# simonamtoft/downsampled-diffusion

Hardware: AMD Instinct MI355X
Metric: images/sec (T=1000 sampling), 256x256 dDDPM-x3 (higher is better)
Workload: dtype f32

## Files before the change

downsampled-diffusion_amd/csrc/attention.hip:

```cpp
#include <cstdlib>

#include "conv_common.h"

namespace ddk {

constexpr int DH = 32;

constexpr int PART = DH + DH + DH * DH;

__global__ __launch_bounds__(256) void linattn_context_kernel(const float* __restrict__ qkv, float* __restrict__ ctx,
                                                              float* __restrict__ part, int HW, int heads, int splits, int rows_per_split,
                                                              int kv_only) {
    __shared__ __attribute__((aligned(16))) float stage[4 * 32 * 33];
    float* kexp = stage;
    float* vs = stage + 64 * DH;
    __shared__ float smax[8 * DH];
    const int bh = blockIdx.x / splits, sp = blockIdx.x % splits;
    const int b = bh / heads, h = bh % heads;
    const int HC = heads * DH, RS = (kv_only ? 2 : 3) * HC;
    const float* base = qkv + (long long)b * HW * RS;
    const float* kp = base + (kv_only ? 0 : HC) + h * DH;
    const float* vp = kp + HC;
    const int tid = threadIdx.x;
    const int n_begin = sp * rows_per_split, n_end = min(HW, n_begin + rows_per_split);

    {
        const int d = tid & 31, ng = tid >> 5;
        float m = -INFINITY;
        for (int n = n_begin + ng; n < n_end; n += 8) m = fmaxf(m, kp[(long long)n * RS + d]);
        smax[ng * DH + d] = m;
        __syncthreads();
        if (tid < DH) {
            float mm = smax[tid];
#pragma unroll
            for (int j = 1; j < 8; ++j) mm = fmaxf(mm, smax[j * DH + tid]);
            smax[tid] = mm;
        }
        __syncthreads();
    }

    const int d = tid >> 3, e0 = (tid & 7) * 4;
    typedef float ctx_f32x16 __attribute__((ext_vector_type(16)));
    const int lane = tid & 63, wv = tid >> 6, l31 = lane & 31, kh = lane >> 5;
    ctx_f32x16 macc;
#pragma unroll
    for (int r = 0; r < 16; ++r) macc[r] = 0.f;
    float dsum = 0.f;
    for (int n0 = n_begin; n0 < n_end; n0 += 64) {
#pragma unroll
        for (int j = 0; j < 2; ++j) {
            const int idx4 = tid + j * 256;
            const int row = idx4 >> 3, c = (idx4 & 7) * 4;
            float4 kv = make_float4(0.f, 0.f, 0.f, 0.f), vv = kv;
            if (n0 + row < n_end) {
                kv = *reinterpret_cast<const float4*>(kp + (long long)(n0 + row) * RS + c);
                vv = *reinterpret_cast<const float4*>(vp + (long long)(n0 + row) * RS + c);
                kv.x = __expf(kv.x - smax[c]);
                kv.y = __expf(kv.y - smax[c + 1]);
                kv.z = __expf(kv.z - smax[c + 2]);
                kv.w = __expf(kv.w - smax[c + 3]);
            }
            *reinterpret_cast<float4*>(kexp + row * DH + c) = kv;
            *reinterpret_cast<float4*>(vs + row * DH + c) = vv;
        }
        __syncthreads();
#pragma unroll
        for (int s2 = 0; s2 < 8; ++s2) {
            const int n = wv * 16 + 2 * s2 + kh;
            const float a = kexp[n * DH + l31];
            macc = __builtin_amdgcn_mfma_f32_32x32x2f32(a, vs[n * DH + l31], macc, 0, 0, 0);
            dsum += a;
        }
        __syncthreads();
    }
    float4 acc;
    float den;
    {
        float* pt = stage;
        static_assert(4 * 32 * 33 >= 2 * 64 * DH, "the staging array holds both tiles");
#pragma unroll
        for (int r = 0; r < 16; ++r) pt[(wv * 32 + (r & 3) + 8 * (r >> 2) + 4 * kh) * 33 + l31] = macc[r];
        dsum += __shfl_xor(dsum, 32, 64);
        __shared__ float dpart[4 * DH];
        if (kh == 0) dpart[wv * DH + l31] = dsum;
        __syncthreads();
        acc = make_float4(0.f, 0.f, 0.f, 0.f);
        den = 0.f;
#pragma unroll
        for (int w = 0; w < 4; ++w) {
            const float* q = pt + (w * 32 + d) * 33 + e0;
            acc.x += q[0]; acc.y += q[1]; acc.z += q[2]; acc.w += q[3];
            den += dpart[w * DH + d];
        }
    }
    if (splits == 1) {
        const float inv = 1.0f / den;
        acc.x *= inv; acc.y *= inv; acc.z *= inv; acc.w *= inv;
        *reinterpret_cast<float4*>(ctx + ((long long)bh * DH + d) * DH + e0) = acc;
    } else {
        float* pp = part + ((long long)bh * splits + sp) * PART;
        if (e0 == 0) { pp[d] = smax[d]; pp[DH + d] = den; }
        *reinterpret_cast<float4*>(pp + 2 * DH + d * DH + e0) = acc;
    }
}

__global__ __launch_bounds__(256) void linattn_merge_kernel(const float* __restrict__ part, float* __restrict__ ctx, int splits) {
    const int bh = blockIdx.x, tid = threadIdx.x;
    const int d = tid >> 3, e0 = (tid & 7) * 4;
    const float* pp = part + (long long)bh * splits * PART;
    float M = -INFINITY;
    for (int s = 0; s < splits; ++s) M = fmaxf(M, pp[s * PART + d]);
    float4 acc = make_float4(0.f, 0.f, 0.f, 0.f);
    float den = 0.f;
    for (int s = 0; s < splits; ++s) {
        const float w = expf(pp[s * PART + d] - M);
        const float4 a = *reinterpret_cast<const float4*>(pp + s * PART + 2 * DH + d * DH + e0);
        den += pp[s * PART + DH + d] * w;
        acc.x += a.x * w; acc.y += a.y * w; acc.z += a.z * w; acc.w += a.w * w;
    }
    const float inv = 1.0f / den;
    acc.x *= inv; acc.y *= inv; acc.z *= inv; acc.w *= inv;
    *reinterpret_cast<float4*>(ctx + ((long long)bh * DH + d) * DH + e0) = acc;
}

constexpr int KC_K = 128, KC_BM = 64;
constexpr int KC_W_FLOATS = 128 * KC_K, KC_A_FLOATS = KC_BM * KC_K;
constexpr int KC_LDS_FLOATS = KC_W_FLOATS + 2 * KC_A_FLOATS + 2 * KC_BM + 64 + 64 + 8 * 64 + 8 * DH;

#if !defined(DDK_TUNING) || !defined(DDK_KVCTX_ABL)
#undef DDK_KVCTX_ABL
#define DDK_KVCTX_ABL 0
#endif
struct KvCtxParams {
    const float* x;
    const float* w;
    const float* c1;
    const float* c2;
    float eps;
    float* part;
    int tiles_per_image, tiles_per_split, splits;
};

__global__ __launch_bounds__(512) void attn_kvctx_kernel(const KvCtxParams p) {
    extern __shared__ __attribute__((aligned(16))) float smem[];
    float* Ws = smem;
    float* As = smem + KC_W_FLOATS;
    float* rowstat = As + 2 * KC_A_FLOATS;
    float* Mx = rowstat + 2 * KC_BM;
    float* Sc = Mx + 64;
    float* cmx = Sc + 64;
    float* dpart = cmx + 8 * 64;
    const int tid = threadIdx.x, lane = tid & 63;
    const int wid = __builtin_amdgcn_readfirstlane(tid >> 6);
    const int sp = blockIdx.x, hp = blockIdx.y, b = blockIdx.z;
// ... 366 lines not shown
        *reinterpret_cast<float4*>(vs + row * DH + c) = vv;
        qs[row * (DH + 1) + c] = qv.x; qs[row * (DH + 1) + c + 1] = qv.y; qs[row * (DH + 1) + c + 2] = qv.z; qs[row * (DH + 1) + c + 3] = qv.w;
    }
    __syncthreads();
    if constexpr (ROWS >= 128) linattn_core_mfma<ROWS>(ks, vs, qs, cs, smax, part, ctx, out, b, h, HW, heads);
    else linattn_small_core<ROWS>(ks, vs, qs, cs, smax, ctx, out, b, h, HW, heads);
}

static size_t small_lds_bytes(int rows) {
    return ((size_t)rows * DH * 2 + (size_t)rows * (DH + 1) + DH * (DH + 4) + 16 * DH + (rows >= 128 ? 4 * 32 * 33 : 0)) * 4;
}

typedef float f32x4_att __attribute__((ext_vector_type(4)));
constexpr int QP_PITCH = 100;

__host__ __device__ static inline size_t small_qkv_lds_bytes(int MB, int C) {
    const size_t xs = (size_t)16 * MB * (C + 4), part = (size_t)4 * 16 * MB * QP_PITCH;
    const size_t core = 64 * DH * 2 + 64 * (DH + 1) + DH * (DH + 4) + 8 * DH + 128 + 192;
    return ((xs > part ? xs : part) + core) * 4;
}

template <int MB>
__global__ __launch_bounds__(256) void linattn_small_qkv_kernel(const float* __restrict__ x, const float* __restrict__ wop,
                                                                const float* __restrict__ c1, const float* __restrict__ c2, float ln_eps,
                                                                float* __restrict__ ctx, float* __restrict__ out, int HW, int C, int heads) {
    extern __shared__ __align__(16) float sm[];
    constexpr int ROWS = 16 * MB;
    const int pitch = C + 4, nch = C >> 5;
    const size_t big = (size_t)ROWS * pitch > (size_t)4 * ROWS * QP_PITCH ? (size_t)ROWS * pitch : (size_t)4 * ROWS * QP_PITCH;
    float* xs = sm;
    float* ks = sm + big;
    float* vs = ks + 64 * DH;
    float* qs = vs + 64 * DH;
    float* cs = qs + 64 * (DH + 1);
    float* smax = cs + DH * (DH + 4);
    float* rowstat = smax + 8 * DH;
    float* cfold = rowstat + 128;
    const int b = blockIdx.x / heads, h = blockIdx.x % heads;
    const int tid = threadIdx.x, lane = tid & 63;
    const int wave = __builtin_amdgcn_readfirstlane(tid >> 6);
    const int m = lane & 15, kq = lane >> 4;
    const int HC = heads * DH;

    const float* wl = wop + (size_t)h * nch * 3072 + lane * 4;
    float4 bA[6][2], bB[6][2];
    auto load_b = [&](int chunk, float4 (&bq)[6][2]) {
        chunk = chunk < nch ? chunk : nch - 1;
        const float* wp = wl + (size_t)chunk * 3072;
#pragma unroll
        for (int nb = 0; nb < 6; ++nb) {
            bq[nb][0] = *reinterpret_cast<const float4*>(wp + nb * 512);
            bq[nb][1] = *reinterpret_cast<const float4*>(wp + nb * 512 + 256);
        }
    };
    load_b(wave, bA);
    load_b(wave + 4, bB);
    if (tid < 192) {
        const int n = tid % 96;
        const int col = (n >> 5) * HC + h * DH + (n & 31);
        cfold[tid] = tid < 96 ? c1[col] : c2[col];
    }
    {
        const int q4 = C >> 2;
        for (int i = tid; i < ROWS * q4; i += 256) {
            const int row = i / q4, c = (i - row * q4) << 2;
            const float4 v = row < HW ? *reinterpret_cast<const float4*>(x + ((long long)b * HW + row) * C + c) : make_float4(0.f, 0.f, 0.f, 0.f);
            *reinterpret_cast<float4*>(xs + row * pitch + c) = v;
        }
    }
    __syncthreads();
    {
        constexpr int TPR = 256 / ROWS;
        const int row = tid / TPR, sub = tid % TPR;
        float s1 = 0.f;
        for (int c = sub * 4; c < C; c += TPR * 4) {
            const float4 v = *reinterpret_cast<const float4*>(xs + row * pitch + c);
            s1 += (v.x + v.y) + (v.z + v.w);
        }
#pragma unroll
        for (int o = 1; o < TPR; o <<= 1) s1 += __shfl_xor(s1, o, 64);
        const float inv_c = 1.0f / (float)C;
        const float mean = s1 * inv_c;
        float s2 = 0.f;
        for (int c = sub * 4; c < C; c += TPR * 4) {
            const float4 v = *reinterpret_cast<const float4*>(xs + row * pitch + c);
            const float a0 = v.x - mean, a1 = v.y - mean, a2 = v.z - mean, a3 = v.w - mean;
            s2 += (a0 * a0 + a1 * a1) + (a2 * a2 + a3 * a3);
        }
#pragma unroll
        for (int o = 1; o < TPR; o <<= 1) s2 += __shfl_xor(s2, o, 64);
        if (sub == 0) {
            const float var = s2 * inv_c;
            const float r = 1.0f / (sqrtf(var) + ln_eps);
            rowstat[2 * row] = r;
            rowstat[2 * row + 1] = r * mean;
        }
    }

    f32x4_att acc[MB][6];
#pragma unroll
    for (int i = 0; i < MB; ++i)
#pragma unroll
        for (int nb = 0; nb < 6; ++nb) acc[i][nb] = f32x4_att{0.f, 0.f, 0.f, 0.f};
    auto compute = [&](int chunk, const float4 (&bq)[6][2]) {
        float4 a[MB][2];
#pragma unroll
        for (int i = 0; i < MB; ++i) {
            const float* ap = xs + (i * 16 + m) * pitch + (chunk << 5) + kq * 8;
            a[i][0] = *reinterpret_cast<const float4*>(ap);
            a[i][1] = *reinterpret_cast<const float4*>(ap + 4);
        }
#pragma unroll
        for (int kk = 0; kk < 8; ++kk)
#pragma unroll
            for (int i = 0; i < MB; ++i) {
                const float av = reinterpret_cast<const float*>(&a[i][0])[kk];
#pragma unroll
                for (int nb = 0; nb < 6; ++nb)
                    acc[i][nb] = __builtin_amdgcn_mfma_f32_16x16x4f32(av, reinterpret_cast<const float*>(&bq[nb][0])[kk], acc[i][nb], 0, 0, 0);
            }
    };
    for (int c = wave; c < nch; c += 8) {
        compute(c, bA);
        load_b(c + 8, bA);
        if (c + 4 < nch) compute(c + 4, bB);
        load_b(c + 12, bB);
    }
    __syncthreads();
#pragma unroll
    for (int i = 0; i < MB; ++i)
#pragma unroll
        for (int nb = 0; nb < 6; ++nb)
#pragma unroll
            for (int r = 0; r < 4; ++r) xs[((wave * ROWS) + i * 16 + kq * 4 + r) * QP_PITCH + nb * 16 + m] = acc[i][nb][r];
    __syncthreads();
    for (int e = tid; e < ROWS * 96; e += 256) {
        const int row = e / 96, n = e - row * 96;
        const int sel = n >> 5, d = n & 31;
        float v = sel == 1 ? -INFINITY : 0.f;
        if (row < HW) {
            float s = xs[row * QP_PITCH + n];
#pragma unroll
            for (int w = 1; w < 4; ++w) s += xs[(w * ROWS + row) * QP_PITCH + n];
            v = rowstat[2 * row] * s - rowstat[2 * row + 1] * cfold[n] + cfold[96 + n];
        }
        if (sel == 0) qs[row * (DH + 1) + d] = v;
        else if (sel == 1) ks[row * DH + d] = v;
        else vs[row * DH + d] = v;
    }
    __syncthreads();
    linattn_small_core<ROWS>(ks, vs, qs, cs, smax, ctx, out, b, h, HW, heads);
}

__global__ __launch_bounds__(256) void qkv_operand_pack_kernel(const float* __restrict__ lnw, float* __restrict__ wop, int heads, int cp,
                                                               long long total) {
    const int nch = cp >> 5, HC = heads * DH;
    for (long long idx = blockIdx.x * 256LL + threadIdx.x; idx < total; idx += (long long)gridDim.x * 256) {
        const int j = (int)(idx & 3), lane = (int)((idx >> 2) & 63), half = (int)((idx >> 8) & 1);
        long long r = idx >> 9;
        const int nb = (int)(r % 6); r /= 6;
        const int chunk = (int)(r % nch);
        const int head = (int)(r / nch);
        const int o = (nb >> 1) * HC + head * DH + (nb & 1) * 16 + (lane & 15);
        const int i = chunk * 32 + (lane >> 4) * 8 + half * 4 + j;
        wop[idx] = lnw[(long long)o * cp + i];
    }
}

typedef float f32x16_att __attribute__((ext_vector_type(16)));
__global__ __launch_bounds__(512) void linattn_apply_kernel(const float* __restrict__ qkv, const float* __restrict__ ctx,
                                                            float* __restrict__ out, int HW, int heads, int tiles_per_sample) {
    extern __shared__ __attribute__((aligned(16))) float qs[];
    const int b = blockIdx.x / tiles_per_sample, tile = blockIdx.x % tiles_per_sample;
    const int HC = heads * DH, RS = 3 * HC;
    const int nthreads = 64 * heads;
    const int n0 = tile * 64;
    const int f4_per_row = HC / 4;
    for (int i = threadIdx.x; i < 64 * f4_per_row; i += nthreads) {
        const int row = i / f4_per_row, c4 = i - row * f4_per_row;
        float4 v = make_float4(0.f, 0.f, 0.f, 0.f);
        if (n0 + row < HW) v = *reinterpret_cast<const float4*>(qkv + ((long long)b * HW + n0 + row) * RS + c4 * 4);
        const int hh = (c4 * 4) / DH, d = (c4 * 4) % DH;
        float* dst = qs + (hh * 64 + row) * 33 + d;
        dst[0] = v.x; dst[1] = v.y; dst[2] = v.z; dst[3] = v.w;
    }
    const int h = threadIdx.x >> 6, lane = threadIdx.x & 63;
    const int l31 = lane & 31, fh = lane >> 5;
    const float* cp = ctx + ((long long)b * heads + h) * DH * DH + l31;
    float bf[16];
#pragma unroll
    for (int kk = 0; kk < 16; ++kk) bf[kk] = cp[(2 * kk + fh) * DH];
    __syncthreads();
    const float* qh = qs + h * 64 * 33;
    f32x16_att acc0, acc1;
#pragma unroll
    for (int r = 0; r < 16; ++r) { acc0[r] = 0.f; acc1[r] = 0.f; }
#pragma unroll
    for (int kk = 0; kk < 16; ++kk) {
        const float a0 = qh[l31 * 33 + 2 * kk + fh], a1 = qh[(32 + l31) * 33 + 2 * kk + fh];
        acc0 = __builtin_amdgcn_mfma_f32_32x32x2f32(a0, bf[kk], acc0, 0, 0, 0);
        acc1 = __builtin_amdgcn_mfma_f32_32x32x2f32(a1, bf[kk], acc1, 0, 0, 0);
    }
#pragma unroll
    for (int r = 0; r < 16; ++r) {
        const int px = (r & 3) + 8 * (r >> 2) + 4 * fh;
        if (n0 + px < HW) out[((long long)b * HW + n0 + px) * HC + h * DH + l31] = acc0[r];
        if (n0 + 32 + px < HW) out[((long long)b * HW + n0 + 32 + px) * HC + h * DH + l31] = acc1[r];
    }
}

static void linattn_splits(int B, int HW, int heads, int& splits, int& rows) {
    const int max_s = (int)ceil_div(HW, 64);
#ifdef DDK_TUNING
    const char* cap_env = getenv("DDK_LINATTN_WGS");
    const int cap = cap_env ? atoi(cap_env) : 1024;
#else
    const int cap = 1024;
#endif
    int s = cap / (B * heads);
    if (s < 1) s = 1;
    if (s > max_s) s = max_s;
    rows = (int)(ceil_div(ceil_div(HW, s), 64) * 64);
    splits = (int)ceil_div(HW, rows);
}

size_t linattn_context_workspace_bytes(int B, int HW, int heads) {
    if (B <= 0 || HW <= 0 || heads <= 0) return 0;
    int s, rows;
    linattn_splits(B, HW, heads, s, rows);
    return s > 1 ? (size_t)B * heads * s * PART * sizeof(float) : 0;
}

int linattn_context(const float* qkv, float* ctx, int B, int HW, int heads, void* workspace, size_t workspace_bytes, hipStream_t st,
                    bool kv_only) {
    DDK_REQUIRE(qkv && ctx && B > 0 && HW > 0 && heads > 0, "linattn_context: arguments");
    DDK_REQUIRE(aligned16(qkv) && aligned16(ctx) && aligned16(workspace), "linattn_context: alignment");
    int s, rows;
    linattn_splits(B, HW, heads, s, rows);
    if (s > 1 && (!workspace || workspace_bytes < (size_t)B * heads * s * PART * sizeof(float))) {
        if (workspace) {
            set_error("linattn_context: workspace too small (%zu < %zu)", workspace_bytes, (size_t)B * heads * s * PART * sizeof(float));
            return DDK_ERR_WORKSPACE;
        }
        s = 1;
        rows = HW;
    }
    hipLaunchKernelGGL(linattn_context_kernel, dim3(B * heads * s), dim3(256), 0, st, qkv, ctx, static_cast<float*>(workspace), HW, heads, s, rows,
                       kv_only ? 1 : 0);
    DDK_TRY(check_launch("linattn_context_kernel"));
    if (s > 1) {
        hipLaunchKernelGGL(linattn_merge_kernel, dim3(B * heads), dim3(256), 0, st, static_cast<const float*>(workspace), ctx, s);
        DDK_TRY(check_launch("linattn_merge_kernel"));
    }
    return DDK_OK;
}

int linattn_fused_small(const float* qkv, float* ctx, float* out, int B, int HW, int heads, hipStream_t st) {
    DDK_REQUIRE(qkv && ctx && out && B > 0 && HW > 0 && HW <= 256 && heads > 0, "linattn_fused_small: arguments (HW <= 256)");
    DDK_REQUIRE(aligned16(qkv) && aligned16(ctx) && aligned16(out), "linattn_fused_small: alignment");
    DDK_TRY(ensure_device_init());
    if (HW <= 64)
        hipLaunchKernelGGL(linattn_small_kernel<64>, dim3(B * heads), dim3(256), small_lds_bytes(64), st, qkv, ctx, out, HW, heads);
    else
        hipLaunchKernelGGL(linattn_small_kernel<256>, dim3(B * heads), dim3(256), small_lds_bytes(256), st, qkv, ctx, out, HW, heads);
    return check_launch("linattn_small_kernel");
}

bool linattn_small_qkv_ok(int HW, int C) { return HW > 0 && HW <= 64 && C % 32 == 0 && C >= 32 && small_qkv_lds_bytes(HW <= 16 ? 1 : 4, C) <= 160 * 1024; }

constexpr int FOLD_C = 128;
constexpr int FOLD_LDS_FLOATS = FOLD_C * FOLD_C + 32 * (FOLD_C + 1) + 2 * FOLD_C;
typedef float f32x16_att __attribute__((ext_vector_type(16)));
__global__ __launch_bounds__(256) void attn_fold_kernel(const float* __restrict__ ctx, const float* __restrict__ wqg,
                                                        const float* __restrict__ c1q, const float* __restrict__ c2q,
                                                        const float* __restrict__ wout, const float* __restrict__ bout,
                                                        float* __restrict__ A, float* __restrict__ a1, float* __restrict__ a2) {
    extern __shared__ __align__(16) float sm[];
    float* T = sm;
    float* Wq = T + FOLD_C * FOLD_C;
    float* t1 = Wq + 32 * (FOLD_C + 1);
    float* t2 = t1 + FOLD_C;
    const int b = blockIdx.x, nq = blockIdx.y, tid = threadIdx.x, lane = tid & 63;
    const int wave = __builtin_amdgcn_readfirstlane(tid >> 6);
    const int l31 = lane & 31, kh = lane >> 5;
    {
        const float* cp = ctx + ((long long)b * 4 + wave) * DH * DH;
        const float* wp = wqg + (long long)wave * DH * FOLD_C;
        f32x16_att acc[4];
#pragma unroll
        for (int j = 0; j < 4; ++j)
#pragma unroll
            for (int r = 0; r < 16; ++r) acc[j][r] = 0.f;
        float av[DH / 2], bv[DH / 2][4];
#pragma unroll
        for (int s2 = 0; s2 < DH / 2; ++s2) {
            const int d = 2 * s2 + kh;
            av[s2] = cp[d * DH + l31];
#pragma unroll
            for (int j = 0; j < 4; ++j) bv[s2][j] = wp[d * FOLD_C + j * 32 + l31];
        }
        __builtin_amdgcn_sched_barrier(0);
#pragma unroll
        for (int s2 = 0; s2 < DH / 2; ++s2)
#pragma unroll
            for (int j = 0; j < 4; ++j) acc[j] = __builtin_amdgcn_mfma_f32_32x32x2f32(av[s2], bv[s2][j], acc[j], 0, 0, 0);
#pragma unroll
        for (int j = 0; j < 4; ++j)
#pragma unroll
            for (int r = 0; r < 16; ++r) T[(wave * DH + (r & 3) + 8 * (r >> 2) + 4 * kh) * FOLD_C + j * 32 + l31] = acc[j][r];
    }
    for (int i = tid; i < 32 * FOLD_C; i += 256) Wq[(i >> 7) * (FOLD_C + 1) + (i & 127)] = wout[(long long)nq * 32 * FOLD_C + i];
    if (tid < FOLD_C) {
        const int h = tid >> 5, e = tid & 31;
        const float* ch = ctx + ((long long)b * 4 + h) * DH * DH;
        float u1 = 0.f, u2 = 0.f;
#pragma unroll
        for (int d = 0; d < DH; ++d) {
            const float cv = ch[d * DH + e];
            u1 += cv * c1q[h * DH + d];
            u2 += cv * c2q[h * DH + d];
        }
        t1[tid] = u1;
        t2[tid] = u2;
    }
    __syncthreads();
    {
        f32x16_att acc;
#pragma unroll
        for (int r = 0; r < 16; ++r) acc[r] = 0.f;
#pragma unroll 8
        for (int s2 = 0; s2 < FOLD_C / 2; ++s2) {
            const int he = 2 * s2 + kh;
            acc = __builtin_amdgcn_mfma_f32_32x32x2f32(Wq[l31 * (FOLD_C + 1) + he], T[he * FOLD_C + wave * 32 + l31], acc, 0, 0, 0);
        }
        float* Ab = A + ((long long)b * FOLD_C + nq * 32) * FOLD_C + wave * 32 + l31;
#pragma unroll
        for (int r = 0; r < 16; ++r) Ab[((r & 3) + 8 * (r >> 2) + 4 * kh) * FOLD_C] = acc[r];
        if (tid < 32) {
            float u1 = 0.f, u2 = 0.f;
#pragma unroll 16
            for (int he = 0; he < FOLD_C; ++he) {
                u1 += Wq[tid * (FOLD_C + 1) + he] * t1[he];
                u2 += Wq[tid * (FOLD_C + 1) + he] * t2[he];
            }
            const int n = nq * 32 + tid;
            a1[(long long)b * FOLD_C + n] = u1;
            a2[(long long)b * FOLD_C + n] = u2 + (bout ? bout[n] : 0.f);
        }
    }
}

int linattn_small_qkv_init_device() {
    DDK_HIP(hipFuncSetAttribute(reinterpret_cast<const void*>(attn_kvctx_kernel), hipFuncAttributeMaxDynamicSharedMemorySize,
                                (int)(KC_LDS_FLOATS * sizeof(float))));
    DDK_HIP(hipFuncSetAttribute(reinterpret_cast<const void*>(attn_fold_kernel), hipFuncAttributeMaxDynamicSharedMemorySize,
                                (int)(FOLD_LDS_FLOATS * sizeof(float))));
    DDK_HIP(hipFuncSetAttribute(reinterpret_cast<const void*>(linattn_small_kernel<256>), hipFuncAttributeMaxDynamicSharedMemorySize, 160 * 1024));
    DDK_HIP(hipFuncSetAttribute(reinterpret_cast<const void*>(linattn_small_qkv_kernel<1>), hipFuncAttributeMaxDynamicSharedMemorySize, 160 * 1024));
    DDK_HIP(hipFuncSetAttribute(reinterpret_cast<const void*>(linattn_small_qkv_kernel<4>), hipFuncAttributeMaxDynamicSharedMemorySize, 160 * 1024));
    return DDK_OK;
}

int qkv_operand_pack(const float* lnw, float* wop, int heads, int cp, hipStream_t st) {
    DDK_REQUIRE(lnw && wop && heads > 0 && cp > 0 && cp % 32 == 0, "qkv_operand_pack: arguments");
    const long long total = (long long)3 * heads * DH * cp;
    const long long blocks = ceil_div(total, 256);
    hipLaunchKernelGGL(qkv_operand_pack_kernel, dim3((unsigned)(blocks < 2048 ? blocks : 2048)), dim3(256), 0, st, lnw, wop, heads, cp, total);
    return check_launch("qkv_operand_pack_kernel");
}

int linattn_small_qkv(const float* x, const float* wop, const float* c1, const float* c2, float ln_eps, float* ctx, float* out, int B, int HW,
                      int C, int heads, hipStream_t st) {
    DDK_REQUIRE(x && wop && c1 && c2 && ctx && out && B > 0 && heads > 0, "linattn_small_qkv: arguments");
    DDK_REQUIRE(linattn_small_qkv_ok(HW, C), "linattn_small_qkv: needs H*W <= 64 and C % 32 == 0 (LDS budget)");
    DDK_REQUIRE(aligned16(x) && aligned16(wop) && aligned16(ctx) && aligned16(out), "linattn_small_qkv: alignment");
    DDK_TRY(ensure_device_init());
    if (HW <= 16)
        hipLaunchKernelGGL(linattn_small_qkv_kernel<1>, dim3(B * heads), dim3(256), small_qkv_lds_bytes(1, C), st, x, wop, c1, c2, ln_eps, ctx, out,
                           HW, C, heads);
    else
        hipLaunchKernelGGL(linattn_small_qkv_kernel<4>, dim3(B * heads), dim3(256), small_qkv_lds_bytes(4, C), st, x, wop, c1, c2, ln_eps, ctx, out,
                           HW, C, heads);
    return check_launch("linattn_small_qkv_kernel");
}

bool attn_kvctx_ok(int B, int HW, int C, int heads) { return B > 0 && C == KC_K && heads == 4 && HW >= 4 * KC_BM && HW % KC_BM == 0; }
int attn_kvctx_splits(int B, int HW) {
    const int tiles = HW / KC_BM;
    int s = 1;
    while (s * 2 <= tiles && tiles % (s * 2) == 0 && (long long)B * 2 * (s * 2) <= 256) s *= 2;
    return s;
}
size_t attn_kvctx_workspace_bytes(int B, int HW) { return (size_t)B * 4 * attn_kvctx_splits(B, HW) * PART * sizeof(float); }

int attn_kvctx(const float* x, const float* w_kv, const float* c1, const float* c2, float ln_eps, float* ctx, int B, int HW, void* workspace,
               size_t workspace_bytes, hipStream_t st) {
    DDK_REQUIRE(x && w_kv && c1 && c2 && ctx && workspace, "attn_kvctx: null pointer");
    DDK_REQUIRE(attn_kvctx_ok(B, HW, KC_K, 4), "attn_kvctx: needs 128 channels, 4 heads, H*W a multiple of 64 and >= 256");
    DDK_REQUIRE(aligned16(x) && aligned16(w_kv) && aligned16(c1) && aligned16(c2) && aligned16(ctx) && aligned16(workspace), "attn_kvctx: alignment");
    DDK_REQUIRE((long long)B * HW * KC_K * 4 < (1LL << 32) && B <= 65535, "attn_kvctx: input of 4 GiB or more, or more than 65535 images");
    const int s = attn_kvctx_splits(B, HW);
    if (workspace_bytes < attn_kvctx_workspace_bytes(B, HW)) {
        set_error("attn_kvctx: workspace too small (%zu < %zu)", workspace_bytes, attn_kvctx_workspace_bytes(B, HW));
        return DDK_ERR_WORKSPACE;
    }
    DDK_TRY(ensure_device_init());
    KvCtxParams p{x, w_kv, c1, c2, ln_eps, static_cast<float*>(workspace), HW / KC_BM, HW / KC_BM / s, s};
    hipLaunchKernelGGL(attn_kvctx_kernel, dim3((unsigned)s, 2, (unsigned)B), dim3(512), KC_LDS_FLOATS * sizeof(float), st, p);
    DDK_TRY(check_launch("attn_kvctx_kernel"));
    hipLaunchKernelGGL(linattn_merge_kernel, dim3(B * 4), dim3(256), 0, st, static_cast<const float*>(workspace), ctx, s);
    return check_launch("linattn_merge_kernel");
}

bool attn_fold_ok(int C, int heads) { return C == FOLD_C && heads * DH == FOLD_C; }
size_t attn_fold_out_floats(int B) { return (size_t)B * (FOLD_C * FOLD_C + 2 * FOLD_C); }

int attn_fold(const float* ctx, const float* wqg, const float* c1q, const float* c2q, const float* wout, const float* bout, float* A,
              float* a1, float* a2, int B, int C, int heads, hipStream_t st) {
    DDK_REQUIRE(ctx && wqg && c1q && c2q && wout && A && a1 && a2 && B > 0, "attn_fold: arguments");
    DDK_REQUIRE(attn_fold_ok(C, heads), "attn_fold: C == 128 and heads * 32 == 128 only");
    DDK_REQUIRE(aligned16(ctx) && aligned16(wout) && aligned16(A), "attn_fold: alignment");
    DDK_TRY(ensure_device_init());
    hipLaunchKernelGGL(attn_fold_kernel, dim3(B, 4), dim3(256), FOLD_LDS_FLOATS * sizeof(float), st, ctx, wqg, c1q, c2q, wout, bout, A, a1, a2);
    return check_launch("attn_fold_kernel");
}

int linattn_apply(const float* qkv, const float* ctx, float* out, int B, int HW, int heads, hipStream_t st) {
    DDK_REQUIRE(qkv && ctx && out && B > 0 && HW > 0, "linattn_apply: arguments");
    DDK_REQUIRE(heads >= 1 && heads <= 8, "linattn_apply: heads must be in 1..8");
    DDK_REQUIRE(aligned16(qkv) && aligned16(ctx) && aligned16(out), "linattn_apply: alignment");
    const int tiles = (int)ceil_div(HW, 64);
    const size_t lds = (size_t)heads * 64 * 33 * sizeof(float);
    hipLaunchKernelGGL(linattn_apply_kernel, dim3(B * tiles), dim3(64 * heads), lds, st, qkv, ctx, out, HW, heads, tiles);
    return check_launch("linattn_apply_kernel");
}

}

extern "C" {
size_t ddk_linattn_context_workspace_bytes(int B, int HW, int heads) { return ddk::linattn_context_workspace_bytes(B, HW, heads); }
int ddk_linattn_context(const float* qkv, float* ctx, int B, int HW, int heads, void* workspace, size_t workspace_bytes, ddk_stream_t s) {
    return ddk::linattn_context(qkv, ctx, B, HW, heads, workspace, workspace_bytes, ddk::as_stream(s), false);
}
int ddk_linattn_context_kv(const float* kv, float* ctx, int B, int HW, int heads, void* workspace, size_t workspace_bytes, ddk_stream_t s) {
    return ddk::linattn_context(kv, ctx, B, HW, heads, workspace, workspace_bytes, ddk::as_stream(s), true);
}
size_t ddk_attention_kv_context_workspace_bytes(int B, int HW) { return ddk::attn_kvctx_workspace_bytes(B, HW); }
int ddk_attention_kv_context_ok(int B, int HW, int C, int heads) { return ddk::attn_kvctx_ok(B, HW, C, heads) ? 1 : 0; }
int ddk_attention_kv_context(const float* x, const float* w_kv, const float* c1, const float* c2, float ln_eps, float* ctx, int B, int HW,
                             void* workspace, size_t workspace_bytes, ddk_stream_t s) {
    return ddk::attn_kvctx(x, w_kv, c1, c2, ln_eps, ctx, B, HW, workspace, workspace_bytes, ddk::as_stream(s));
}
int ddk_attention_fold(const float* ctx, const float* wqg, const float* c1q, const float* c2q, const float* wout, const float* bout, float* A,
                       float* a1, float* a2, int B, int C, int heads, ddk_stream_t s) {
    return ddk::attn_fold(ctx, wqg, c1q, c2q, wout, bout, A, a1, a2, B, C, heads, ddk::as_stream(s));
}
int ddk_linattn_fused_small(const float* qkv, float* ctx, float* out, int B, int HW, int heads, ddk_stream_t s) {
    return ddk::linattn_fused_small(qkv, ctx, out, B, HW, heads, ddk::as_stream(s));
}
int ddk_pack_qkv_operand(const float* folded_w, float* dst, int heads, int c_pad, ddk_stream_t s) {
    return ddk::qkv_operand_pack(folded_w, dst, heads, c_pad, ddk::as_stream(s));
}
int ddk_linattn_small_from_x(const float* x, const float* w_operand, const float* c1, const float* c2, float ln_eps, float* ctx, float* out,
                             int B, int HW, int C, int heads, ddk_stream_t s) {
    return ddk::linattn_small_qkv(x, w_operand, c1, c2, ln_eps, ctx, out, B, HW, C, heads, ddk::as_stream(s));
}
int ddk_linattn_apply(const float* qkv, const float* ctx, float* out, int B, int HW, int heads, ddk_stream_t s) {
    return ddk::linattn_apply(qkv, ctx, out, B, HW, heads, ddk::as_stream(s));
}
}
```

downsampled-diffusion_amd/csrc/ddk_internal.h:

```cpp
#pragma once
#include <hip/hip_runtime.h>

#include <cstdarg>
#include <cstddef>
#include <cstdint>
#include <cstdio>

#include "ddk.h"

#ifdef DDK_HOST_SANITIZE
#include "host_sanitize.h"
#endif

namespace ddk {

void set_error(const char* fmt, ...);

inline int fail_arg(const char* what) {
    set_error("bad argument: %s", what);
    return DDK_ERR_ARG;
}

inline int check_launch(const char* what) {
    hipError_t e = hipGetLastError();
    if (e != hipSuccess) {
        set_error("%s: %s", what, hipGetErrorString(e));
        return DDK_ERR_HIP;
    }
    return DDK_OK;
}

#define DDK_REQUIRE(cond, msg)              \
    do {                                    \
        if (!(cond)) return ddk::fail_arg(msg); \
    } while (0)

#define DDK_HIP(call)                                                    \
    do {                                                                 \
        hipError_t e_ = (call);                                          \
        if (e_ != hipSuccess) {                                          \
            ddk::set_error("%s: %s", #call, hipGetErrorString(e_));      \
            return DDK_ERR_HIP;                                          \
        }                                                                \
    } while (0)

#define DDK_TRY(expr)              \
    do {                           \
        int rc_ = (expr);          \
        if (rc_ != DDK_OK) return rc_; \
    } while (0)

inline bool aligned16(const void* p) { return (reinterpret_cast<uintptr_t>(p) & 15u) == 0; }
inline hipStream_t as_stream(ddk_stream_t s) { return reinterpret_cast<hipStream_t>(s); }
inline long long ceil_div(long long a, long long b) { return (a + b - 1) / b; }

__device__ __forceinline__ float mish_f(float x) {
    if (x > 20.0f) return x;
    const float e = __expf(x);
    const float n = e * (e + 2.0f);
    return x * (n * __frcp_rn(n + 2.0f));
}

__device__ __forceinline__ float mish_grad_f(float u) {
    if (u > 20.0f) return 1.0f;
    const float e = __expf(u);
    const float n = e * (e + 2.0f);
    const float r = __frcp_rn(n + 2.0f);
    return n * r + u * (4.0f * e * (e + 1.0f)) * (r * r);
}

__device__ __forceinline__ int div_upr(int u, int upr) {
    return (upr & (upr - 1)) == 0 ? u >> (31 - __builtin_clz(upr)) : u / upr;
}
__device__ __forceinline__ long long div_upr(long long u, int upr) {
    return (upr & (upr - 1)) == 0 ? u >> (31 - __builtin_clz(upr)) : u / upr;
}

__device__ __forceinline__ float wave_sum(float v) {
#pragma unroll
    for (int o = 32; o > 0; o >>= 1) v += __shfl_xor(v, o, 64);
    return v;
}

__device__ __forceinline__ float wave_max(float v) {
#pragma unroll
    for (int o = 32; o > 0; o >>= 1) v = fmaxf(v, __shfl_xor(v, o, 64));
    return v;
}

__device__ __forceinline__ float block_sum(float v, float* red) {
    v = wave_sum(v);
    const int lane = threadIdx.x & 63, wid = threadIdx.x >> 6, nw = blockDim.x >> 6;
    __syncthreads();
    if (lane == 0) red[wid] = v;
    __syncthreads();
    float t = (lane < nw) ? red[lane] : 0.0f;
    t = wave_sum(t);
    return t;
}

__device__ __forceinline__ float block_max(float v, float* red) {
    v = wave_max(v);
    const int lane = threadIdx.x & 63, wid = threadIdx.x >> 6, nw = blockDim.x >> 6;
    __syncthreads();
    if (lane == 0) red[wid] = v;
    __syncthreads();
    float t = (lane < nw) ? red[lane] : -INFINITY;
    t = wave_max(t);
    return t;
}

int ensure_device_init();
int conv_init_device();
int wgrad_init_device();

size_t conv_workspace_bytes(int kind, int B, int H, int W, int cin, int N);
struct ConvLnFold {
    const float* c1;
    const float* c2;
    float eps;
};
struct WinoGnFuse {
    const float* gamma;
    const float* beta;
    const float* temb;
    const long long* temb_rows;
    int temb_stride;
    float eps;
    int groups;
    float* records;
    unsigned* counters;
    unsigned* fail;
    unsigned* pairs = nullptr;
    const float* res_x = nullptr;
    const float* res_w = nullptr;
    const float* res_b = nullptr;
    int res_cin = 0, res_ld = 0;
};
bool conv_ln_fold_ok(int B, int H, int W, int cin, int N);
int conv_forward(const ddk_conv_args& a, hipStream_t st, const ConvLnFold* ln = nullptr, const WinoGnFuse* fuse = nullptr);
int conv_splits(int kind, int B, int H, int W, int cin, int N);
bool conv_wino_ok(int kind, int H, int W, int cin, int N);
int conv_wino_splits(int B, int H, int W, int cin, int N);
int conv_wino_forward(const ddk_conv_args& a, int splits, hipStream_t st, const WinoGnFuse* fuse = nullptr);
int conv_wino_cluster_np(int B, int H, int W, int cin, int N, int groups);
int conv_wino_cluster_split_np(int B, int H, int W, int cin, int N, int groups, int* splits_out);
size_t conv_wino_cluster_pair_words(int B, int H, int W, int N);
bool conv_wino_variant_new(int B, int H, int W, int N);
bool conv_wino_cluster_device_ok();
size_t conv_wino_cluster_ws_floats(int B, int H, int W, int N);
unsigned conv_wino_cluster_timeouts();
unsigned conv_first_cluster_timeouts();
unsigned level_chain_cluster_timeouts();
constexpr size_t CL_PAIR_WORDS = 128 * 16;
inline size_t cl_fail_offset(int B) { return (size_t)B * 8 * 16; }
inline size_t cl_front_floats(int B) { return cl_fail_offset(B) + 16; }
inline size_t cl_chain_offset(int B) { return cl_front_floats(B); }
inline size_t cl_pair_offset(int B) { return cl_chain_offset(B) + (size_t)B * 64; }
inline size_t cl_counter_floats(int B) { return cl_pair_offset(B) + CL_PAIR_WORDS; }
struct ClWords { unsigned* counters; unsigned* fail; };
inline ClWords cl_words(float* cl, int B) { return {reinterpret_cast<unsigned*>(cl), reinterpret_cast<unsigned*>(cl + cl_fail_offset(B))}; }
int cluster_fail_check(unsigned* word, hipStream_t st, const char* who, const char* tail);
bool convT_wino_ok(int H, int W, int cin, int N);
int convT_wino_splits(int B, int H, int W, int cin, int N);
int convT_wino_forward(const ddk_conv_args& a, int splits, hipStream_t st);
int conv_wino_init_device();
int conv_wino_stats_parts(int B, int H, int W, int cin, int N, int groups);
bool conv_first_ok(int cin, int N, int H, int W, int groups);
int conv_first(const float* x, const float* wp, const float* bias, float* out, float* gn_partials, int B, int H, int W, int cin, int N,
               int groups, int64_t* counter, int64_t* t_cur, hipStream_t st);
int conv_first_init_device();
bool conv_first_gn_ok(int cin, int N, int H, int W, int groups);
size_t conv_first_gn_ws_floats(int B, int H, int W);
int conv_first_gn(const float* x, const float* wp, const float* bias, const float* gamma, const float* beta, const float* temb,
                  int temb_stride, const long long* temb_rows, float eps, float* out, int B, int H, int W, int cin, int N, int groups,
                  float* records, unsigned* counters, unsigned* fail, int64_t* counter, int64_t* t_cur, hipStream_t st);
bool conv1x1_sm_ok(long long M, int c0, int c1, int N);
int conv1x1_sm(const float* src0, int c0, const float* src1, int c1, const float* w, const float* bias, const float* resid, float* out,
               long long M, int N, const ConvLnFold* ln, hipStream_t st);
int conv1x1_sm_init_device();
bool conv1x1_stream_ok(long long M, int cin, int N);
int conv1x1_stream(const float* x, int cin, const float* w, const float* bias, const float* dmish_src, const float* resid, float* out,
                   float* mish_out, long long M, int N, int pre_mish, int post_mish, hipStream_t st);
bool conv1x1_ws_ok(long long M, int K, int N);
int conv1x1_ws(const float* x, const float* w, const float* bias, const float* resid, float* out, long long M, int N, const ConvLnFold* ln,
               hipStream_t st, int images = 0);
int conv1x1_ws_init_device();
struct AddendSlabs {
    int n = 1;
    long long stride = 0;
    const float* bias = nullptr;
};
bool conv_gn_local_ok(int H, int W, int cin, int c0, int N, int groups);
int conv_gn_local(const float* src0, int c0, const float* src1, int c1, const float* w, const float* bias, const float* gamma,
                  const float* beta, const float* temb, int temb_stride, const long long* temb_rows, const float* addend, float* out,
                  int B, int H, int W, int N, int groups, float eps, hipStream_t st, const AddendSlabs& as = AddendSlabs(),
                  const AddendSlabs& src_slabs = AddendSlabs());
int conv_gn_local_init_device();
bool conv_gn_wlocal_ok(int H, int W, int cin, int c0, int N, int groups);
int conv_gn_wlocal(const float* src0, int c0, const float* src1, int c1, const float* w, const float* bias, const float* gamma,
                   const float* beta, const float* temb, int temb_stride, const long long* temb_rows, const float* addend, float* out,
                   int B, int H, int W, int N, int groups, float eps, hipStream_t st, const AddendSlabs& as = AddendSlabs(),
                   const AddendSlabs& src_slabs = AddendSlabs());
double conv_flops(int kind, int B, int H, int W, int cin, int N);
size_t groupnorm_workspace_bytes(int B, int HW, int C, int groups);
int gn_train_nsplit(int HW, int cpg);
int gn_stats_partials(const float* x, float* part, int B, int HW, int C, int groups, int ns, hipStream_t st);
int groupnorm_mish(const float* x, const float* gamma, const float* beta, const float* temb, int temb_stride,
                   const float* addend, float* out, int B, int HW, int C, int groups, float eps, void* ws, size_t ws_bytes,
                   hipStream_t st, const long long* temb_rows = nullptr);
int groupnorm_mish_ex(const float* x, int nslab, long long slab_stride, const float* cbias, const float* gamma,
                      const float* beta, const float* temb, int temb_stride, const float* addend, float* out, int B, int HW, int C,
                      int groups, float eps, void* ws, size_t ws_bytes, hipStream_t st, const long long* temb_rows = nullptr);
int groupnorm_mish_parts(const float* x, const float* part, int np, const float* gamma, const float* beta, const float* temb,
                         int temb_stride, const float* addend, float* out, int B, int HW, int C, int groups, float eps, hipStream_t st,
                         const long long* temb_rows = nullptr, const float* rc_x = nullptr, const float* rc_w = nullptr,
                         const float* rc_b = nullptr, int rc_cin = 0, int rc_ld = 0);
int chan_layernorm(const float* x, const float* g, const float* b, float* out, long long M, int C, float eps, hipStream_t st);
int groupnorm_mish_generic(const float* x, const float* gamma, const float* beta, const float* temb, int temb_stride, const float* addend,
                           float* out, int B, int HW, int CP, int C, int groups, float eps, hipStream_t st, const long long* temb_rows = nullptr);
int chan_layernorm_generic(const float* x, const float* g, const float* b, float* out, long long M, int CP, int C, float eps, hipStream_t st);
int unary(int op, const float* x, float* out, long long n, hipStream_t st);
int add(const float* a, const float* b, float* out, long long n, hipStream_t st);
int avgpool2(const float* x, float* out, int B, int H, int W, int C, hipStream_t st);
int upsample_nearest2(const float* x, float* out, int B, int H, int W, int C, hipStream_t st);
size_t linattn_context_workspace_bytes(int B, int HW, int heads);
int linattn_context(const float* qkv, float* ctx, int B, int HW, int heads, void* workspace, size_t workspace_bytes, hipStream_t st,
                    bool kv_only = false);
bool attn_fold_ok(int C, int heads);
bool attn_kvctx_ok(int B, int HW, int C, int heads);
size_t attn_kvctx_workspace_bytes(int B, int HW);
int attn_kvctx(const float* x, const float* w_kv, const float* c1, const float* c2, float ln_eps, float* ctx, int B, int HW, void* workspace,
               size_t workspace_bytes, hipStream_t st);
size_t attn_fold_out_floats(int B);
int attn_fold(const float* ctx, const float* wqg, const float* c1q, const float* c2q, const float* wout, const float* bout, float* A,
              float* a1, float* a2, int B, int C, int heads, hipStream_t st);
int linattn_apply(const float* qkv, const float* ctx, float* out, int B, int HW, int heads, hipStream_t st);
int linattn_fused_small(const float* qkv, float* ctx, float* out, int B, int HW, int heads, hipStream_t st);
bool linattn_small_qkv_ok(int HW, int C);
int linattn_small_qkv_init_device();
int qkv_operand_pack(const float* lnw, float* wop, int heads, int cp, hipStream_t st);
int linattn_small_qkv(const float* x, const float* wop, const float* c1, const float* c2, float ln_eps, float* ctx, float* out, int B, int HW,
                      int C, int heads, hipStream_t st);
int time_mlp(const int64_t* t, const float* freqs, const float* w1t, const float* b1, const float* w2t, const float* b2,
             float* act, float* raw, int B, int dim, hipStream_t st);
int time_proj(const float* act, const float* wt, const float* bias, float* out, int B, int dim, int n_out, hipStream_t st);
int conv1x1_small_n(const float* x, const float* w, const float* bias, float* out, long long M, int C, int n_out, hipStream_t st);
struct InpaintOps {
    const float* known;
    const float* mask;
    const float *ka, *kb;
    const float *ja, *jb;
};
struct NoisyTables {
    const float *lam, *sgm;
};
constexpr uint32_t INPAINT_Z2_BIT = 0x40000000u;
constexpr uint32_t INPAINT_Z3_BIT = 0x20000000u;
struct RestoreOps {
    const float* y;
    int n;
    int H, W;
    int gray;
    const float* mask;
};
static_assert(sizeof(RestoreOps) == 32 && offsetof(RestoreOps, mask) == 24, "RestoreOps: gray fills the padding, nothing moves");
constexpr int GRAY_MEAN = 1;
constexpr int GRAY_LUMA = 2;
struct VlbStep {
    const float* x;
    float* xt;
    const float* noise;
    long long noise_step_stride;
    int t_first;
    const float *c_recip, *c_recipm1, *c1, *c2, *logvar;
    float* partials;
    int nslot;
};
constexpr uint32_t VLB_STREAM_BIT = 0x80000000u;

enum class StepKind {
    Eps,
    Ancestral,
    Multistep,
    Inpaint,
    Restore,
    RestoreMasked,
    Vlb,
    RestoreMultistep,
    RestoreNoisy,
    RestoreGray
};
struct StepRule {
    StepKind kind;
    float* eps_out;
    float* x;
    const float* noise;
    long long noise_step_stride;
    int t_first;
    const float *c_recip, *c_recipm1, *c1, *c2, *sigma;
    float* x0_hist;
    const float* c3;
    union {
        InpaintOps inp;
        NoisyTables nsy;
    };
    const VlbStep* vlb;
    RestoreOps rst;
};
inline StepRule vlb_rule(const VlbStep& v) {
    StepRule r{};
    r.kind = StepKind::Vlb;
    r.x = const_cast<float*>(v.x); r.noise = v.noise; r.noise_step_stride = v.noise_step_stride; r.t_first = v.t_first;
    r.c_recip = v.c_recip; r.c_recipm1 = v.c_recipm1; r.c1 = v.c1; r.c2 = v.c2;
    r.vlb = &v;
    return r;
}
struct ChainHooks {
    const int64_t* chain_state;
    int64_t* dec_counter;
    uint64_t seed;
    uint32_t stream_id;
};
int p_update(const StepRule& r, const float* eps_hat, const int64_t* t, int B, long long per, const ChainHooks& h, hipStream_t st,
             const char* who = "p_update");
int randn(float* out, long long n, uint64_t seed, uint32_t step, uint32_t stream_id, hipStream_t st);
int vlb_sweep_slots_unfused(int B, long long per);
int vlb_step_input(const VlbStep& v, const float* sqrt_acp, const float* sqrt_1m_acp, const int64_t* chain_state, int B, long long per,
                   hipStream_t st);
int vlb_sweep_finalize(const float* partials, int nslot, float* vlb_t, float* l_simple_t, int T, int B, long long per, hipStream_t st);
struct TailIn {
    const float* raw;
    const float* part;
    int np;
    const float *gamma, *beta;
    float eps;
    const float* w;
    const float* bias;
    int n_out, B, HW, C, groups;
};
bool final_tail_ok(int HW, int C, int groups, int n_out, int np, StepKind kind, int restore_w = 0, int restore_n = 0);
int final_tail(const TailIn& in, const StepRule& r, const int64_t* t, const ChainHooks& h, hipStream_t st);

}
```

downsampled-diffusion_amd/csrc/unet_plan.hip:

```cpp
#include <algorithm>
#include <mutex>
#include <string>
#include <vector>

#include "ddk_internal.h"
#include "level_chain.h"

namespace ddk {

constexpr int HEADS = 4;
constexpr int HIDDEN = HEADS * 32;
constexpr int GROUPS = 8;
constexpr float GN_EPS = 1e-5f, LN_EPS = 1e-5f;

static inline int pad32(int c) { return (c + 31) / 32 * 32; }

enum PackKind { PK_COPY = 0, PK_CONV = 1, PK_CONVT = 2, PK_LINEAR_T = 3, PK_WINO = 4, PK_LOCAL = 5, PK_WLOCAL = 6, PK_FIRST = 7, PK_CONVT_WINO = 8,
                PK_ROWS = 9 , PK_LOCAL1 = 10 ,
                PK_CONVT_LOCAL = 11  };

struct Slot {
    std::string name;
    long long numel;
    int kind;
    size_t off;
    int O, I, KH, KW, i_pad, ld, col0;
    int split = 0, split_pad = 0;
    int attn = -1;
};

struct ConvW {
    size_t w = 0, b = 0;
    bool has_bias = false;
    int cin = 0, cin_pad = 0, cout = 0;
    size_t wu = 0;
    bool has_wu = false;
    size_t wl = 0;
    bool has_wl = false;
    size_t wwl = 0;
    bool has_wwl = false;
    size_t wf = 0;
    bool has_wf = false;
    size_t wl1 = 0;
    bool has_wl1 = false;
    size_t wtl = 0;
    bool has_wtl = false;
};
struct NormW { size_t g = 0, b = 0; int c_real = 0; };
struct ResW {
    int ci = 0, ci_pad = 0, co = 0, temb_off = 0, ci_real = 0, co_real = 0;
    ConvW c1, c2, res;
    NormW n1, n2;
    bool has_res = false;
};
struct AttnW {
    int c = 0, c_real = 0;
    NormW ln;
    ConvW qkv, out;
    size_t qkv_lnw = 0, ln_c1 = 0, ln_c2 = 0;
    size_t qkv_op = 0;
};

}

using namespace ddk;

struct ChainKey {
    StepKind kind;
    const void* bufs[14];
    const void* ws;
    const void* noise;
    int B, H, W, t_start, device;
    unsigned long long pack_epoch;
    int restore_n = 0;
    bool restore_mask = false;
    int restore_gray = 0;
    bool operator==(const ChainKey& o) const {
        for (int i = 0; i < 14; ++i)
            if (bufs[i] != o.bufs[i]) return false;
        return kind == o.kind && ws == o.ws && noise == o.noise && B == o.B && H == o.H && W == o.W && t_start == o.t_start &&
               device == o.device && pack_epoch == o.pack_epoch && restore_n == o.restore_n && restore_mask == o.restore_mask && restore_gray == o.restore_gray;
    }
};
struct SamplerGraph {
    ChainKey key;
    hipGraph_t graph = nullptr;
    hipGraphExec_t exec = nullptr;
    hipGraph_t graph_multi = nullptr;
    hipGraphExec_t exec_multi = nullptr;
    hipEvent_t done = nullptr;
    unsigned long long last_use = 0;
};
constexpr int SAMPLER_MULTI = 16;

struct ddk_unet {
    std::mutex mu;
    std::vector<SamplerGraph> graphs;
    unsigned long long use_clock = 0;
    unsigned long long pack_epoch = 0;
    struct {
        const void* ws = nullptr;
        int t_start = -1, B = 0, H = 0, W = 0;
        unsigned long long pack_epoch = 0;
        std::vector<int64_t> map;
    } table;
    ddk_unet_config cfg;
    int cluster_gn = 1;
    int cluster_limit = 1 << 30;
    int cluster_np_max = 8;
    bool cluster_split = true;
    bool attn_kvctx = true;
    bool fold_down_reduce = false;
    bool restore_fused = true;
    bool first_gn = true;
    int level_chain = 9;
    int level_chain_max_batch = 32;
    int attn_fold_min_hw = 256;
    bool attn_fold = true;
    bool generic = false;
    std::vector<int> dimp;
    std::vector<Slot> slots;
    size_t packed_floats = 0;
    int L = 0;
    std::vector<int> dims;
    int time_dim = 0, temb_total = 0;
    size_t freqs = 0, w1t = 0, b1 = 0, w2t = 0, b2 = 0, temb_wt = 0, temb_bias = 0;
    std::vector<ResW> down_res, up_res;
    std::vector<AttnW> down_attn, up_attn;
    std::vector<ConvW> down_conv, up_conv;
    ResW mid1, mid2;
    AttnW mid_attn;
    ConvW final_conv;
    NormW final_norm;
    size_t final_w = 0, final_b = 0;

    size_t alloc(size_t n) {
        const size_t o = packed_floats;
        packed_floats += (n + 3) / 4 * 4;
        return o;
    }
    size_t add_copy(const std::string& name, long long n) {
        const size_t o = alloc((size_t)n);
        slots.push_back(Slot{name, n, PK_COPY, o, 0, 0, 0, 0, 0, 0, 0});
        return o;
    }
    void add_copy_at(const std::string& name, long long n, size_t off) {
        slots.push_back(Slot{name, n, PK_COPY, off, 0, 0, 0, 0, 0, 0, 0});
    }
    ConvW add_conv(const std::string& prefix, int cout, int cin, int k, bool bias, bool gn_follows = false, int split = 0, bool local = false) {
        ConvW c;
        c.cin = cin; c.cin_pad = split > 0 ? pad32(split) + pad32(cin - split) : pad32(cin); c.cout = cout;
        const int cout_rows = pad32(cout);
        c.w = alloc((size_t)cout_rows * k * k * c.cin_pad);
        Slot sl{prefix + "weight", (long long)cout * cin * k * k, PK_CONV, c.w, cout, cin, k, k, c.cin_pad, 0, 0};
        if (split > 0 && c.cin_pad != cin) { sl.split = split; sl.split_pad = pad32(split); }
        slots.push_back(sl);
        c.has_bias = bias;
        if (bias) {
            c.b = alloc((size_t)cout_rows);
            slots.push_back(Slot{prefix + "bias", cout, PK_COPY, c.b, 0, 0, 0, 0, 0, 0, 0});
        }
        if (generic) return c;
        if (k == 1 && bias && cout % 32 == 0 && c.cin_pad == cin && cin % 32 == 0) {
            c.wl1 = alloc((size_t)cout * c.cin_pad);
            c.has_wl1 = true;
            slots.push_back(Slot{prefix + "weight", (long long)cout * cin, PK_LOCAL1, c.wl1, cout, cin, 1, 1, c.cin_pad, 0, 0});
        }
        if (k == 3 && cout % 64 == 0) {
            c.wu = alloc((size_t)16 * cout * c.cin_pad);
            c.has_wu = true;
            slots.push_back(Slot{prefix + "weight", (long long)cout * cin * k * k, PK_WINO, c.wu, cout, cin, k, k, c.cin_pad, 0, 0});
        }
        if (k == 3 && (gn_follows || local) && cout % 32 == 0) {
            c.wl = alloc((size_t)9 * cout * c.cin_pad);
            c.has_wl = true;
            slots.push_back(Slot{prefix + "weight", (long long)cout * cin * k * k, PK_LOCAL, c.wl, cout, cin, k, k, c.cin_pad, 0, 0});
            if (gn_follows && (c.cin_pad <= 320 || c.cin_pad == 512)) {
                c.wwl = alloc((size_t)16 * cout * c.cin_pad);
                c.has_wwl = true;
                slots.push_back(Slot{prefix + "weight", (long long)cout * cin * k * k, PK_WLOCAL, c.wwl, cout, cin, k, k, c.cin_pad, 0, 0});
            }
        }
        return c;
    }
    ConvW add_convT(const std::string& prefix, int ch, bool local = false) {
        ConvW c;
        c.cin = ch; c.cin_pad = pad32(ch); c.cout = ch;
        c.w = alloc((size_t)16 * pad32(ch) * pad32(ch));
        slots.push_back(Slot{prefix + "weight", (long long)16 * ch * ch, PK_CONVT, c.w, ch, ch, 4, 4, pad32(ch), 0, 0});
        c.has_bias = true;
        c.b = alloc((size_t)pad32(ch));
        slots.push_back(Slot{prefix + "bias", ch, PK_COPY, c.b, 0, 0, 0, 0, 0, 0, 0});
        if (local && ch % 32 == 0 && !generic) {
            c.wtl = alloc((size_t)16 * ch * ch);
            c.has_wtl = true;
            slots.push_back(Slot{prefix + "weight", (long long)16 * ch * ch, PK_CONVT_LOCAL, c.wtl, ch, ch, 4, 4, ch, 0, 0});
        }
        if (ch % 128 == 0) {
            c.wu = alloc((size_t)36 * ch * ch);
            c.has_wu = true;
            slots.push_back(Slot{prefix + "weight", (long long)16 * ch * ch, PK_CONVT_WINO, c.wu, ch, ch, 4, 4, ch, 0, 0});
        }
        return c;
    }
    NormW add_norm(const std::string& wname, const std::string& bname, int c) {
        NormW n;
        n.c_real = c;
        n.g = alloc((size_t)pad32(c));
        slots.push_back(Slot{wname, c, PK_COPY, n.g, 0, 0, 0, 0, 0, 0, 0});
        n.b = alloc((size_t)pad32(c));
        slots.push_back(Slot{bname, c, PK_COPY, n.b, 0, 0, 0, 0, 0, 0, 0});
        return n;
    }
    ResW add_res(const std::string& p, int ci, int co, int& temb_cursor, int split = 0) {
        ResW r;
        r.ci_real = ci; r.co_real = co;
        r.ci = ci; r.ci_pad = split > 0 ? pad32(split) + pad32(ci - split) : pad32(ci); r.co = pad32(co);
        if (!generic) r.co = co;
        r.temb_off = temb_cursor;
        temb_cursor += co;
        slots.push_back(Slot{p + "mlp.1.weight", (long long)co * time_dim, PK_LINEAR_T, temb_wt, co, time_dim, 0, 0, 0, temb_total, r.temb_off});
        add_copy_at(p + "mlp.1.bias", co, temb_bias + r.temb_off);
        r.c1 = add_conv(p + "block1.block.0.", co, ci, 3, true, true, split);
        r.n1 = add_norm(p + "block1.block.1.weight", p + "block1.block.1.bias", co);
        r.c2 = add_conv(p + "block2.block.0.", co, co, 3, true, true);
        r.n2 = add_norm(p + "block2.block.1.weight", p + "block2.block.1.bias", co);
        r.has_res = ci != co;
        if (r.has_res) r.res = add_conv(p + "res_conv.", co, ci, 1, true, false, split);
        return r;
    }
    int n_attn = 0;
    std::vector<AttnW> attn_all;
    AttnW add_attn(const std::string& p, int c) {
        AttnW a;
        a.c = generic ? pad32(c) : c;
        a.c_real = c;
        const size_t s0 = slots.size();
        a.qkv = add_conv(p + "fn.fn.to_qkv.", 3 * HIDDEN, c, 1, false);
        const size_t s1 = slots.size();
        a.out = add_conv(p + "fn.fn.to_out.", c, HIDDEN, 1, true);
        const size_t s2 = slots.size();
        a.ln = add_norm(p + "fn.norm.g", p + "fn.norm.b", c);
        for (size_t i = s0; i < s1; ++i) slots[i].attn = n_attn;
        for (size_t i = s2; i < slots.size(); ++i) slots[i].attn = n_attn;
        a.qkv_lnw = alloc((size_t)3 * HIDDEN * pad32(c));
        a.ln_c1 = alloc((size_t)3 * HIDDEN);
        a.ln_c2 = alloc((size_t)3 * HIDDEN);
        a.qkv_op = alloc((size_t)3 * HIDDEN * pad32(c));
        attn_all.push_back(a);
        ++n_attn;
        return a;
    }
};

static int total_temb(const ddk_unet& u) {
    int tot = 0;
    for (int l = 0; l < u.L; ++l) tot += 2 * u.dims[l + 1];
    tot += 2 * u.dims[u.L];
    for (int i = 0; i < u.L - 1; ++i) tot += 2 * u.dims[u.L - 1 - i];
    return tot;
}

extern "C" ddk_unet* ddk_unet_create(const ddk_unet_config* cfg) {
    if (!cfg || cfg->n_levels < 1 || cfg->n_levels > 8 || cfg->in_ch < 1 || cfg->chan < 8 || cfg->chan % 8 ||
        cfg->chan > 512) {
        set_error("unet_create: need 1 <= n_levels <= 8, in_ch >= 1, unet_chan a multiple of 8 in [8, 512]");
        return nullptr;
    }
    for (int i = 0; i < cfg->n_levels; ++i)
        if (cfg->mults[i] < 1) { set_error("unet_create: unet_dims entries must be >= 1"); return nullptr; }
    if (cfg->mults[0] != 1) {
        set_error("unet_create: unet_dims[0] must be 1 (the reference's final Block(dim, dim) meets dim * unet_dims[0] channels "
                  "otherwise and raises, unet.py:69-72)");
        return nullptr;
    }
    {
        int ndev = 0;
        if (hipGetDeviceCount(&ndev) == hipSuccess && ndev > 0 && ensure_device_init() != DDK_OK) return nullptr;
        (void)hipGetLastError();
    }
    ddk_unet* u = new ddk_unet();
    u->cfg = *cfg;
    u->L = cfg->n_levels;
    u->generic = cfg->chan % 32 != 0;
    for (int i = 0; i < cfg->n_levels; ++i)
        if (cfg->chan * cfg->mults[i] > 512) { set_error("unet_create: level widths above 512 channels are not supported"); delete u; return nullptr; }
    u->dims.push_back(cfg->in_ch);
    for (int i = 0; i < u->L; ++i) u->dims.push_back(cfg->chan * cfg->mults[i]);
    for (int d : u->dims) u->dimp.push_back(u->generic ? pad32(d) : d);
    u->time_dim = cfg->chan;
    u->temb_total = total_temb(*u);
    const int td = u->time_dim;

    u->freqs = u->add_copy("@sinusoidal_freqs", td / 2);
    u->w1t = u->alloc((size_t)td * 4 * td);
    u->slots.push_back(Slot{"time_mlp.1.weight", (long long)4 * td * td, PK_LINEAR_T, u->w1t, 4 * td, td, 0, 0, 0, 4 * td, 0});
    u->b1 = u->add_copy("time_mlp.1.bias", 4 * td);
    u->w2t = u->alloc((size_t)4 * td * td);
    u->slots.push_back(Slot{"time_mlp.3.weight", (long long)4 * td * td, PK_LINEAR_T, u->w2t, td, 4 * td, 0, 0, 0, td, 0});
    u->b2 = u->add_copy("time_mlp.3.bias", td);
    u->temb_wt = u->alloc((size_t)td * u->temb_total);
    u->temb_bias = u->alloc((size_t)u->temb_total);

    int cur = 0;
    for (int l = 0; l < u->L; ++l) {
        const std::string p = "downs." + std::to_string(l) + ".";
        const int ci = u->dims[l], co = u->dims[l + 1];
        u->down_res.push_back(u->add_res(p + "0.", ci, co, cur));
        if (l == 0 && ci <= 8 && co <= 256 && !u->generic) {
            ConvW& c1 = u->down_res[0].c1;
            const int K2 = (9 * ci + 1) / 2;
            c1.wf = u->alloc((size_t)(co / 32) * K2 * 64);
            c1.has_wf = true;
            u->slots.push_back(Slot{p + "0.block1.block.0.weight", (long long)co * ci * 9, PK_FIRST, c1.wf, co, ci, 3, 3, 0, 0, 0});
        }
        u->down_res.push_back(u->add_res(p + "1.", co, co, cur));
        u->down_attn.push_back(u->add_attn(p + "2.", co));
        if (l < u->L - 1) u->down_conv.push_back(u->add_conv(p + "3.conv.", co, co, 3, true, false, 0, l == u->L - 2));
    }
    const int mid = u->dims[u->L];
    u->mid1 = u->add_res("mid_block1.", mid, mid, cur);
    u->mid_attn = u->add_attn("mid_attn.", mid);
    u->mid2 = u->add_res("mid_block2.", mid, mid, cur);
    for (int i = 0; i < u->L - 1; ++i) {
        const std::string p = "ups." + std::to_string(i) + ".";
        const int din = u->dims[u->L - 1 - i], dout = u->dims[u->L - i];
        u->up_res.push_back(u->add_res(p + "0.", 2 * dout, din, cur, dout));
        u->up_res.push_back(u->add_res(p + "1.", din, din, cur));
        u->up_attn.push_back(u->add_attn(p + "2.", din));
        u->up_conv.push_back(u->add_convT(p + "3.conv.", din, i == 0));
    }
    u->final_conv = u->add_conv("final_conv.0.block.0.", cfg->chan, cfg->chan, 3, true, true);
    u->final_norm = u->add_norm("final_conv.0.block.1.weight", "final_conv.0.block.1.bias", cfg->chan);
    if (u->generic) {
        u->final_w = u->alloc((size_t)cfg->in_ch * pad32(cfg->chan));
        u->slots.push_back(Slot{"final_conv.1.weight", (long long)cfg->in_ch * cfg->chan, PK_ROWS, u->final_w, cfg->in_ch, cfg->chan, 0, 0, 0,
                                pad32(cfg->chan), 0});
    } else {
        u->final_w = u->add_copy("final_conv.1.weight", (long long)cfg->in_ch * cfg->chan);
    }
    u->final_b = u->add_copy("final_conv.1.bias", cfg->in_ch);
    if (cur != u->temb_total) {
        set_error("unet_create: internal temb accounting mismatch");
        delete u;
        return nullptr;
    }
    return u;
}

static void drop_graphs(ddk_unet* u) {
    for (SamplerGraph& g : u->graphs) {
        if (g.exec) (void)hipGraphExecDestroy(g.exec);
        if (g.graph) (void)hipGraphDestroy(g.graph);
        if (g.exec_multi) (void)hipGraphExecDestroy(g.exec_multi);
        if (g.graph_multi) (void)hipGraphDestroy(g.graph_multi);
        if (g.done) (void)hipEventDestroy(g.done);
    }
    u->graphs.clear();
    u->table.ws = nullptr;
}

extern "C" void ddk_unet_destroy(ddk_unet* u) {
    if (!u) return;
    if (!u->graphs.empty()) (void)hipDeviceSynchronize();
    drop_graphs(u);
    delete u;
}

extern "C" int ddk_sampler_invalidate(ddk_unet* u) {
    DDK_REQUIRE(u, "sampler_invalidate: null plan");
    std::lock_guard<std::mutex> lock(u->mu);
    if (!u->graphs.empty()) DDK_HIP(hipDeviceSynchronize());
    drop_graphs(u);
    return DDK_OK;
}
static void destroy_entry(SamplerGraph& g) {
    if (g.done) { (void)hipEventSynchronize(g.done); (void)hipEventDestroy(g.done); }
    if (g.exec) (void)hipGraphExecDestroy(g.exec);
    if (g.graph) (void)hipGraphDestroy(g.graph);
    if (g.exec_multi) (void)hipGraphExecDestroy(g.exec_multi);
    if (g.graph_multi) (void)hipGraphDestroy(g.graph_multi);
}

extern "C" int ddk_sampler_release_workspace(ddk_unet* u, const void* workspace) {
    DDK_REQUIRE(u && workspace, "sampler_release_workspace: arguments");
    std::lock_guard<std::mutex> lock(u->mu);
    for (size_t i = 0; i < u->graphs.size();) {
        if (u->graphs[i].key.ws == workspace) {
            destroy_entry(u->graphs[i]);
            u->graphs.erase(u->graphs.begin() + (long)i);
        } else {
            ++i;
        }
    }
    if (u->table.ws == workspace) u->table.ws = nullptr;
    return DDK_OK;
}

extern "C" int ddk_unet_set_option(ddk_unet* u, int option, int value) {
    DDK_REQUIRE(u, "unet_set_option: null plan");
    static const struct {
        int option;
        bool drops_graphs;
        void (*set)(ddk_unet&, int);
    } options[] = {
        {DDK_OPT_CLUSTER_GROUPNORM, true, [](ddk_unet& p, int v) { p.cluster_gn = v < 0 ? 0 : v > 2 ? 2 : v; }},
        {DDK_OPT_ATTENTION_FOLD, true, [](ddk_unet& p, int v) { p.attn_fold = v != 0; }},
        {DDK_OPT_ATTENTION_KV_CONTEXT, true, [](ddk_unet& p, int v) { p.attn_kvctx = v != 0; }},
        {DDK_OPT_FIRST_GROUPNORM, true, [](ddk_unet& p, int v) { p.first_gn = v != 0; }},
        {DDK_OPT_RESTORE_FUSED_TAIL, true, [](ddk_unet& p, int v) { p.restore_fused = v != 0; }},
        {DDK_OPT_LEVEL_CHAIN, true, [](ddk_unet& p, int v) {
             p.level_chain = v == 1 ? 9 : v == 2 ? 1 : v == 3 ? 15 : v == 4 ? 6 : v == 8 ? 2 : v == 16 ? 4 : v != 0 ? 9 : 0;
         }},
        {DDK_OPT_FOLD_DOWNSAMPLE_REDUCE, true, [](ddk_unet& p, int v) { p.fold_down_reduce = v != 0; }},
        {10, true, [](ddk_unet& p, int v) { p.level_chain_max_batch = v; }},
        {9, true, [](ddk_unet& p, int v) { p.attn_fold_min_hw = v; }},
        {2, false, [](ddk_unet& p, int v) { p.cluster_limit = v; }},
        {4, true, [](ddk_unet& p, int v) { p.cluster_np_max = v; }},
        {11, true, [](ddk_unet& p, int v) { p.cluster_split = v != 0; }},
    };
    for (const auto& o : options) {
        if (o.option != option) continue;
        std::lock_guard<std::mutex> lock(u->mu);
        if (o.drops_graphs) {
            if (!u->graphs.empty()) DDK_HIP(hipDeviceSynchronize());
            drop_graphs(u);
        }
        o.set(*u, value);
        return DDK_OK;
    }
    return fail_arg("unet_set_option: unknown option");
}
extern "C" unsigned ddk_debug_cluster_timeouts(void) {
    unsigned sum = 0;
    for (unsigned v : {ddk::conv_wino_cluster_timeouts(), ddk::conv_first_cluster_timeouts(), ddk::level_chain_cluster_timeouts()}) {
        if (v == ~0u) return ~0u;
        sum += v;
    }
    return sum;
}
extern "C" int ddk_unet_num_slots(const ddk_unet* u) { return u ? (int)u->slots.size() : 0; }
extern "C" const char* ddk_unet_slot_name(const ddk_unet* u, int slot) {
    return (u && slot >= 0 && slot < (int)u->slots.size()) ? u->slots[slot].name.c_str() : nullptr;
}
extern "C" long long ddk_unet_slot_numel(const ddk_unet* u, int slot) {
    return (u && slot >= 0 && slot < (int)u->slots.size()) ? u->slots[slot].numel : -1;
}
extern "C" size_t ddk_unet_packed_bytes(const ddk_unet* u) { return u ? u->packed_floats * sizeof(float) : 0; }

__global__ __launch_bounds__(64) void ln_fold_kernel(const float* __restrict__ w, const float* __restrict__ g, const float* __restrict__ b,
                                                     float* __restrict__ wg, float* __restrict__ c1, float* __restrict__ c2, int C, int cp) {
    const int n = blockIdx.x;
    float s1 = 0.f, s2 = 0.f;
    for (int c = threadIdx.x; c < cp; c += 64) {
        const float wv = w[(long long)n * cp + c];
        const float gv = c < C ? g[c] : 0.f, bv = c < C ? b[c] : 0.f;
        wg[(long long)n * cp + c] = wv * gv;
        s1 += wv * gv;
        s2 += wv * bv;
    }
    s1 = wave_sum(s1);
    s2 = wave_sum(s2);
    if (threadIdx.x == 0) { c1[n] = s1; c2[n] = s2; }
}

static int fold_attn(const AttnW& a, float* P, hipStream_t st) {
    hipLaunchKernelGGL(ln_fold_kernel, dim3(3 * HIDDEN), dim3(64), 0, st, P + a.qkv.w, P + a.ln.g, P + a.ln.b, P + a.qkv_lnw, P + a.ln_c1,
                       P + a.ln_c2, a.c, pad32(a.c));
    DDK_TRY(check_launch("ln_fold_kernel"));
    return qkv_operand_pack(P + a.qkv_lnw, P + a.qkv_op, HEADS, pad32(a.c), st);
}

static void weights_changed(const ddk_unet* u) {
    ddk_unet* m = const_cast<ddk_unet*>(u);
    std::lock_guard<std::mutex> lock(m->mu);
    ++m->pack_epoch;
}

extern "C" int ddk_unet_finalize_pack(const ddk_unet* u, void* packed, ddk_stream_t s) {
    DDK_REQUIRE(u && packed, "unet_finalize_pack: arguments");
    weights_changed(u);
    for (const AttnW& a : u->attn_all) DDK_TRY(fold_attn(a, static_cast<float*>(packed), as_stream(s)));
    return DDK_OK;
}

extern "C" int ddk_unet_pack_slot(const ddk_unet* u, int slot, const float* canonical, void* packed, ddk_stream_t s) {
    DDK_REQUIRE(u && canonical && packed && slot >= 0 && slot < (int)u->slots.size(), "unet_pack_slot: arguments");
    const Slot& sl = u->slots[slot];
    float* dst = static_cast<float*>(packed) + sl.off;
    weights_changed(u);
    int rc;
    switch (sl.kind) {
        case PK_COPY:
            DDK_HIP(hipMemcpyAsync(dst, canonical, (size_t)sl.numel * sizeof(float), hipMemcpyDeviceToDevice, as_stream(s)));
            rc = DDK_OK;
            break;
        case PK_CONV:
            rc = sl.split > 0 ? ddk_pack_conv_weight_split(canonical, dst, sl.O, sl.I, sl.KH, sl.KW, sl.i_pad, sl.split, sl.split_pad, s)
                              : ddk_pack_conv_weight(canonical, dst, sl.O, sl.I, sl.KH, sl.KW, sl.i_pad, s);
            break;
        case PK_CONVT: rc = sl.i_pad == sl.I ? ddk_pack_convT_weight(canonical, dst, sl.I, sl.O, s)
                                             : ddk_pack_convT_weight_padded(canonical, dst, sl.I, sl.O, sl.i_pad, s); break;
        case PK_ROWS:
            DDK_HIP(hipMemcpy2DAsync(dst, (size_t)sl.ld * sizeof(float), canonical, (size_t)sl.I * sizeof(float), (size_t)sl.I * sizeof(float),
                                     (size_t)sl.O, hipMemcpyDeviceToDevice, as_stream(s)));
            rc = DDK_OK;
            break;
        case PK_LINEAR_T: rc = ddk_pack_linear_T(canonical, dst, sl.O, sl.I, sl.ld, sl.col0, s); break;
        case PK_WINO: rc = ddk_pack_conv_weight_wino(canonical, dst, sl.O, sl.I, sl.i_pad, s); break;
        case PK_LOCAL: rc = ddk_pack_conv_weight_local(canonical, dst, sl.O, sl.I, sl.i_pad, s); break;
        case PK_LOCAL1: rc = ddk_pack_conv1x1_weight_local(canonical, dst, sl.O, sl.I, sl.i_pad, s); break;
        case PK_CONVT_LOCAL: rc = ddk_pack_convT_weight_local(canonical, dst, sl.I, sl.O, s); break;
        case PK_WLOCAL: rc = ddk_pack_conv_weight_wino_local(canonical, dst, sl.O, sl.I, sl.i_pad, s); break;
        case PK_FIRST: rc = ddk_pack_conv_weight_first(canonical, dst, sl.O, sl.I, s); break;
        case PK_CONVT_WINO: rc = ddk_pack_convT_weight_wino(canonical, dst, sl.I, sl.O, sl.i_pad, s); break;
        default: return fail_arg("unet_pack_slot: slot kind");
    }
    DDK_TRY(rc);
    if (sl.attn >= 0) DDK_TRY(fold_attn(u->attn_all[sl.attn], static_cast<float*>(packed), as_stream(s)));
    return DDK_OK;
}

namespace ddk {

struct Layout {
    size_t act = 0;
    size_t qkv = 0, o = 0, ctx = 0, splitk = 0, gn_ws = 0, cl = 0, chain = 0;
    std::vector<size_t> skip;
    size_t xpad = 0, temb = 0, tact = 0;
    size_t off_A = 0, off_B = 0, off_C = 0, off_raw = 0, off_a1 = 0, off_res = 0, off_xn = 0, off_qkv = 0, off_o = 0, off_ctx = 0,
           off_splitk = 0, off_gn = 0, off_xpad = 0, off_temb = 0, off_tact = 0, off_cl = 0, off_chain = 0;
    std::vector<size_t> off_skip;
    size_t total = 0;
};

static size_t al4(size_t n) { return (n + 3) / 4 * 4; }

static void upd(size_t& m, size_t v) { if (v > m) m = v; }

static bool convT_wino_use(int B, int H, int W, int cin, int N) {
    return convT_wino_ok(H, W, cin, N) && convT_wino_splits(B, H, W, cin, N) <= 2;
}
static bool use_wino(const ConvW& cw, int H, int W, int cin, int N) {
    return cw.has_wu && conv_wino_ok(DDK_CONV3X3_S1, H, W, cin, N);
}
static size_t conv3_ws_floats(const ConvW& cw, int B, int H, int W, int cin, int N) {
    if (!use_wino(cw, H, W, cin, N)) return conv_workspace_bytes(DDK_CONV3X3_S1, B, H, W, cin, N) / 4;
    const int s = conv_wino_splits(B, H, W, cin, N);
    return s > 1 ? (size_t)s * B * H * W * N : 0;
}

constexpr int CHAIN_BUFS = 18;
constexpr int CHAIN8_BUFS = 5;

static void res_sizes(const ResW& r, int B, int H, int W, Layout& ly) {
    const size_t M = (size_t)B * H * W;
    upd(ly.act, M * r.co);
    upd(ly.splitk, conv3_ws_floats(r.c1, B, H, W, r.ci_pad, r.co));
    upd(ly.splitk, conv3_ws_floats(r.c2, B, H, W, r.co, r.co));
    if (r.has_res) upd(ly.splitk, conv_workspace_bytes(DDK_CONV1X1, B, H, W, r.ci_pad, r.co) / 4);
    upd(ly.gn_ws, groupnorm_workspace_bytes(B, H * W, r.co, GROUPS) / 4);
    upd(ly.gn_ws, (size_t)2 * GROUPS * (M / 128 + 1));
    upd(ly.cl, cl_counter_floats(B) + conv_wino_cluster_ws_floats(B, H, W, r.co));
    if (H * W % 128 == 0 && H * W / 128 <= 8) upd(ly.cl, cl_counter_floats(B) + conv_first_gn_ws_floats(B, H, W));
}

static void attn_sizes(const AttnW& a, int B, int H, int W, Layout& ly) {
    const size_t M = (size_t)B * H * W;
    upd(ly.act, M * a.c);
    upd(ly.qkv, M * 3 * HIDDEN);
    upd(ly.o, M * HIDDEN);
    upd(ly.ctx, (size_t)B * HEADS * 32 * 32);
    upd(ly.splitk, linattn_context_workspace_bytes(B, H * W, HEADS) / 4);
    if (attn_kvctx_ok(B, H * W, a.c, HEADS)) upd(ly.splitk, attn_kvctx_workspace_bytes(B, H * W) / 4);
    upd(ly.splitk, conv_workspace_bytes(DDK_CONV1X1, B, H, W, a.c, 3 * HIDDEN) / 4);
    upd(ly.splitk, conv_workspace_bytes(DDK_CONV1X1, B, H, W, HIDDEN, a.c) / 4);
}

static bool chain_plain(const ResW& r, bool wino) {
    return r.ci == 256 && r.co == 256 && !r.has_res && r.c1.has_bias && r.c2.has_bias && (wino ? r.c1.has_wwl && r.c2.has_wwl : r.c1.has_wl && r.c2.has_wl);
}
static bool chain_att(const AttnW& a) { return a.c == 256 && a.out.has_wl1 && a.out.has_bias; }
static bool chain_cat(const ResW& r, bool wino) {
    return r.ci == 512 && r.ci_pad == 512 && r.co == 256 && r.has_res && r.res.has_wl1 && r.res.has_bias && r.c1.cin_pad == 512 && r.c1.has_bias &&
           r.c2.has_bias && (wino ? r.c1.has_wwl && r.c2.has_wwl : r.c1.has_wl && r.c2.has_wl);
}
static bool level_chain_shape_ok(const ddk_unet& u, int H0, int W0) {
    if (u.generic || u.L < 2) return false;
    const int sh = u.L - 1;
    if ((H0 >> sh) != 4 || (W0 >> sh) != 4 || (H0 & ((1 << sh) - 1)) || (W0 & ((1 << sh) - 1))) return false;
    if (u.dimp[u.L] != 256 || u.dimp[u.L - 1] != 256 || GROUPS != 8) return false;
    return chain_plain(u.down_res[2 * sh], false) && chain_plain(u.down_res[2 * sh + 1], false) && chain_plain(u.mid1, false) &&
           chain_plain(u.mid2, false) && chain_plain(u.up_res[1], false) && chain_att(u.down_attn[sh]) && chain_att(u.mid_attn) &&
           chain_att(u.up_attn[0]) && chain_cat(u.up_res[0], false);
}
static bool level8_chain_shape_ok(const ddk_unet& u, int H0, int W0) {
    if (u.generic || u.L < 3) return false;
    const int sh = u.L - 2;
    if ((H0 >> sh) != 8 || (W0 >> sh) != 8 || (H0 & ((1 << sh) - 1)) || (W0 & ((1 << sh) - 1))) return false;
    if (u.dimp[sh + 1] != 256 || u.dimp[sh] != 256 || u.dimp[sh + 2] != 256 || GROUPS != 8) return false;
    return chain_plain(u.down_res[2 * sh], true) && chain_plain(u.down_res[2 * sh + 1], true) && chain_att(u.down_attn[sh]) &&
           chain_cat(u.up_res[2], true) && chain_plain(u.up_res[3], true) && chain_att(u.up_attn[1]);
}

static Layout make_layout(const ddk_unet& u, int B, int H0, int W0) {
    Layout ly;
    int H = H0, W = W0;
    ly.skip.resize(u.L);
    for (int l = 0; l < u.L; ++l) {
        res_sizes(u.down_res[2 * l], B, H, W, ly);
        res_sizes(u.down_res[2 * l + 1], B, H, W, ly);
        attn_sizes(u.down_attn[l], B, H, W, ly);
        ly.skip[l] = al4((size_t)B * H * W * u.dimp[l + 1]);
        if (l < u.L - 1) {
            upd(ly.splitk, conv_workspace_bytes(DDK_CONV3X3_S2, B, H, W, u.dimp[l + 1], u.dimp[l + 1]) / 4);
            H /= 2; W /= 2;
            upd(ly.act, (size_t)B * H * W * u.dimp[l + 1]);
        }
    }
    res_sizes(u.mid1, B, H, W, ly);
    attn_sizes(u.mid_attn, B, H, W, ly);
    res_sizes(u.mid2, B, H, W, ly);
    for (int i = 0; i < u.L - 1; ++i) {
        res_sizes(u.up_res[2 * i], B, H, W, ly);
        res_sizes(u.up_res[2 * i + 1], B, H, W, ly);
        attn_sizes(u.up_attn[i], B, H, W, ly);
        const int c = pad32(u.up_conv[i].cout);
        upd(ly.splitk, conv_workspace_bytes(DDK_CONVT4X4_S2, B, H, W, c, c) / 4);
        H *= 2; W *= 2;
        upd(ly.act, (size_t)B * H * W * c);
    }
    upd(ly.act, (size_t)B * H * W * pad32(u.cfg.chan));
    upd(ly.splitk, conv3_ws_floats(u.final_conv, B, H, W, pad32(u.cfg.chan), pad32(u.cfg.chan)));
    upd(ly.gn_ws, groupnorm_workspace_bytes(B, H * W, pad32(u.cfg.chan), GROUPS) / 4);
    upd(ly.gn_ws, (size_t)2 * GROUPS * ((size_t)B * H * W / 128 + 1));
    ly.xpad = al4((size_t)B * H0 * W0 * pad32(u.cfg.in_ch));
    ly.temb = al4((size_t)B * u.temb_total);
    ly.tact = al4((size_t)B * u.time_dim);
    ly.act = al4(ly.act); ly.qkv = al4(ly.qkv); ly.o = al4(ly.o); ly.ctx = al4(ly.ctx);
    ly.splitk = al4(ly.splitk); ly.gn_ws = al4(ly.gn_ws); ly.cl = al4(ly.cl);
    if (level_chain_shape_ok(u, H0, W0)) ly.chain = (size_t)CHAIN_BUFS * B * 16 * 256;
    if (level8_chain_shape_ok(u, H0, W0)) upd(ly.chain, (size_t)CHAIN8_BUFS * B * 64 * 256);

    size_t off = 0;
    auto take = [&](size_t n) { const size_t o = off; off += n; return o; };
    ly.off_A = take(ly.act); ly.off_B = take(ly.act); ly.off_C = take(ly.act);
    ly.off_raw = take(ly.act); ly.off_a1 = take(ly.act); ly.off_res = take(ly.act); ly.off_xn = take(ly.act);
    ly.off_qkv = take(ly.qkv); ly.off_o = take(ly.o); ly.off_ctx = take(ly.ctx);
    ly.off_splitk = take(ly.splitk); ly.off_gn = take(ly.gn_ws); ly.off_cl = take(ly.cl); ly.off_chain = take(ly.chain);
    ly.off_xpad = take(ly.xpad); ly.off_temb = take(ly.temb); ly.off_tact = take(ly.tact);
    ly.off_skip.resize(u.L);
    for (int l = 0; l < u.L; ++l) ly.off_skip[l] = take(ly.skip[l]);
    ly.total = off;
    return ly;
}

struct Ctx {
    const ddk_unet& u;
    const float* P;
    float* W;
    const Layout& ly;
    int B;
    hipStream_t st;
    const float* temb;
    const long long* temb_rows;
    bool allow_cluster = false;
    int n_cluster = 0;
    const float* x_first = nullptr;
    const float* x_padded = nullptr;

    ddk_conv_args conv_args(int kind, const ConvW& cw, const float* src0, int c0, const float* src1, int c1, float* out, int H, int Wd, int N,
                            const float* weight_override = nullptr) const {
        ddk_conv_args a{};
        a.kind = kind;
        a.src0 = src0; a.src1 = src1; a.c0 = c0; a.c1 = c1;
        a.weight = weight_override ? weight_override : P + cw.w;
        a.bias = cw.has_bias ? P + cw.b : nullptr;
        a.out = out;
        a.B = B; a.H = H; a.W = Wd; a.N = N;
        a.workspace = W + ly.off_splitk;
        a.workspace_bytes = ly.splitk * sizeof(float);
        if (kind == DDK_CONV3X3_S1 && !weight_override && use_wino(cw, H, Wd, c0 + c1, N)) a.weight_wino = P + cw.wu;
        if (kind == DDK_CONVT4X4_S2 && !weight_override && cw.has_wu && !src1 && convT_wino_use(B, H, Wd, c0, N)) a.weight_wino = P + cw.wu;
        return a;
    }
    WinoGnFuse gn_fuse(const NormW& n, const float* temb_shift, const long long* rows) const {
        float* cl = W + ly.off_cl;
        const ClWords w = cl_words(cl, B);
        return WinoGnFuse{P + n.g, P + n.b, temb_shift, rows, u.temb_total, GN_EPS, GROUPS, cl + cl_counter_floats(B), w.counters, w.fail};
    }
};

static int run_conv(Ctx& c, int kind, const ConvW& cw, const float* src0, int c0, const float* src1, int c1, const float* resid,
                    float* out, int H, int W, int N, const float* weight_override = nullptr, const ConvLnFold* ln = nullptr) {
    ddk_conv_args a = c.conv_args(kind, cw, src0, c0, src1, c1, out, H, W, N, weight_override);
    a.resid = resid;
    return conv_forward(a, c.st, ln);
}
static int run_conv_slabs(Ctx& c, int kind, const ConvW& cw, const float* src0, int c0, const float* src1, int c1, float* out, int H, int W, int N,
                          int splits, AddendSlabs& left) {
    ddk_conv_args a = c.conv_args(kind, cw, src0, c0, src1, c1, out, H, W, N);
    a.bias = nullptr;
    a.defer_reduce = 1;
    const int s = kind == DDK_CONV3X3_S2 ? 2 : 1;
    left = AddendSlabs{splits, (long long)c.B * (H / s) * (W / s) * N, cw.has_bias ? c.P + cw.b : nullptr};
    return conv_forward(a, c.st);
}
static int run_conv_parts(Ctx& c, const ConvW& cw, const float* src0, int c0, const float* src1, int c1, float* raw, int H, int W, int N) {
    ddk_conv_args a = c.conv_args(DDK_CONV3X3_S1, cw, src0, c0, src1, c1, raw, H, W, N);
    a.gn_partials = c.W + c.ly.off_gn;
    a.gn_groups = GROUPS;
    return conv_forward(a, c.st);
}

enum ConvGnPath {
    CG_GENERIC,
    CG_LOCAL,
    CG_WLOCAL,
    CG_FIRST,
    CG_CLUSTER,
    CG_CLUSTER_SPLIT,
    CG_PARTS,
    CG_SLABS,
    CG_PLAIN
};
struct ConvGnChoice {
    ConvGnPath path = CG_PLAIN;
    int np = 0;
    int cl_splits = 1;
    int splits = 1;
    bool wino = false;
    bool local() const { return path == CG_LOCAL || path == CG_WLOCAL; }
};
static ConvGnChoice classify_conv_gn(const ddk_unet& u, const ConvW& cw, int B, int H, int W, int c0, int c1, int N, bool first_input,
                                     bool cluster, size_t splitk_floats) {
    ConvGnChoice k;
    const int cin = c0 + c1;
    auto is = [&](ConvGnPath p) { k.path = p; return k; };
    if (u.generic) return is(CG_GENERIC);
    if (cw.has_wl && (H * W == 16 || (H * W == 4 && B % 4 == 0)) && conv_gn_local_ok(H, W, cin, c0, N, GROUPS)) return is(CG_LOCAL);
    if (cw.has_wwl && H * W == 64 && conv_gn_wlocal_ok(H, W, cin, c0, N, GROUPS)) return is(CG_WLOCAL);
    k.wino = use_wino(cw, H, W, cin, N);
    if (cw.has_wf && first_input && conv_first_ok(u.cfg.in_ch, N, H, W, GROUPS)) return is(CG_FIRST);
    cluster = cluster && cw.has_wu && conv_wino_cluster_device_ok();
    k.np = cluster ? conv_wino_cluster_np(B, H, W, cin, N, GROUPS) : 0;
    if (k.np > 0 && k.np <= u.cluster_np_max) return is(CG_CLUSTER);
    k.np = cluster && u.cluster_split ? conv_wino_cluster_split_np(B, H, W, cin, N, GROUPS, &k.cl_splits) : 0;
    if (k.np > 0 && k.np <= u.cluster_np_max && (size_t)k.cl_splits * B * H * W * N <= splitk_floats &&
        conv_wino_cluster_pair_words(B, H, W, N) <= CL_PAIR_WORDS)
        return is(CG_CLUSTER_SPLIT);
    k.np = cw.has_wu ? conv_wino_stats_parts(B, H, W, cin, N, GROUPS) : 0;
    if (k.np > 0) return is(CG_PARTS);
    k.splits = k.wino ? conv_wino_splits(B, H, W, cin, N) : conv_splits(DDK_CONV3X3_S1, B, H, W, cin, N);
    return is(k.splits > 1 && groupnorm_workspace_bytes(B, H * W, N, GROUPS) == 0 ? CG_SLABS : CG_PLAIN);
}
static bool conv_gn_is_local(const ddk_unet& u, const ConvW& cw, int B, int H, int W, int c0, int c1, int N) {
    return classify_conv_gn(u, cw, B, H, W, c0, c1, N, false, false, 0).local();
}

static int run_conv_gn(Ctx& c, const ConvW& cw, const float* src0, int c0, const float* src1, int c1, float* raw, const NormW& n,
                       const float* temb, const float* addend, float* out, int H, int W, int N, const AddendSlabs& as = AddendSlabs(),
                       const AddendSlabs& ss = AddendSlabs()) {
    const ConvGnChoice k = classify_conv_gn(c.u, cw, c.B, H, W, c0, c1, N, c.x_first && src0 == c.x_padded && !src1,
                                            c.allow_cluster && c.n_cluster < c.u.cluster_limit, c.ly.splitk);
    if (ss.n > 1 && !k.local()) return fail_arg("run_conv_gn: slab source on a path that cannot sum it");
    if (as.n > 1 && !k.local())
        return fail_arg(k.path == CG_GENERIC ? "run_conv_gn: slab addend / source on the generic path"
                                             : "run_conv_gn: slab addend on a path that cannot sum it");
    const float* bias = cw.has_bias ? c.P + cw.b : nullptr;
    const float *g = c.P + n.g, *b = c.P + n.b;
    float* gnp = c.W + c.ly.off_gn;
    switch (k.path) {
        case CG_GENERIC:
            DDK_TRY(run_conv(c, DDK_CONV3X3_S1, cw, src0, c0, src1, c1, nullptr, raw, H, W, N));
            return groupnorm_mish_generic(raw, g, b, temb, c.u.temb_total, addend, out, c.B, H * W, N, n.c_real, GROUPS, GN_EPS, c.st, c.temb_rows);
        case CG_LOCAL:
        case CG_WLOCAL:
            return (k.path == CG_LOCAL ? conv_gn_local : conv_gn_wlocal)(src0, c0, src1, c1, c.P + (k.path == CG_LOCAL ? cw.wl : cw.wwl), bias, g, b,
                       temb, c.u.temb_total, c.temb_rows, addend, out, c.B, H, W, N, GROUPS, GN_EPS, c.st, as, ss);
        case CG_FIRST:
            DDK_TRY(conv_first(c.x_first, c.P + cw.wf, bias, raw, nullptr, c.B, H, W, c.u.cfg.in_ch, N, GROUPS, nullptr, nullptr, c.st));
            break;
        case CG_CLUSTER:
        case CG_CLUSTER_SPLIT: {
            ++c.n_cluster;
            ddk_conv_args a = c.conv_args(DDK_CONV3X3_S1, cw, src0, c0, src1, c1, out, H, W, N);
            a.resid = addend;
            WinoGnFuse f = c.gn_fuse(n, temb, c.temb_rows);
            if (k.path == CG_CLUSTER_SPLIT) f.pairs = reinterpret_cast<unsigned*>(c.W + c.ly.off_cl + cl_pair_offset(c.B));
            return conv_forward(a, c.st, nullptr, &f);
        }
        case CG_PARTS:
            DDK_TRY(run_conv_parts(c, cw, src0, c0, src1, c1, raw, H, W, N));
            return groupnorm_mish_parts(raw, gnp, k.np, g, b, temb, c.u.temb_total, addend, out, c.B, H * W, N, GROUPS, GN_EPS, c.st, c.temb_rows);
        case CG_SLABS: {
            AddendSlabs sl;
            DDK_TRY(run_conv_slabs(c, DDK_CONV3X3_S1, cw, src0, c0, src1, c1, raw, H, W, N, k.splits, sl));
            return groupnorm_mish_ex(c.W + c.ly.off_splitk, sl.n, sl.stride, sl.bias, g, b, temb, c.u.temb_total, addend, out, c.B, H * W, N,
                                     GROUPS, GN_EPS, nullptr, 0, c.st, c.temb_rows);
        }
        case CG_PLAIN:
            DDK_TRY(run_conv(c, DDK_CONV3X3_S1, cw, src0, c0, src1, c1, nullptr, raw, H, W, N));
            break;
    }
    return groupnorm_mish(raw, g, b, temb, c.u.temb_total, addend, out, c.B, H * W, N, GROUPS, GN_EPS, gnp, c.ly.gn_ws * sizeof(float), c.st,
                          c.temb_rows);
}

static bool res_takes_slab_source(const ddk_unet& u, const ResW& r, int B, int H, int W, int c0) {
    return !u.generic && !r.has_res && conv_gn_is_local(u, r.c1, B, H, W, c0, 0, r.co) && conv_gn_is_local(u, r.c2, B, H, W, r.co, 0, r.co);
}

static int run_res(Ctx& c, const ResW& r, const float* src0, int c0, const float* src1, int c1, float* out, int H, int W,
                   const AddendSlabs& ss = AddendSlabs()) {
    float* raw = c.W + c.ly.off_raw;
    float* a1 = c.W + c.ly.off_a1;
    float* res = c.W + c.ly.off_res;
    const float* addend = src0;
    AddendSlabs as;
    if (ss.n > 1) {
        if (r.has_res || src1) return fail_arg("run_res: slab source with a skip conv or a second source");
        as = ss;
    }
    if (r.has_res) {
        const int rs = conv_splits(DDK_CONV1X1, c.B, H, W, c0 + c1, r.co);
        if (rs > 1 && !conv1x1_sm_ok((long long)c.B * H * W, c0, c1, r.co) && conv_gn_is_local(c.u, r.c1, c.B, H, W, c0, c1, r.co) &&
            conv_gn_is_local(c.u, r.c2, c.B, H, W, r.co, 0, r.co)) {
            DDK_TRY(run_conv_slabs(c, DDK_CONV1X1, r.res, src0, c0, src1, c1, res, H, W, r.co, rs, as));
            addend = c.W + c.ly.off_splitk;
        } else {
            DDK_TRY(run_conv(c, DDK_CONV1X1, r.res, src0, c0, src1, c1, nullptr, res, H, W, r.co));
            addend = res;
        }
    }
    DDK_TRY(run_conv_gn(c, r.c1, src0, c0, src1, c1, raw, r.n1, c.temb + r.temb_off, nullptr, a1, H, W, r.co, AddendSlabs(), ss));
    return run_conv_gn(c, r.c2, a1, r.co, nullptr, 0, raw, r.n2, nullptr, addend, out, H, W, r.co, as);
}

static bool attn_fold_eligible(const ddk_unet& u, const AttnW& a, int B, int H, int W) {
    const long long M = (long long)B * H * W;
    return u.attn_fold && H * W > u.attn_fold_min_hw && (H * W) % 64 == 0 && attn_fold_ok(a.c, HEADS) && conv1x1_ws_ok(M, a.c, a.c) &&
           conv_ln_fold_ok(B, H, W, a.c, 2 * HIDDEN) && B <= 256;
}

static int run_attn(Ctx& c, const AttnW& a, const float* x, float* out, int H, int W) {
    float* xn = c.W + c.ly.off_xn;
    float* qkv = c.W + c.ly.off_qkv;
    float* ctx = c.W + c.ly.off_ctx;
    float* o = c.W + c.ly.off_o;
    const long long M = (long long)c.B * H * W;
    if (!c.u.generic && H * W <= 16 && a.c % 32 == 0 && linattn_small_qkv_ok(H * W, a.c)) {
        DDK_TRY(linattn_small_qkv(x, c.P + a.qkv_op, c.P + a.ln_c1, c.P + a.ln_c2, LN_EPS, ctx, o, c.B, H * W, a.c, HEADS, c.st));
        return run_conv(c, DDK_CONV1X1, a.out, o, HIDDEN, nullptr, 0, x, out, H, W, a.c);
    }
    if (!c.u.generic && attn_fold_eligible(c.u, a, c.B, H, W)) {
        if (c.u.attn_kvctx && attn_kvctx_ok(c.B, H * W, a.c, HEADS) && c.ly.splitk * sizeof(float) >= attn_kvctx_workspace_bytes(c.B, H * W)) {
            DDK_TRY(attn_kvctx(x, c.P + a.qkv_lnw + (size_t)HIDDEN * a.c, c.P + a.ln_c1 + HIDDEN, c.P + a.ln_c2 + HIDDEN, LN_EPS, ctx, c.B, H * W,
                               c.W + c.ly.off_splitk, c.ly.splitk * sizeof(float), c.st));
        } else {
            const ConvLnFold lnkv{c.P + a.ln_c1 + HIDDEN, c.P + a.ln_c2 + HIDDEN, LN_EPS};
            DDK_TRY(run_conv(c, DDK_CONV1X1, a.qkv, x, a.c, nullptr, 0, nullptr, qkv, H, W, 2 * HIDDEN, c.P + a.qkv_lnw + (size_t)HIDDEN * a.c,
                             &lnkv));
            DDK_TRY(linattn_context(qkv, ctx, c.B, H * W, HEADS, c.W + c.ly.off_splitk, c.ly.splitk * sizeof(float), c.st, true));
        }
        float* A = o;
        float* a1 = A + (size_t)c.B * a.c * a.c;
        float* a2 = a1 + (size_t)c.B * a.c;
        DDK_TRY(attn_fold(ctx, c.P + a.qkv_lnw, c.P + a.ln_c1, c.P + a.ln_c2, c.P + a.out.w, a.out.has_bias ? c.P + a.out.b : nullptr, A, a1,
                          a2, c.B, a.c, HEADS, c.st));
        const ConvLnFold lnA{a1, a2, LN_EPS};
        return conv1x1_ws(x, A, nullptr, x, out, M, a.c, &lnA, c.st, c.B);
    }
    if (!c.u.generic && conv_ln_fold_ok(c.B, H, W, a.c, 3 * HIDDEN)) {
        const ConvLnFold ln{c.P + a.ln_c1, c.P + a.ln_c2, LN_EPS};
        DDK_TRY(run_conv(c, DDK_CONV1X1, a.qkv, x, a.c, nullptr, 0, nullptr, qkv, H, W, 3 * HIDDEN, c.P + a.qkv_lnw, &ln));
    } else {
        DDK_TRY(c.u.generic ? chan_layernorm_generic(x, c.P + a.ln.g, c.P + a.ln.b, xn, M, a.c, a.c_real, LN_EPS, c.st)
                            : chan_layernorm(x, c.P + a.ln.g, c.P + a.ln.b, xn, M, a.c, LN_EPS, c.st));
        DDK_TRY(run_conv(c, DDK_CONV1X1, a.qkv, xn, a.c, nullptr, 0, nullptr, qkv, H, W, 3 * HIDDEN));
    }
    if (H * W <= 256) {
        DDK_TRY(linattn_fused_small(qkv, ctx, o, c.B, H * W, HEADS, c.st));
    } else {
        DDK_TRY(linattn_context(qkv, ctx, c.B, H * W, HEADS, c.W + c.ly.off_splitk, c.ly.splitk * sizeof(float), c.st));
        DDK_TRY(linattn_apply(qkv, ctx, o, c.B, H * W, HEADS, c.st));
    }
    return run_conv(c, DDK_CONV1X1, a.out, o, HIDDEN, nullptr, 0, x, out, H, W, a.c);
}

static bool level_chain_use(const Ctx& c, int H0, int W0, int bit) {
    return c.allow_cluster && (c.u.level_chain & bit) && c.B <= c.u.level_chain_max_batch && c.ly.chain > 0 &&
           (bit == 1 ? level_chain_shape_ok(c.u, H0, W0) : level8_chain_shape_ok(c.u, H0, W0)) && level_chain_device_ok();
}

static int run_level_chain(Ctx& c, int part, const float* in, float* skip, float* out, const float* down_src = nullptr, float* up_out = nullptr) {
    const ddk_unet& u = c.u;
    const int hw = part == 0 ? 16 : 64;
    const bool wino = hw == 64;
    ChainParams p{};
    int n = 0, e = 0;
    const size_t per = (size_t)c.B * hw * 256;
    auto buf = [&](int i) { return c.W + c.ly.off_chain + (size_t)i * per; };
    auto conv3 = [&](const ConvW& cw, const NormW& nw, const float* s0, int c0, const float* s1, int c1, int temb_off, int flags, float* o) {
        ChainOp& op = p.op[n++];
        op = ChainOp{s0, s1, c.P + (wino ? cw.wwl : cw.wl), c.P + cw.b, c.P + nw.g, c.P + nw.b, o, c0, c1, CH_CONV3, flags, temb_off, 256};
    };
    auto conv1 = [&](const ConvW& cw, const float* s0, int c0, const float* s1, int c1, int flags, float* o) {
        ChainOp& op = p.op[n++];
        op = ChainOp{s0, s1, c.P + cw.wl1, c.P + cw.b, nullptr, nullptr, o, c0, c1, CH_CONV1, flags, -1, 256};
    };
    auto attn = [&](const AttnW& a, const float* s0, float* o) {
        ChainOp& op = p.op[n++];
        op = ChainOp{s0, nullptr, c.P + a.qkv_op, nullptr, c.P + a.ln_c1, c.P + a.ln_c2, o, a.c, 0, CH_ATTN, CHF_WAIT | CHF_SIGNAL, -1, HIDDEN};
    };
    const int WS = CHF_WAIT | CHF_SIGNAL, RES = CHF_ADD_KEEP | CHF_SAVE_KEEP;
    auto res_plain = [&](const ResW& r, const float* x, bool external, float* o) {
        float* h = buf(e++);
        conv3(r.c1, r.n1, x, 256, nullptr, 0, r.temb_off, external ? (CHF_SIGNAL | CHF_KEEP_FROM_SRC) : WS, h);
        conv3(r.c2, r.n2, h, 256, nullptr, 0, -1, WS | RES, o);
    };
    auto attn_block = [&](const AttnW& a, const float* x, float* o, bool signals) {
        float* heads = buf(e++);
        attn(a, x, heads);
        conv1(a.out, heads, HIDDEN, nullptr, 0, (signals ? WS : CHF_WAIT) | RES, o);
    };
    auto res_cat = [&](const ResW& r, const float* x, bool x_external, const float* sk, float* o) {
        conv1(r.res, x, 256, sk, 256, (x_external ? 0 : CHF_WAIT) | CHF_SAVE_KEEP2 | CHF_NO_OUT, nullptr);
        float* h = buf(e++);
        conv3(r.c1, r.n1, x, 256, sk, 256, r.temb_off, CHF_SIGNAL, h);
        conv3(r.c2, r.n2, h, 256, nullptr, 0, -1, WS | CHF_ADD_KEEP2 | CHF_SAVE_KEEP, o);
    };
    if (part == 0) {
        const int sh = u.L - 1;
        if (down_src) {
            const ConvW& dc = u.down_conv[sh - 1];
            float* dn = buf(e++);
            ChainOp& op = p.op[n++];
            op = ChainOp{down_src, nullptr, c.P + dc.wl, c.P + dc.b, nullptr, nullptr, dn, 256, 0, CH_CONV3,
                         CHF_DOWN | CHF_NO_GN | CHF_SIGNAL | CHF_SAVE_KEEP, -1, 256};
            in = dn;
        }
        float* d0 = buf(e++);
        res_plain(u.down_res[2 * sh], in, down_src == nullptr, d0);
        float* d1 = buf(e++);
        res_plain(u.down_res[2 * sh + 1], d0, false, d1);
        attn_block(u.down_attn[sh], d1, skip, true);
        float* m1 = buf(e++);
        res_plain(u.mid1, skip, false, m1);
        float* ma = buf(e++);
        attn_block(u.mid_attn, m1, ma, true);
        float* m2 = buf(e++);
        res_plain(u.mid2, ma, false, m2);
        float* u0 = buf(e++);
        res_cat(u.up_res[0], m2, false, skip, u0);
        float* u1 = buf(e++);
        res_plain(u.up_res[1], u0, false, u1);
        if (up_out) {
            float* ua = buf(e++);
            attn_block(u.up_attn[0], u1, ua, true);
            const ConvW& uc = u.up_conv[0];
            ChainOp& op = p.op[n++];
            op = ChainOp{ua, nullptr, c.P + uc.wtl, c.P + uc.b, nullptr, nullptr, up_out, 256, 0, CH_UPT, CHF_WAIT, -1, 256};
        } else {
            attn_block(u.up_attn[0], u1, out, false);
        }
    } else if (part == 1) {
        const int sh = u.L - 2;
        float* d0 = buf(e++);
        res_plain(u.down_res[2 * sh], in, true, d0);
        float* d1 = buf(e++);
        res_plain(u.down_res[2 * sh + 1], d0, false, d1);
        attn_block(u.down_attn[sh], d1, skip, false);
    } else {
        float* u0 = buf(e++);
        res_cat(u.up_res[2], in, true, skip, u0);
        float* u1 = buf(e++);
        res_plain(u.up_res[3], u0, false, u1);
        attn_block(u.up_attn[1], u1, out, false);
    }
    if (n > CH_MAX_OPS || e > (part == 0 ? CHAIN_BUFS : CHAIN8_BUFS)) return fail_arg("level_chain: internal op / buffer count");
    p.n_ops = n;
    p.B = c.B;
    p.hw = hw;
    p.temb = c.temb;
    p.temb_rows = c.temb_rows;
    p.temb_stride = u.temb_total;
    float* cl = c.W + c.ly.off_cl;
    p.cnt = reinterpret_cast<unsigned*>(cl + cl_chain_offset(c.B));
    p.done = p.cnt + (size_t)c.B * 32;
    p.fail = cl_words(cl, c.B).fail;
    p.gn_eps = GN_EPS;
    p.ln_eps = LN_EPS;
    return level_chain_launch(p, c.st);
}

struct StepArgs {
    int64_t* state;
    float* eps_hat;
    long long per;
    StepRule rule;
};

static bool restore_kind(StepKind k) {
    return k == StepKind::Restore || k == StepKind::RestoreMasked || k == StepKind::RestoreMultistep || k == StepKind::RestoreNoisy ||
           k == StepKind::RestoreGray;
}
static int fused_tail_parts(const ddk_unet& u, int B, int H, int W, int cin, StepKind kind, int restore_n = 0) {
    const int chan = u.generic ? pad32(u.cfg.chan) : u.cfg.chan, n_out = u.cfg.in_ch;
    const int npf = u.final_conv.has_wu ? conv_wino_stats_parts(B, H, W, cin, chan, GROUPS) : 0;
    if (npf <= 0 || (restore_kind(kind) && !u.restore_fused)) return 0;
    return final_tail_ok(H * W, chan, GROUPS, n_out, npf, kind, W, restore_n) ? npf : 0;
}

__global__ __launch_bounds__(256) void step_prepare_kernel(const float* __restrict__ x, float* __restrict__ xpad, long long total,
                                                           int C, int c_pad, int64_t* __restrict__ counter,
                                                           int64_t* __restrict__ t_cur, int B) {
    if (blockIdx.x == 0) {
        const int64_t v = *counter;
        for (int b = threadIdx.x; b < B; b += blockDim.x) t_cur[b] = v;
        __syncthreads();
        if (threadIdx.x == 0) *counter = v - 1;
    }
    for (long long i = blockIdx.x * 256LL + threadIdx.x; i < total; i += (long long)gridDim.x * 256) {
        const int ch = (int)(i % c_pad);
// ... 857 lines not shown
```

downsampled-diffusion_amd/ddk/lib.py:

```python
import ctypes as C
import os

import torch

_HERE = os.path.dirname(os.path.abspath(__file__))
LIB_PATH = os.environ.get("DDK_LIB", os.path.join(os.path.dirname(_HERE), "csrc", "libddk.so"))


class DDKError(RuntimeError):
    pass


ABI_VERSION = 400
ERR_CLUSTER = -4


class ConvArgs(C.Structure):
    _fields_ = [
        ("kind", C.c_int), ("src0", C.c_void_p), ("src1", C.c_void_p), ("c0", C.c_int), ("c1", C.c_int),
        ("weight", C.c_void_p), ("bias", C.c_void_p), ("resid", C.c_void_p), ("out", C.c_void_p),
        ("B", C.c_int), ("H", C.c_int), ("W", C.c_int), ("N", C.c_int), ("pre_mish", C.c_int), ("post_mish", C.c_int), ("defer_reduce", C.c_int),
        ("workspace", C.c_void_p), ("workspace_bytes", C.c_size_t), ("weight_wino", C.c_void_p),
        ("gn_partials", C.c_void_p), ("gn_groups", C.c_int), ("mish_out", C.c_void_p), ("dmish_src", C.c_void_p),
    ]


class UnetConfig(C.Structure):
    _fields_ = [("in_ch", C.c_int), ("chan", C.c_int), ("n_levels", C.c_int), ("mults", C.c_int * 8)]


class SamplerArgs(C.Structure):
    _fields_ = [
        ("unet", C.c_void_p), ("packed", C.c_void_p), ("x", C.c_void_p), ("noise", C.c_void_p),
        ("c_recip", C.c_void_p), ("c_recipm1", C.c_void_p), ("c1", C.c_void_p), ("c2", C.c_void_p),
        ("sigma", C.c_void_p), ("B", C.c_int), ("H", C.c_int), ("W", C.c_int), ("t_start", C.c_int),
        ("t_end", C.c_int), ("seed", C.c_uint64), ("stream_id", C.c_uint32), ("use_graph", C.c_int),
        ("workspace", C.c_void_p), ("workspace_bytes", C.c_size_t),
    ]


class InpaintArgs(C.Structure):
    _fields_ = [
        ("timestep_map", C.POINTER(C.c_int64)), ("known", C.c_void_p), ("mask", C.c_void_p), ("ka", C.c_void_p), ("kb", C.c_void_p),
        ("ja", C.c_void_p), ("jb", C.c_void_p),
    ]


class VlbSweepArgs(C.Structure):
    _fields_ = [
        ("unet", C.c_void_p), ("packed", C.c_void_p), ("x", C.c_void_p), ("noise", C.c_void_p),
        ("sqrt_acp", C.c_void_p), ("sqrt_1m_acp", C.c_void_p), ("c_recip", C.c_void_p), ("c_recipm1", C.c_void_p),
        ("c1", C.c_void_p), ("c2", C.c_void_p), ("post_logvar", C.c_void_p), ("B", C.c_int), ("H", C.c_int), ("W", C.c_int),
        ("T", C.c_int), ("seed", C.c_uint64), ("stream_id", C.c_uint32), ("use_graph", C.c_int),
        ("workspace", C.c_void_p), ("workspace_bytes", C.c_size_t), ("vlb_t", C.c_void_p), ("l_simple_t", C.c_void_p),
    ]


class WgradReduceJob(C.Structure):
    _fields_ = [("slab", C.c_void_p), ("grad", C.c_void_p), ("bias_slab", C.c_void_p), ("grad_b", C.c_void_p), ("slab_stride", C.c_longlong),
                ("block0", C.c_longlong), ("splits", C.c_int), ("N", C.c_int), ("ntaps", C.c_int), ("cx", C.c_int), ("c_real", C.c_int),
                ("cw", C.c_int), ("c_off", C.c_int), ("reserved", C.c_int)]


class RowsSumJob(C.Structure):
    _fields_ = [("rows", C.c_void_p), ("out", C.c_void_p * 4), ("batch_stride", C.c_longlong), ("row_stride", C.c_longlong),
                ("block0", C.c_longlong), ("nbatch", C.c_int), ("nrows", C.c_int), ("n", C.c_int), ("reserved", C.c_int)]


class PackJob(C.Structure):
    _fields_ = [("src", C.c_void_p), ("dst", C.c_void_p), ("total", C.c_longlong), ("block0", C.c_longlong), ("kind", C.c_int),
                ("p", C.c_int * 7)]


_P, _I, _LL, _F, _SZ = C.c_void_p, C.c_int, C.c_longlong, C.c_float, C.c_size_t

GRAY_WEIGHTS = {"mean": 1, "luma": 2}

SIGNATURES = {
    "ddk_version": (_I, []),
    "ddk_last_error": (C.c_char_p, []),
    "ddk_device_ok": (_I, []),
    "ddk_nchw_to_nhwc": (_I, [_P, _P, _I, _I, _I, _I, _I, _P]),
    "ddk_nhwc_to_nchw": (_I, [_P, _P, _I, _I, _I, _I, _I, _P]),
    "ddk_pad_channels": (_I, [_P, _P, _LL, _I, _I, _P]),
    "ddk_pack_conv_weight": (_I, [_P, _P, _I, _I, _I, _I, _I, _P]),
    "ddk_pack_convT_weight": (_I, [_P, _P, _I, _I, _P]),
    "ddk_pack_conv_weight_split": (_I, [_P, _P, _I, _I, _I, _I, _I, _I, _I, _P]),
    "ddk_pack_convT_weight_padded": (_I, [_P, _P, _I, _I, _I, _P]),
    "ddk_pack_linear_T": (_I, [_P, _P, _I, _I, _I, _I, _P]),
    "ddk_pack_conv_weight_wino": (_I, [_P, _P, _I, _I, _I, _P]),
    "ddk_pack_conv_weight_wino_dgrad": (_I, [_P, _P, _I, _I, _I, _I, _I, _P]),
    "ddk_conv_wino_splits": (_I, [_I, _I, _I, _I, _I]),
    "ddk_pack_convT_weight_wino": (_I, [_P, _P, _I, _I, _I, _P]),
    "ddk_convT_wino_splits": (_I, [_I, _I, _I, _I, _I]),
    "ddk_conv_gn_partials": (_I, [_I, _I, _I, _I, _I, _I]),
    "ddk_groupnorm_mish_partials": (_I, [_P, _P, _I, _P, _P, _P, _I, _P, _P, _I, _I, _I, _I, _F, _P]),
    "ddk_pack_conv_weight_first": (_I, [_P, _P, _I, _I, _P]),
    "ddk_conv_first_ok": (_I, [_I, _I, _I, _I, _I]),
    "ddk_conv_first": (_I, [_P, _P, _P, _P, _P, _I, _I, _I, _I, _I, _I, _P]),
    "ddk_conv1x1_ws_ok": (_I, [C.c_longlong, _I, _I]),
    "ddk_conv1x1_ws": (_I, [_P, _P, _P, _P, _P, C.c_longlong, _I, _P, _P, _F, _P]),
    "ddk_conv1x1_ws_images": (_I, [_P, _P, _P, _P, _P, C.c_longlong, _I, _P, _P, _F, _I, _P]),
    "ddk_linattn_context_kv": (_I, [_P, _P, _I, _I, _I, _P, _SZ, _P]),
    "ddk_attention_fold": (_I, [_P, _P, _P, _P, _P, _P, _P, _P, _P, _I, _I, _I, _P]),
    "ddk_groupnorm_mish_partials_res1x1": (_I, [_P, _P, _I, _P, _P, _P, _I, _P, _P, _P, _I, _P, _I, _I, _I, _I, _F, _P]),
    "ddk_final_tail": (_I, [_P, _P, _I, _P, _P, _F, _P, _P, _I, _P, _P, _P, _P, _P, _P, _P, _P, _P, C.c_uint64, C.c_uint32, _I, _I, _I, _I, _P]),
    "ddk_pack_conv_weight_local": (_I, [_P, _P, _I, _I, _I, _P]),
    "ddk_pack_conv1x1_weight_local": (_I, [_P, _P, _I, _I, _I, _P]),
    "ddk_pack_convT_weight_local": (_I, [_P, _P, _I, _I, _P]),
    "ddk_pack_conv_weight_wino_local": (_I, [_P, _P, _I, _I, _I, _P]),
    "ddk_conv3x3_gn_mish_wino_ok": (_I, [_I, _I, _I, _I, _I, _I]),
    "ddk_conv3x3_gn_mish_wino": (_I, [_P, _I, _P, _I, _P, _P, _P, _P, _P, _I, _P, _P, _I, _I, _I, _I, _I, _F, _P]),
    "ddk_conv3x3_gn_mish_slabs": (_I, [_P, _I, _LL, _P, _I, _P, _P, _P, _P, _P, _I, _P, _I, _LL, _P, _P, _I, _I, _I, _I, _I, _F, _P]),
    "ddk_attention_kv_context_workspace_bytes": (_SZ, [_I, _I]),
    "ddk_attention_kv_context_ok": (_I, [_I, _I, _I, _I]),
    "ddk_attention_kv_context": (_I, [_P, _P, _P, _P, _F, _P, _I, _I, _P, _SZ, _P]),
    "ddk_pack_qkv_operand": (_I, [_P, _P, _I, _I, _P]),
    "ddk_linattn_small_from_x": (_I, [_P, _P, _P, _P, _F, _P, _P, _I, _I, _I, _I, _P]),
    "ddk_conv3x3_gn_mish_ok": (_I, [_I, _I, _I, _I, _I, _I]),
    "ddk_conv3x3_gn_mish": (_I, [_P, _I, _P, _I, _P, _P, _P, _P, _P, _I, _P, _P, _I, _I, _I, _I, _I, _F, _P]),
    "ddk_conv_workspace_bytes": (_SZ, [_I, _I, _I, _I, _I, _I]),
    "ddk_conv_splits": (_I, [_I, _I, _I, _I, _I, _I]),
    "ddk_conv_forward": (_I, [C.POINTER(ConvArgs), _P]),
    "ddk_debug_read_stamps": (_I, [_P]),
    "ddk_groupnorm_mish": (_I, [_P, _P, _P, _P, _I, _P, _P, _I, _I, _I, _I, _F, _P, _SZ, _P]),
    "ddk_groupnorm_workspace_bytes": (_SZ, [_I, _I, _I, _I]),
    "ddk_groupnorm_mish_slabs": (_I, [_P, _I, _LL, _P, _P, _P, _P, _I, _P, _P, _I, _I, _I, _I, _F, _P]),
    "ddk_chan_layernorm": (_I, [_P, _P, _P, _P, _LL, _I, _F, _P]),
    "ddk_mish": (_I, [_P, _P, _LL, _P]),
    "ddk_tanh": (_I, [_P, _P, _LL, _P]),
    "ddk_avgpool2": (_I, [_P, _P, _I, _I, _I, _I, _P]),
    "ddk_upsample_nearest2": (_I, [_P, _P, _I, _I, _I, _I, _P]),
    "ddk_add": (_I, [_P, _P, _P, _LL, _P]),
    "ddk_linattn_context_workspace_bytes": (_SZ, [_I, _I, _I]),
    "ddk_linattn_context": (_I, [_P, _P, _I, _I, _I, _P, _SZ, _P]),
    "ddk_linattn_apply": (_I, [_P, _P, _P, _I, _I, _I, _P]),
    "ddk_linattn_fused_small": (_I, [_P, _P, _P, _I, _I, _I, _P]),
    "ddk_time_mlp": (_I, [_P, _P, _P, _P, _P, _P, _P, _P, _I, _I, _P]),
    "ddk_time_proj": (_I, [_P, _P, _P, _P, _I, _I, _I, _P]),
    "ddk_conv1x1_small_n": (_I, [_P, _P, _P, _P, _LL, _I, _I, _P]),
    "ddk_q_sample": (_I, [_P, _P, _P, _P, _P, _P, _I, _LL, _P]),
    "ddk_p_sample_update": (_I, [_P, _P, _P, _P, _P, _P, _P, _P, _P, _I, _LL, C.c_uint64, C.c_uint32, _P]),
    "ddk_p_sample_update_multistep": (_I, [_P, _P, _P, _P, _P, _P, _P, _P, _P, _I, _LL, _P]),
    "ddk_p_sample_update_inpaint": (_I, [_P] * 14 + [_I, _LL, C.c_uint64, C.c_uint32, _P]),
    "ddk_p_sample_update_restore": (_I, [_P, _P, _P, _I] + [_P] * 6 + [_I, _I, _I, _I, C.c_uint64, C.c_uint32, _P]),
    "ddk_p_sample_update_restore_masked": (_I, [_P, _P, _P, _P, _I] + [_P] * 6 + [_I, _I, _I, _I, C.c_uint64, C.c_uint32, _P]),
    "ddk_p_sample_update_restore_multistep": (_I, [_P, _P, _P, _P, _P, _I] + [_P] * 6 + [_I, _I, _I, _I, _P]),
    "ddk_p_sample_update_restore_noisy": (_I, [_P, _P, _P, _P, _I] + [_P] * 8 + [_I, _I, _I, _I, C.c_uint64, C.c_uint32, _P]),
    "ddk_p_sample_update_restore_gray": (_I, [_P, _P, _P, _P, _I, _I] + [_P] * 8 + [_I, _I, _I, _I, C.c_uint64, C.c_uint32, _P]),
    "ddk_randn": (_I, [_P, _LL, C.c_uint64, C.c_uint32, C.c_uint32, _P]),
    "ddk_fix_samples": (_I, [_P, _P, _I, _I, _I, _I, _P]),
    "ddk_sq_err_sum": (_I, [_P, _P, _P, _I, _LL, _P]),
    "ddk_vlb_terms_workspace_bytes": (_SZ, [_I, _LL]),
    "ddk_vlb_terms": (_I, [_P, _P, _P, _P, _P, _P, _P, _P, _P, _P, _P, _P, _I, _LL, _P, _SZ, _P]),
    "ddk_image_metrics_workspace_bytes": (_SZ, [_I, _I, _I, _I]),
    "ddk_image_metrics": (_I, [_P, _P, _P, _I, _I, _I, _I, _P, _P, _P, _SZ, _P]),
    "ddk_unet_create": (_P, [C.POINTER(UnetConfig)]),
    "ddk_unet_destroy": (None, [_P]),
    "ddk_unet_num_slots": (_I, [_P]),
    "ddk_unet_slot_name": (C.c_char_p, [_P, _I]),
    "ddk_unet_slot_numel": (_LL, [_P, _I]),
    "ddk_unet_packed_bytes": (_SZ, [_P]),
    "ddk_unet_pack_slot": (_I, [_P, _I, _P, _P, _P]),
    "ddk_unet_finalize_pack": (_I, [_P, _P, _P]),
    "ddk_unet_workspace_bytes": (_SZ, [_P, _I, _I, _I]),
    "ddk_unet_forward": (_I, [_P, _P, _P, _P, _P, _I, _I, _I, _P, _SZ, _P]),
    "ddk_conv3x3_gn_mish_cluster_ok": (_I, [_I, _I, _I, _I, _I, _I]),
    "ddk_conv3x3_gn_mish_cluster_workspace_bytes": (_SZ, [_I, _I, _I, _I]),
    "ddk_conv3x3_gn_mish_cluster_split_workspace_bytes": (_SZ, [_I, _I, _I, _I, _I, _I]),
    "ddk_conv3x3_gn_mish_cluster": (_I, [_P, _I, _P, _I, _P, _P, _P, _P, _P, _I, _P, _P, _I, _I, _I, _I, _I, _F, _P, _SZ, _P]),
    "ddk_unet_set_option": (_I, [_P, _I, _I]),
    "ddk_debug_cluster_timeouts": (C.c_uint, []),
    "ddk_conv3x3_gn_mish_cluster_check": (_I, [_P, _I, _P]),
    "ddk_unet_cluster_check": (_I, [_P, _P, _I, _I, _I, _P]),
    "ddk_debug_occupy": (_I, [_I, _I, _I, _P]),
    "ddk_debug_clock_probe": (_I, [_P, _I, _P]),
    "ddk_unet_flops": (C.c_double, [_P, _I, _I, _I]),
    "ddk_unet_flops_executed": (C.c_double, [_P, _I, _I, _I]),
    "ddk_sampler_workspace_bytes": (_SZ, [_P, _I, _I, _I, _I]),
    "ddk_sampler_run": (_I, [C.POINTER(SamplerArgs), _P]),
    "ddk_sampler_run_spaced": (_I, [C.POINTER(SamplerArgs), C.POINTER(C.c_int64), _P]),
    "ddk_sampler_multistep_workspace_bytes": (_SZ, [_P, _I, _I, _I, _I]),
    "ddk_sampler_run_multistep": (_I, [C.POINTER(SamplerArgs), C.POINTER(C.c_int64), _P, _P]),
    "ddk_sampler_inpaint_workspace_bytes": (_SZ, [_P, _I, _I, _I, _I]),
    "ddk_sampler_run_inpaint": (_I, [C.POINTER(SamplerArgs), C.POINTER(InpaintArgs), _P]),
    "ddk_sampler_restore_workspace_bytes": (_SZ, [_P, _I, _I, _I, _I]),
    "ddk_sampler_restore_tail_parts": (_I, [_P, _I, _I, _I, _I]),
    "ddk_sampler_run_restore": (_I, [C.POINTER(SamplerArgs), C.POINTER(C.c_int64), _P, _I, _P]),
    "ddk_sampler_restore_masked_workspace_bytes": (_SZ, [_P, _I, _I, _I, _I, _I]),
    "ddk_sampler_restore_masked_tail_parts": (_I, [_P, _I, _I, _I, _I]),
    "ddk_sampler_run_restore_masked": (_I, [C.POINTER(SamplerArgs), C.POINTER(C.c_int64), _P, _P, _I, _P]),
    "ddk_sampler_restore_multistep_workspace_bytes": (_SZ, [_P, _I, _I, _I, _I, _I]),
    "ddk_sampler_restore_multistep_tail_parts": (_I, [_P, _I, _I, _I, _I]),
    "ddk_sampler_run_restore_multistep": (_I, [C.POINTER(SamplerArgs), C.POINTER(C.c_int64), _P, _P, _P, _I, _P]),
    "ddk_sampler_restore_noisy_workspace_bytes": (_SZ, [_P, _I, _I, _I, _I, _I]),
    "ddk_sampler_restore_noisy_tail_parts": (_I, [_P, _I, _I, _I, _I]),
    "ddk_sampler_run_restore_noisy": (_I, [C.POINTER(SamplerArgs), C.POINTER(C.c_int64), _P, _P, _P, _P, _I, _P]),
    "ddk_sampler_restore_gray_workspace_bytes": (_SZ, [_P, _I, _I, _I, _I, _I]),
    "ddk_sampler_restore_gray_tail_parts": (_I, [_P, _I, _I, _I, _I]),
    "ddk_sampler_run_restore_gray": (_I, [C.POINTER(SamplerArgs), C.POINTER(C.c_int64), _P, _P, _P, _P, _I, _I, _P]),
    "ddk_sampler_invalidate": (_I, [_P]),
    "ddk_sampler_release_workspace": (_I, [_P, _P]),
    "ddk_vlb_sweep_workspace_bytes": (_SZ, [_P, _I, _I, _I, _I]),
    "ddk_vlb_sweep_run": (_I, [C.POINTER(VlbSweepArgs), _P]),
    "ddk_pack_conv_weight_dgrad": (_I, [_P, _P, _I, _I, _I, _I, _I, _I, _P]),
    "ddk_zero_stuff2": (_I, [_P, _P, _I, _I, _I, _I, _I, _I, _P]),
    "ddk_conv_wgrad_workspace_bytes": (_SZ, [_I, _I, _I, _I, _I, _I]),
    "ddk_conv_wgrad": (_I, [_I, _P, _P, _P, _I, _I, _I, _I, _I, _I, _I, _I, _P, _SZ, _P]),
    "ddk_conv_wgrad_bias": (_I, [_I, _P, _P, _P, _P, _I, _I, _I, _I, _I, _I, _I, _I, _P, _SZ, _P]),
    "ddk_bias_grad": (_I, [_P, _P, _LL, _I, _I, _P, _SZ, _P]),
    "ddk_groupnorm_train_workspace_bytes": (_SZ, [_I, _I, _I, _I]),
    "ddk_dropout_epoch": (_I, [C.c_uint64, _I, _P]),
    "ddk_groupnorm_mish_train_fwd": (_I, [_P, _P, _P, _P, _I, _P, _F, C.c_uint64, C.c_uint32, _P, _I, _I, _I, _I, _F, _P, _SZ, _P]),
    "ddk_groupnorm_mish_bwd": (_I, [_P, _P, _P, _F, C.c_uint64, C.c_uint32, _P, _P, _P, _I, _I, _I, _I, _F, _P, _SZ, _P]),
    "ddk_groupnorm_mish_train_fwd_slabs": (_I, [_P, _I, _LL, _P, _P, _P, _P, _P, _I, _P, _F, C.c_uint64, C.c_uint32, _P, _I, _I, _I, _I,
                                                _F, _P]),
    "ddk_groupnorm_mish_bwd_slabs": (_I, [_P, _P, _P, _F, C.c_uint64, C.c_uint32, _P, _I, _LL, _P, _P, _I, _I, _I, _I, _F, _P]),
    "ddk_rows_sum": (_I, [_P, _I, _LL, _P, _I, _I, _P]),
    "ddk_rows_sum_batched": (_I, [_P, _I, _LL, _I, _LL, _P, _I, _I, _P]),
    "ddk_rows_sum_targets": (_I, [_P, _I, _LL, _I, _LL, _P, _P, _P, _P, _I, _I, _P]),
    "ddk_multi_add": (_I, [_P, _P, _I, _LL, _P]),
    "ddk_conv_wgrad_defer": (_I, [_I, _P, _P, _P, _P, _I, _I, _I, _I, _I, _I, _I, _I, _P, _SZ, _P, _P]),
    "ddk_wgrad_reduce_jobs": (_I, [_P, _I, _P]),
    "ddk_rows_sum_jobs": (_I, [_P, _I, _P]),
    "ddk_pack_jobs_layout": (_LL, [_P, _I]),
    "ddk_pack_jobs": (_I, [_P, _I, _LL, _P]),
    "ddk_chan_layernorm_bwd": (_I, [_P, _P, _P, _P, _P, _I, C.POINTER(C.c_int), _LL, _I, _F, _P]),
    "ddk_chan_layernorm_bwd_add": (_I, [_P, _P, _P, _P, _P, _P, _I, C.POINTER(C.c_int), _LL, _I, _F, _P]),
    "ddk_groupnorm_mish_generic_train_fwd": (_I, [_P, _P, _P, _P, _I, _P, _F, C.c_uint64, C.c_uint32, _P, _I, _I, _I, _I, _I, _F, _P]),
    "ddk_groupnorm_mish_generic_bwd": (_I, [_P, _P, _P, _F, C.c_uint64, C.c_uint32, _P, _P, _P, _I, _I, _I, _I, _I, _F, _P]),
    "ddk_chan_layernorm_generic": (_I, [_P, _P, _P, _P, _LL, _I, _I, _F, _P]),
    "ddk_chan_layernorm_generic_bwd": (_I, [_P, _P, _P, _P, _P, _P, _I, C.POINTER(C.c_int), _LL, _I, _I, _F, _P]),
    "ddk_linattn_train_workspace_bytes": (_SZ, [_I, _I, _I]),
    "ddk_linattn_stats": (_I, [_P, _P, _I, _I, _I, _P, _SZ, _P]),
    "ddk_linattn_bwd": (_I, [_P, _P, _P, _P, _P, _P, _I, _I, _I, _P, _SZ, _P]),
    "ddk_linattn_bwd_recompute": (_I, [_P, _P, _P, _P, _P, _P, _I, _I, _I, _P, _SZ, _P]),
    "ddk_mish_bwd": (_I, [_P, _P, _P, _LL, _P]),
    "ddk_tanh_bwd": (_I, [_P, _P, _P, _LL, _P]),
    "ddk_avgpool2_bwd": (_I, [_P, _P, _I, _I, _I, _I, _P]),
    "ddk_upsample_nearest2_bwd": (_I, [_P, _P, _I, _I, _I, _I, _P]),
    "ddk_sq_err_grad": (_I, [_P, _P, _P, _P, _I, _LL, _P]),
    "ddk_ae_objective": (_I, [_P, _P, _P, _I, _I, _P, _P]),
    "ddk_ae_objective_bwd": (_I, [_P, _P, _I, _I, _P, _P, _P]),
    "ddk_scale_per_sample": (_I, [_P, _P, _P, _I, _LL, _P]),
    "ddk_conv1x1_small_n_bwd": (_I, [_P, _P, _P, _P, _P, _I, C.POINTER(C.c_int), _LL, _I, _I, _P]),
    "ddk_small_gemm_workspace_bytes": (_SZ, [_I, _I, _I, _I]),
    "ddk_small_gemm": (_I, [_I, _P, _P, _P, _I, _I, _I, _I, _I, _I, _I, _P, _SZ, _P]),
    "ddk_sincos_embed": (_I, [_P, _P, _P, _I, _I, _P]),
    "ddk_bias_act": (_I, [_P, _P, _P, _LL, _I, _P]),
    "ddk_grad_norm_clip": (_I, [_P, _LL, _F, _P, _P, _SZ, _P]),
    "ddk_adam_step": (_I, [_P, _P, _P, _P, _LL, C.c_double, C.c_double, C.c_double, C.c_double, _I, _P, _P]),
    "ddk_ema_update": (_I, [_P, _P, _LL, _F, _P]),
}

_lib = None


def load():
    global _lib
    if _lib is not None:
        return _lib
    if not os.path.exists(LIB_PATH):
        raise DDKError(
            f"HIP kernel library not found at {LIB_PATH}. Build it with `make -C {os.path.dirname(LIB_PATH)}` "
            "(or `python -c 'import __graft_entry__ as g; g.build()'`). There is no CPU fallback.")
    lib = C.CDLL(LIB_PATH)
    for name, (res, args) in SIGNATURES.items():
        fn = getattr(lib, name)
        fn.restype = res
# ... 30 lines not shown
```

downsampled-diffusion_amd/ddk/ops.py:

```python
import ctypes as C

import torch

from . import lib as L

CONV3X3_S1, CONV3X3_S2, CONV1X1, CONVT4X4_S2 = 0, 1, 2, 3
GN_GROUPS, GN_EPS, LN_EPS = 8, 1e-5, 1e-5


def pad32(c):
    return (c + 31) // 32 * 32


class _PackEntry:
    __slots__ = ("wref", "out", "job", "fresh", "pooled")


_pack_cache = {}
_weights_epoch = [0]
_pack_table = {}
pack_stats = {"single": 0, "batched_launches": 0, "batched_jobs": 0}
_graph_tables = []
_graph_keep = [_graph_tables]

# ... 997 lines not shown
    stride = temb.stride(0) if temb is not None else 0
    lib = L.load()
    if slabs is not None:
        L.check(lib.ddk_groupnorm_mish_train_fwd_slabs(L.ptr(slabs), slabs.shape[0], slabs.stride(0), L.ptr(conv_bias), L.ptr(x), L.ptr(gamma),
                                                       L.ptr(beta), temb.data_ptr() if temb is not None else None, stride, L.ptr(addend),
                                                       float(drop_p), seed, layer, L.ptr(out), b, h * w, c, groups, eps, L.stream()),
                "groupnorm_mish_train_fwd_slabs")
        return out
    nbytes = lib.ddk_groupnorm_train_workspace_bytes(b, h * w, c, groups)
    ws = _ws(x.device, nbytes, "gn_train") if nbytes else None
    L.check(lib.ddk_groupnorm_mish_train_fwd(L.ptr(_f32(x)), L.ptr(gamma), L.ptr(beta),
                                             temb.data_ptr() if temb is not None else None, stride, L.ptr(addend),
                                             float(drop_p), seed, layer, L.ptr(out), b, h * w, c, groups, eps, L.ptr(ws), nbytes,
                                             L.stream()),
            "groupnorm_mish_train_fwd")
    return out


def groupnorm_mish_bwd(x, gamma, beta, dy, drop_p=0.0, seed=0, layer=0, groups=GN_GROUPS, eps=GN_EPS, acc=None, dy_slabs=None):
    b, h, w, c = x.shape
    dx = torch.empty_like(x)
    part = torch.empty((4, b, c), device=x.device, dtype=torch.float32)
    lib = L.load()
    if dy_slabs is not None:
        L.check(lib.ddk_groupnorm_mish_bwd_slabs(L.ptr(_f32(x)), L.ptr(gamma), L.ptr(beta), float(drop_p), seed, layer, L.ptr(dy_slabs),
                                                 dy_slabs.shape[0], dy_slabs.stride(0), L.ptr(dx), L.ptr(part), b, h * w, c, groups, eps,
                                                 L.stream()), "groupnorm_mish_bwd_slabs")
    else:
        nbytes = lib.ddk_groupnorm_train_workspace_bytes(b, h * w, c, groups)
        ws = _ws(x.device, nbytes, "gn_train") if nbytes else None
        L.check(lib.ddk_groupnorm_mish_bwd(L.ptr(_f32(x)), L.ptr(gamma), L.ptr(beta), float(drop_p), seed, layer, L.ptr(_f32(dy)),
                                           L.ptr(dx), L.ptr(part), b, h * w, c, groups, eps, L.ptr(ws), nbytes, L.stream()),
                "groupnorm_mish_bwd")
    sums = [None, None, None]
    missing = [k for k in range(3) if acc is None or acc[k] is None]
    if acc is not None and any(t is not None for t in acc):
        _rows_sum_targets(part[1], 3, b * c, b, c, [acc[0], acc[1], acc[2]], c)
    if missing:
        out = torch.empty((3, c), device=x.device, dtype=torch.float32)
        L.check(lib.ddk_rows_sum_batched(L.ptr(part[1]), 3, b * c, b, c, L.ptr(out), c, 0, L.stream()), "rows_sum_batched")
        for k in missing:
            sums[k] = out[k]
    return dx, part[0], sums


def groupnorm_mish_generic_train(x, gamma, beta, temb=None, addend=None, drop_p=0.0, seed=0, layer=0, groups=GN_GROUPS, eps=GN_EPS):
    b, h, w, cp = x.shape
    c = gamma.numel()
    out = torch.empty_like(x)
    stride = temb.stride(0) if temb is not None else 0
    L.check(L.load().ddk_groupnorm_mish_generic_train_fwd(L.ptr(_f32(x)), L.ptr(gamma), L.ptr(beta), temb.data_ptr() if temb is not None else None,
                                                          stride, L.ptr(addend), float(drop_p), seed, layer, L.ptr(out), b, h * w, cp, c, groups,
                                                          eps, L.stream()), "groupnorm_mish_generic_train_fwd")
    return out


def groupnorm_mish_generic_bwd(x, gamma, beta, dy, drop_p=0.0, seed=0, layer=0, groups=GN_GROUPS, eps=GN_EPS):
    b, h, w, cp = x.shape
    c = gamma.numel()
    dx = torch.empty_like(x)
    part = torch.empty((4, b, c), device=x.device, dtype=torch.float32)
    lib = L.load()
    L.check(lib.ddk_groupnorm_mish_generic_bwd(L.ptr(_f32(x)), L.ptr(gamma), L.ptr(beta), float(drop_p), seed, layer, L.ptr(_f32(dy)), L.ptr(dx),
                                               L.ptr(part), b, h * w, cp, c, groups, eps, L.stream()), "groupnorm_mish_generic_bwd")
    sums = torch.empty((3, c), device=x.device, dtype=torch.float32)
    L.check(lib.ddk_rows_sum_batched(L.ptr(part[1]), 3, b * c, b, c, L.ptr(sums), c, 0, L.stream()), "rows_sum_batched")
    return dx, part[0], sums


def chan_layernorm_generic(x, g, b, eps=LN_EPS):
    cp, c = x.shape[-1], g.numel()
    out = torch.empty_like(x)
    L.check(L.load().ddk_chan_layernorm_generic(L.ptr(_f32(x)), L.ptr(g.reshape(-1)), L.ptr(b.reshape(-1)), L.ptr(out), x.numel() // cp, cp, c,
                                                eps, L.stream()), "chan_layernorm_generic")
    return out


def chan_layernorm_generic_bwd(x, g, dy, eps=LN_EPS, addend=None):
    cp, c = x.shape[-1], g.numel()
    m = x.numel() // cp
    dx = torch.empty_like(x)
    max_parts = 512
    part = torch.empty((2, max_parts, c), device=x.device, dtype=torch.float32)
    n = C.c_int(0)
    lib = L.load()
    L.check(lib.ddk_chan_layernorm_generic_bwd(L.ptr(_f32(x)), L.ptr(g.reshape(-1)), L.ptr(_f32(dy)), L.ptr(addend), L.ptr(dx), L.ptr(part),
                                               max_parts, C.byref(n), m, cp, c, eps, L.stream()), "chan_layernorm_generic_bwd")
    flat = part.view(-1)
    dg = rows_sum(flat[:n.value * c], n.value, c, c)
    db = rows_sum(flat[n.value * c:2 * n.value * c], n.value, c, c)
    return dx, dg, db


def rows_sum(rows, nrows, row_stride, n, out=None):
    if out is None:
        out = torch.empty(n, device=rows.device, dtype=torch.float32)
    L.check(L.load().ddk_rows_sum(rows.data_ptr(), nrows, row_stride, out.data_ptr(), n, 0, L.stream()), "rows_sum")
    return out


_multi_add_tables = {}


def multi_add_(src, segments):
    key = (str(src.device),) + tuple((int(o), d.data_ptr(), d.numel()) for o, d in segments)
    tab = _multi_add_tables.get(key)
    if tab is None:
        if len(_multi_add_tables) > 64:
            _multi_add_tables.clear()
        host = torch.tensor([[int(o), d.data_ptr(), d.numel()] for o, d in segments], dtype=torch.int64)
        tab = _multi_add_tables[key] = host.to(src.device)
    if torch.cuda.is_current_stream_capturing():
        _graph_keep[-1].append((tab, [d for _, d in segments]))
    L.check(L.load().ddk_multi_add(L.ptr(src), tab.data_ptr(), len(segments), max(d.numel() for _, d in segments), L.stream()), "multi_add")


def chan_layernorm_bwd(x, g, dy, eps=LN_EPS, acc=None, addend=None):
    c = x.shape[-1]
    m = x.numel() // c
    dx = torch.empty_like(x)
    max_parts = 512
    part = torch.empty((2, max_parts, c), device=x.device, dtype=torch.float32)
    n = C.c_int(0)
    lib = L.load()
    L.check(lib.ddk_chan_layernorm_bwd_add(L.ptr(_f32(x)), L.ptr(g.reshape(-1)), L.ptr(_f32(dy)), L.ptr(addend), L.ptr(dx), L.ptr(part),
                                           max_parts, C.byref(n), m, c, eps, L.stream()), "chan_layernorm_bwd")
    if acc is not None and acc[0] is not None and acc[1] is not None:
        _rows_sum_targets(part, 2, n.value * c, n.value, c, [acc[0], acc[1]], c)
        return dx, None, None
    out = torch.empty((2, c), device=x.device, dtype=torch.float32)
    L.check(lib.ddk_rows_sum_batched(L.ptr(part), 2, n.value * c, n.value, c, L.ptr(out), c, 0, L.stream()), "rows_sum_batched")
    return dx, out[0], out[1]


def linattn_small_from_x(x, w_qkv, ln_g, ln_b, heads=4, eps=LN_EPS):
    b, h, w, c = x.shape
    wq = w_qkv.reshape(w_qkv.shape[0], -1).to(torch.float32)
    g, bb = ln_g.reshape(-1).to(torch.float32), ln_b.reshape(-1).to(torch.float32)
    cp = pad32(c)
    lnw = torch.zeros((wq.shape[0], cp), device=x.device, dtype=torch.float32)
    lnw[:, :c] = wq * g[None, :]
    c1 = (wq * g[None, :]).sum(dim=1).contiguous()
    c2 = (wq * bb[None, :]).sum(dim=1).contiguous()
    wop = torch.empty_like(lnw)
    lib = L.load()
    L.check(lib.ddk_pack_qkv_operand(L.ptr(lnw), L.ptr(wop), heads, cp, L.stream()), "pack_qkv_operand")
    ctx = torch.empty((b, heads, 32, 32), device=x.device, dtype=torch.float32)
    out = torch.empty((b, h, w, heads * 32), device=x.device, dtype=torch.float32)
    L.check(lib.ddk_linattn_small_from_x(L.ptr(_f32(x)), L.ptr(wop), L.ptr(c1), L.ptr(c2), eps, L.ptr(ctx), L.ptr(out), b, h * w, c, heads,
                                         L.stream()), "linattn_small_from_x")
    return out, ctx


def linattn_train(qkv, heads=4):
    out, ctx = linattn(qkv, heads)
    b, h, w, _ = qkv.shape
    stats = torch.empty((b, heads, 2, 32), device=qkv.device, dtype=torch.float32)
    lib = L.load()
    nbytes = lib.ddk_linattn_train_workspace_bytes(b, h * w, heads)
    ws = _ws(qkv.device, nbytes, "linattn_train") if nbytes else None
    L.check(lib.ddk_linattn_stats(L.ptr(qkv), L.ptr(stats), b, h * w, heads, L.ptr(ws), nbytes, L.stream()), "linattn_stats")
    return out, ctx, stats


def linattn_bwd(qkv, dout, ctx, stats, heads=4):
    b, h, w, _ = qkv.shape
    dctx = torch.empty_like(ctx)
    dqkv = torch.empty_like(qkv)
    lib = L.load()
    nbytes = lib.ddk_linattn_train_workspace_bytes(b, h * w, heads)
    ws = _ws(qkv.device, nbytes, "linattn_train") if nbytes else None
    if stats is None:
        scratch = torch.empty((b, heads, 2, 32), device=qkv.device, dtype=torch.float32)
        L.check(lib.ddk_linattn_bwd_recompute(L.ptr(qkv), L.ptr(_f32(dout)), L.ptr(ctx), L.ptr(scratch), L.ptr(dctx), L.ptr(dqkv), b, h * w,
                                              heads, L.ptr(ws), nbytes, L.stream()), "linattn_bwd_recompute")
        return dqkv
    L.check(lib.ddk_linattn_bwd(L.ptr(qkv), L.ptr(_f32(dout)), L.ptr(ctx), L.ptr(stats), L.ptr(dctx), L.ptr(dqkv), b, h * w,
                                heads, L.ptr(ws), nbytes, L.stream()), "linattn_bwd")
    return dqkv


def ae_objective(l_ddpm, l_rec, t, t_rec_max):
    out = torch.empty(3, device=l_ddpm.device, dtype=torch.float32)
    L.check(L.load().ddk_ae_objective(L.ptr(_f32(l_ddpm)), L.ptr(_f32(l_rec)), t.data_ptr(), int(t_rec_max), l_ddpm.numel(), L.ptr(out),
                                      L.stream()), "ae_objective")
    return out


def ae_objective_bwd(g, t, t_rec_max):
    d1 = torch.empty(t.numel(), device=g.device, dtype=torch.float32)
    d2 = torch.empty_like(d1)
    L.check(L.load().ddk_ae_objective_bwd(L.ptr(_f32(g)), t.data_ptr(), int(t_rec_max), t.numel(), L.ptr(d1), L.ptr(d2), L.stream()),
            "ae_objective_bwd")
    return d1, d2


def mish_bwd(x, dy):
    dx = torch.empty_like(x)
    L.check(L.load().ddk_mish_bwd(L.ptr(_f32(x)), L.ptr(_f32(dy)), L.ptr(dx), x.numel(), L.stream()), "mish_bwd")
    return dx


def tanh_bwd(y, dy):
    dx = torch.empty_like(y)
    L.check(L.load().ddk_tanh_bwd(L.ptr(_f32(y)), L.ptr(_f32(dy)), L.ptr(dx), y.numel(), L.stream()), "tanh_bwd")
    return dx


def avgpool2_bwd(dy):
    b, h2, w2, c = dy.shape
    dx = torch.empty((b, 2 * h2, 2 * w2, c), device=dy.device, dtype=torch.float32)
    L.check(L.load().ddk_avgpool2_bwd(L.ptr(_f32(dy)), L.ptr(dx), b, 2 * h2, 2 * w2, c, L.stream()), "avgpool2_bwd")
    return dx


def upsample_nearest2_bwd(dy):
    b, h2, w2, c = dy.shape
    dx = torch.empty((b, h2 // 2, w2 // 2, c), device=dy.device, dtype=torch.float32)
    L.check(L.load().ddk_upsample_nearest2_bwd(L.ptr(_f32(dy)), L.ptr(dx), b, h2 // 2, w2 // 2, c, L.stream()), "upsample_nearest2_bwd")
    return dx


def sq_err_grad(a, b, scale):
    out = torch.empty_like(b)
    bsz = a.shape[0]
    L.check(L.load().ddk_sq_err_grad(L.ptr(_f32(a)), L.ptr(_f32(b)), L.ptr(_f32(scale)), L.ptr(out), bsz, a.numel() // bsz, L.stream()),
            "sq_err_grad")
    return out


def scale_per_sample(x, scale):
    out = torch.empty_like(x)
    bsz = x.shape[0]
    L.check(L.load().ddk_scale_per_sample(L.ptr(_f32(x)), L.ptr(_f32(scale)), L.ptr(out), bsz, x.numel() // bsz, L.stream()),
            "scale_per_sample")
    return out


def conv1x1_small_n_bwd(a, w, dy, acc=None):
    c = a.shape[-1]
    n_out = w.shape[0]
    m = a.numel() // c
    da = torch.empty_like(a)
    max_rows = 1024
    rowlen = n_out * c + n_out
    part = torch.empty((max_rows, rowlen), device=a.device, dtype=torch.float32)
    n = C.c_int(0)
    L.check(L.load().ddk_conv1x1_small_n_bwd(L.ptr(_f32(a)), L.ptr(w.reshape(n_out, c).contiguous()), L.ptr(_f32(dy)), L.ptr(da),
                                             L.ptr(part), max_rows, C.byref(n), m, c, n_out, L.stream()), "conv1x1_small_n_bwd")
    if acc is not None and acc[0] is not None and acc[1] is not None:
        flat = part.view(-1)
        _rows_sum_targets(flat, 1, 0, n.value, rowlen, [acc[0]], n_out * c)
        _rows_sum_targets(flat[n_out * c:], 1, 0, n.value, rowlen, [acc[1]], n_out)
        return da, None, None
    tot = rows_sum(part, n.value, rowlen, rowlen)
    return da, tot[:n_out * c].reshape(n_out, c), tot[n_out * c:]


def small_gemm(mode, a, b, out, m, n, k, lda, ldb, ldc, accumulate=False):
    lib = L.load()
    nbytes = lib.ddk_small_gemm_workspace_bytes(m, n, k, ldc)
    ws = _ws(out.device, nbytes, "small_gemm") if nbytes else None
    L.check(lib.ddk_small_gemm(mode, a.data_ptr(), b.data_ptr(), out.data_ptr(), m, n, k, lda, ldb, ldc, int(accumulate), L.ptr(ws), nbytes,
                               L.stream()), "small_gemm")
    return out


def sincos_embed(t, freqs):
    bsz, dim = t.shape[0], freqs.numel() * 2
    e = torch.empty((bsz, dim), device=t.device, dtype=torch.float32)
    L.check(L.load().ddk_sincos_embed(L.ptr(t), L.ptr(freqs), L.ptr(e), bsz, dim, L.stream()), "sincos_embed")
    return e


def bias_act_(y, bias, want_act):
    act = torch.empty_like(y) if want_act else None
    L.check(L.load().ddk_bias_act(L.ptr(y), L.ptr(bias), L.ptr(act), y.shape[0], y.shape[1], L.stream()), "bias_act")
    return act


def grad_norm_clip(flat_grad, max_norm):
    out = torch.empty(2, device=flat_grad.device, dtype=torch.float32)
    ws = _ws(flat_grad.device, 4096, "norm")
    L.check(L.load().ddk_grad_norm_clip(L.ptr(flat_grad), flat_grad.numel(), float(max_norm), L.ptr(out), L.ptr(ws), 4096, L.stream()),
            "grad_norm_clip")
    return out


def adam_step_(p, g, m, v, lr, step, clip=None, betas=(0.9, 0.999), eps=1e-8):
    L.check(L.load().ddk_adam_step(L.ptr(p), L.ptr(g), L.ptr(m), L.ptr(v), p.numel(), float(lr), float(betas[0]), float(betas[1]),
                                   float(eps), int(step), L.ptr(clip), L.stream()), "adam_step")


def ema_update_(p_ema, p, decay):
    L.check(L.load().ddk_ema_update(L.ptr(p_ema), L.ptr(p), p.numel(), float(decay), L.stream()), "ema_update")
```

downsampled-diffusion_amd/ddk/plan.py:

```python
import contextlib
import ctypes as C
import math
import warnings

import torch

from . import lib as L


def sinusoidal_freqs(dim):
    half = dim // 2
    step = math.log(10000) / (half - 1)
    return torch.exp(torch.arange(half) * -step)


SAMPLERS = {"smp": ("sample", "sampler", "sampler"), "sms": ("sample_multistep", "sampler_multistep", "multistep sampler"),
            "sin": ("sample_inpaint", "sampler_inpaint", "inpainting sampler"),
            "srs": ("sample_restore", "sampler_restore", "super-resolution sampler"),
            "srm": ("sample_restore_masked", "sampler_restore_masked", "masked restoration sampler"),
            "srx": ("sample_restore_multistep", "sampler_restore_multistep", "restoration solver"),
            "srn": ("sample_restore_noisy", "sampler_restore_noisy", "noisy restoration sampler"),
            "srg": ("sample_restore_gray", "sampler_restore_gray", "colourisation sampler")}
CHAIN_WORKSPACES = (*SAMPLERS, "vsw")


class UnetPlan:
    def __init__(self, in_ch, chan, mults):
        lib = L.load()
        cfg = L.UnetConfig(in_ch, chan, len(mults), (C.c_int * 8)(*list(mults) + [0] * (8 - len(mults))))
        self._lib = lib
        self.handle = lib.ddk_unet_create(C.byref(cfg))
        if not self.handle:
            raise L.DDKError(f"ddk_unet_create failed: {L.last_error()}")
        self.in_ch, self.chan, self.mults = in_ch, chan, tuple(mults)
        self.slot_names = [lib.ddk_unet_slot_name(self.handle, i).decode() for i in range(lib.ddk_unet_num_slots(self.handle))]
        self.slot_numel = [lib.ddk_unet_slot_numel(self.handle, i) for i in range(len(self.slot_names))]
        self.packed = None
        self._ws = {}
        self._state = {}
        self._cluster = 1
        self._cluster_dev = None

    def __deepcopy__(self, memo):
        return None

    def __del__(self):
        try:
            if getattr(self, "handle", None):
                self._lib.ddk_unet_destroy(self.handle)
                self.handle = None
        except Exception:
            pass

    def pack(self, tensors, device):
        lib = self._lib
        nbytes = lib.ddk_unet_packed_bytes(self.handle)
        packed = torch.zeros(nbytes // 4, device=device, dtype=torch.float32)
        keep = []
        for i, name in enumerate(self.slot_names):
            if name == "@sinusoidal_freqs":
                src = sinusoidal_freqs(self.chan)
            else:
                if name not in tensors:
                    raise L.DDKError(f"UNet weight '{name}' missing from the state dict")
                src = tensors[name]
            src = src.detach().to(device=device, dtype=torch.float32).contiguous()
            if src.numel() != self.slot_numel[i]:
                raise L.DDKError(f"UNet weight '{name}': expected {self.slot_numel[i]} elements, got {src.numel()}")
            keep.append(src)
            L.check(lib.ddk_unet_pack_slot(self.handle, i, L.ptr(src), L.ptr(packed), L.stream()), f"pack {name}")
        torch.cuda.current_stream().synchronize()
        self.packed = packed
        return packed

    def _workspace(self, kind, nbytes, device):
        key = (kind, nbytes, str(device))
        hit = self._ws.get(key)
        if hit is not None:
            self._ws[key] = self._ws.pop(key)
            return hit
        if kind in CHAIN_WORKSPACES:
            mine = [k for k in self._ws if k[0] == kind]
            if len(mine) >= 3:
                old = self._ws[mine[0]]
                L.check(self._lib.ddk_sampler_release_workspace(self.handle, L.ptr(old)), "sampler_release_workspace")
                del self._ws[mine[0]]
        else:
            for k in [k for k in self._ws if k[0] == kind]:
                del self._ws[k]
        buf = torch.empty(max(nbytes, 16) // 4 + 4, device=device, dtype=torch.float32)
        self._ws[key] = buf
        return buf

    OPT_CLUSTER_GROUPNORM = 1
    OPT_ATTENTION_FOLD = 3
    OPT_FOLD_DOWNSAMPLE_REDUCE = 5
    OPT_ATTENTION_KV_CONTEXT = 6
    OPT_LEVEL_CHAIN = 7
    OPT_FIRST_GROUPNORM = 8
    OPT_RESTORE_FUSED_TAIL = 12

    def set_option(self, option, value):
        L.check(self._lib.ddk_unet_set_option(self.handle, option, int(value)), "unet_set_option")
        if option == self.OPT_CLUSTER_GROUPNORM:
            self._cluster = max(0, min(2, int(value)))

    @contextlib.contextmanager
    def forwards_as_in_chain(self):
        raised = self._cluster == 1
        if raised:
            self.set_option(self.OPT_CLUSTER_GROUPNORM, 2)
        try:
            yield
        finally:
            if raised and self._cluster == 2:
                self.set_option(self.OPT_CLUSTER_GROUPNORM, 1)

    def _cluster_failed(self, ws, b, h, w, stream_ptr):
        rc = self._lib.ddk_unet_cluster_check(self.handle, L.ptr(ws), b, h, w, stream_ptr)
        if rc == 0:
            return False
        if rc != L.ERR_CLUSTER:
            L.check(rc, "unet_cluster_check")
        warnings.warn("ddk: " + L.last_error() + " -- switching DDK_OPT_CLUSTER_GROUPNORM off for this plan and rerunning",
                      RuntimeWarning, stacklevel=3)
        self.set_option(self.OPT_CLUSTER_GROUPNORM, 0)
        return True

    def _chain_guarded(self):
        if self._cluster_dev is None:
            self._cluster_dev = self._lib.ddk_conv3x3_gn_mish_cluster_ok(32, 32, 32, 128, 128, 8) > 0
        return self._cluster >= 1 and self._cluster_dev

    def _run_chain(self, who, call, ws, b, h, w, graphed, restore=None):
        guard = self._chain_guarded()
        for rerun in (False, True):
            if rerun and restore is not None:
                restore()
            if graphed:
                cur = torch.cuda.current_stream()
                side = _side_stream(ws.device)
                side.wait_stream(cur)
                with torch.cuda.stream(side):
                    call(side.cuda_stream)
                    failed = guard and self._cluster >= 1 and self._cluster_failed(ws, b, h, w, side.cuda_stream)
                cur.wait_stream(side)
            else:
                call(L.stream())
                failed = guard and self._cluster >= 1 and self._cluster_failed(ws, b, h, w, L.stream())
            if not failed:
                return
        raise L.DDKError(f"{who}: in-launch GroupNorm reported a failure with the option off")

    def cluster_timeouts(self):
        return int(self._lib.ddk_debug_cluster_timeouts())

    def flops(self, b, h, w):
        return self._lib.ddk_unet_flops(self.handle, b, h, w)

    def flops_executed(self, b, h, w):
        return self._lib.ddk_unet_flops_executed(self.handle, b, h, w)

    def forward_nhwc(self, x, t):
        if self.packed is None:
            raise L.DDKError("UnetPlan.forward before pack()")
        b, h, w, c = x.shape
        if c != self.in_ch:
            raise L.DDKError(f"expected {self.in_ch} input channels, got {c}")
        if t.dtype != torch.int64:
            raise L.DDKError("timesteps must be int64")
        lib = self._lib
        nbytes = lib.ddk_unet_workspace_bytes(self.handle, b, h, w)
        if nbytes == 0:
            raise L.DDKError(f"unet workspace query failed: {L.last_error()}")
        ws = self._workspace("fwd", nbytes, x.device)
        out = torch.empty_like(x)
        for _ in range(2):
            L.check(lib.ddk_unet_forward(self.handle, L.ptr(self.packed), L.ptr(x), L.ptr(t), L.ptr(out), b, h, w,
                                         L.ptr(ws), nbytes, L.stream()), "unet_forward")
            if self._cluster < 2 or not self._cluster_failed(ws, b, h, w, L.stream()):
                break
        return out

    def _need_packed(self, kind):
        if self.packed is None:
            raise L.DDKError(f"UnetPlan.{SAMPLERS[kind][0]} before pack()")

    def _run_sampler(self, kind, x, t_start, t_end, bytes_query, call, use_graph):
        _, who, label = SAMPLERS[kind]
        b, h, w, _ = x.shape
        nbytes = bytes_query(b, h, w)
        if nbytes == 0:
            raise L.DDKError(f"{label} workspace query failed: {L.last_error()}")
        ws = self._workspace(kind, nbytes, x.device)
        caller_x, x = x, self._chain_x(x)
        x_start = x.clone() if self._chain_guarded() else None
        self._run_chain(who, lambda stream_ptr: call(x, ws, nbytes, stream_ptr), ws, b, h, w, use_graph and t_start - t_end + 1 > 1,
                        restore=lambda: x.copy_(x_start))
        if caller_x.data_ptr() != x.data_ptr():
            caller_x.copy_(x)
        return caller_x

    @staticmethod
    def _timestep_map(timesteps, t_start):
        if timesteps is None:
            return None
        if len(timesteps) != t_start + 1:
            raise L.DDKError(f"timestep map must have t_start + 1 = {t_start + 1} entries, got {len(timesteps)}")
        return (C.c_int64 * len(timesteps))(*[int(v) for v in timesteps])

    def _sampler_args(self, x, noise, tables, t_start, t_end, seed, stream_id, use_graph, ws, nbytes):
        b, h, w, _ = x.shape
        return L.SamplerArgs(self.handle, L.ptr(self.packed), L.ptr(x), L.ptr(noise), L.ptr(tables["c_recip"]),
                             L.ptr(tables["c_recipm1"]), L.ptr(tables["c1"]), L.ptr(tables["c2"]), L.ptr(tables.get("sigma")),
                             b, h, w, t_start, t_end, seed, stream_id, int(use_graph), L.ptr(ws), nbytes)

    def sample_nhwc(self, x, tables, t_start, t_end=0, noise=None, seed=0, stream_id=0, use_graph=True, timesteps=None):
        self._need_packed("smp")
        lib = self._lib
        tmap = self._timestep_map(timesteps, t_start)
        n_steps = t_start - t_end + 1
        if noise is not None and tuple(noise.shape) != (n_steps, *x.shape):
            raise L.DDKError(f"injected noise must be {(n_steps, *x.shape)}, got {tuple(noise.shape)}")

        def call(x, ws, nbytes, stream_ptr):
            a = self._sampler_args(x, noise, tables, t_start, t_end, seed, stream_id, use_graph, ws, nbytes)
            if tmap is None:
                L.check(lib.ddk_sampler_run(C.byref(a), stream_ptr), "sampler_run")
            else:
                L.check(lib.ddk_sampler_run_spaced(C.byref(a), tmap, stream_ptr), "sampler_run_spaced")

        return self._run_sampler("smp", x, t_start, t_end,
                                 lambda b, h, w: lib.ddk_sampler_workspace_bytes(self.handle, b, h, w, t_start), call, use_graph)

    def _chain_x(self, x):
        skey = (tuple(x.shape), str(x.device))
        mode = self._state.get(skey)
        if mode is None:
            mode = self._state[skey] = {"ptr": x.data_ptr(), "buf": None}
        if mode["buf"] is None and mode["ptr"] != x.data_ptr():
            mode["buf"] = torch.empty_like(x)
        if mode["buf"] is not None:
            mode["buf"].copy_(x)
            return mode["buf"]
        return x

    def sample_multistep_nhwc(self, x, tables, t_start, t_end=0, stream_id=0, use_graph=True, timesteps=None):
        self._need_packed("sms")
        lib = self._lib
        tmap = self._timestep_map(timesteps, t_start)

        def call(x, ws, nbytes, stream_ptr):
            a = self._sampler_args(x, None, tables, t_start, t_end, 0, stream_id, use_graph, ws, nbytes)
# ... 202 lines not shown
```

include/ddk.h:

```cpp
#ifndef DDK_H
#define DDK_H

#include <stddef.h>
#include <stdint.h>

#ifdef __cplusplus
extern "C" {
#endif

typedef void* ddk_stream_t;

#define DDK_OK 0
#define DDK_ERR_ARG (-1)
#define DDK_ERR_HIP (-2)
#define DDK_ERR_WORKSPACE (-3)
#define DDK_ERR_CLUSTER (-4)

int ddk_version(void);
const char* ddk_last_error(void);
int ddk_device_ok(void);

int ddk_nchw_to_nhwc(const float* src, float* dst, int B, int C, int H, int W, int c_pad, ddk_stream_t s);
int ddk_nhwc_to_nchw(const float* src, float* dst, int B, int C, int H, int W, int c_stride, ddk_stream_t s);
int ddk_pad_channels(const float* src, float* dst, long long M, int C, int c_pad, ddk_stream_t s);
int ddk_pack_conv_weight(const float* w_oihw, float* dst, int O, int I, int KH, int KW, int i_pad, ddk_stream_t s);
int ddk_pack_conv_weight_split(const float* w_oihw, float* dst, int O, int I, int KH, int KW, int i_pad, int split, int split_pad,
                               ddk_stream_t s);
int ddk_pack_convT_weight(const float* w_iohw, float* dst, int I, int O, ddk_stream_t s);
int ddk_pack_convT_weight_padded(const float* w_iohw, float* dst, int I, int O, int c_pad, ddk_stream_t s);
int ddk_pack_linear_T(const float* w_oi, float* dst, int O, int I, int ld, int col0, ddk_stream_t s);

enum ddk_conv_kind {
    DDK_CONV3X3_S1 = 0,
    DDK_CONV3X3_S2 = 1,
    DDK_CONV1X1 = 2,
    DDK_CONVT4X4_S2 = 3,
    DDK_CONV4X4_S2 = 4
};

typedef struct ddk_conv_args {
    int kind;
    const float* src0;
    const float* src1;
    int c0, c1;
    const float* weight;
    const float* bias;
    const float* resid;
    float* out;
    int B, H, W;
    int N;
    int pre_mish;
    int post_mish;
    int defer_reduce;
    void* workspace;
    size_t workspace_bytes;
    const float* weight_wino;
    float* gn_partials;
    int gn_groups;
    float* mish_out;
    const float* dmish_src;
} ddk_conv_args;

int ddk_pack_conv_weight_wino(const float* w_oihw, float* dst, int O, int I, int i_pad, ddk_stream_t s);
int ddk_conv_gn_partials(int B, int H, int W, int cin, int N, int groups);
int ddk_conv_wino_splits(int B, int H, int W, int cin, int N);
size_t ddk_conv_workspace_bytes(int kind, int B, int H, int W, int cin, int N);
int ddk_conv_splits(int kind, int B, int H, int W, int cin, int N);
int ddk_conv_forward(const ddk_conv_args* a, ddk_stream_t s);
int ddk_debug_read_stamps(unsigned long long* host_out);

int ddk_groupnorm_mish(const float* x, const float* gamma, const float* beta, const float* temb,
                       int temb_stride, const float* addend, float* out, int B, int HW, int C, int groups,
                       float eps, void* workspace, size_t workspace_bytes, ddk_stream_t s);
size_t ddk_groupnorm_workspace_bytes(int B, int HW, int C, int groups);
int ddk_groupnorm_mish_slabs(const float* slabs, int nslab, long long slab_stride, const float* conv_bias,
                             const float* gamma, const float* beta, const float* temb, int temb_stride,
                             const float* addend, float* out, int B, int HW, int C, int groups, float eps,
                             ddk_stream_t s);
int ddk_pack_conv_weight_local(const float* w_oihw, float* dst, int O, int I, int i_pad, ddk_stream_t s);
int ddk_pack_conv1x1_weight_local(const float* w_oi, float* dst, int O, int I, int i_pad, ddk_stream_t s);
int ddk_pack_convT_weight_local(const float* w_iohw, float* dst, int I, int O, ddk_stream_t s);
int ddk_conv3x3_gn_mish_ok(int H, int W, int cin, int c0, int N, int groups);
int ddk_conv3x3_gn_mish(const float* src0, int c0, const float* src1, int c1, const float* weight, const float* bias,
                        const float* gamma, const float* beta, const float* temb, int temb_stride, const float* addend,
                        float* out, int B, int H, int W, int N, int groups, float eps, ddk_stream_t s);
int ddk_groupnorm_mish_partials(const float* x, const float* partials, int tiles_per_image, const float* gamma, const float* beta,
                                const float* temb, int temb_stride, const float* addend, float* out, int B, int HW, int C,
                                int groups, float eps, ddk_stream_t s);
int ddk_pack_conv_weight_first(const float* w_oihw, float* dst, int O, int I, ddk_stream_t s);
int ddk_conv_first_ok(int cin, int N, int H, int W, int groups);
int ddk_conv_first(const float* x, const float* w_first, const float* bias, float* out, float* gn_partials, int B, int H, int W,
                   int cin, int N, int groups, ddk_stream_t s);
int ddk_conv1x1_ws_ok(long long M, int K, int N);
int ddk_conv1x1_ws(const float* x, const float* w, const float* bias, const float* resid, float* out, long long M, int N,
                   const float* ln_c1, const float* ln_c2, float ln_eps, ddk_stream_t s);
int ddk_conv1x1_ws_images(const float* x, const float* w, const float* bias, const float* resid, float* out, long long M, int N,
                          const float* ln_c1, const float* ln_c2, float ln_eps, int images, ddk_stream_t s);
int ddk_groupnorm_mish_partials_res1x1(const float* x, const float* partials, int tiles_per_image, const float* gamma, const float* beta,
                                       const float* temb, int temb_stride, const float* res_x, const float* res_w, const float* res_b,
                                       int res_cin, float* out, int B, int HW, int C, int groups, float eps, ddk_stream_t s);
int ddk_pack_conv_weight_wino_local(const float* w_oihw, float* dst, int O, int I, int i_pad, ddk_stream_t s);
int ddk_conv3x3_gn_mish_wino_ok(int H, int W, int cin, int c0, int N, int groups);
int ddk_conv3x3_gn_mish_wino(const float* src0, int c0, const float* src1, int c1, const float* weight, const float* bias,
                             const float* gamma, const float* beta, const float* temb, int temb_stride, const float* addend,
                             float* out, int B, int H, int W, int N, int groups, float eps, ddk_stream_t s);
int ddk_conv3x3_gn_mish_slabs(const float* src, int src_slabs, long long src_stride, const float* src_bias, int c0, const float* weight,
                              const float* bias, const float* gamma, const float* beta, const float* temb, int temb_stride,
                              const float* addend, int addend_slabs, long long addend_stride, const float* addend_bias, float* out, int B,
                              int H, int W, int N, int groups, float eps, ddk_stream_t s);
int ddk_conv3x3_gn_mish_cluster_ok(int B, int H, int W, int cin, int N, int groups);
int ddk_conv3x3_gn_mish_cluster_check(void* workspace, int B, ddk_stream_t s);
size_t ddk_conv3x3_gn_mish_cluster_workspace_bytes(int B, int H, int W, int N);
size_t ddk_conv3x3_gn_mish_cluster_split_workspace_bytes(int B, int H, int W, int cin, int N, int groups);
int ddk_conv3x3_gn_mish_cluster(const float* src0, int c0, const float* src1, int c1, const float* weight_wino, const float* bias,
                                const float* gamma, const float* beta, const float* temb, int temb_stride, const float* addend,
                                float* out, int B, int H, int W, int N, int groups, float eps, void* workspace, size_t workspace_bytes,
                                ddk_stream_t s);
int ddk_chan_layernorm(const float* x, const float* g, const float* b, float* out, long long M, int C,
                       float eps, ddk_stream_t s);
int ddk_mish(const float* x, float* out, long long n, ddk_stream_t s);
int ddk_tanh(const float* x, float* out, long long n, ddk_stream_t s);
int ddk_avgpool2(const float* x, float* out, int B, int H, int W, int C, ddk_stream_t s);
int ddk_upsample_nearest2(const float* x, float* out, int B, int H, int W, int C, ddk_stream_t s);
int ddk_add(const float* a, const float* b, float* out, long long n, ddk_stream_t s);

size_t ddk_linattn_context_workspace_bytes(int B, int HW, int heads);
int ddk_linattn_context(const float* qkv, float* ctx, int B, int HW, int heads, void* workspace, size_t workspace_bytes, ddk_stream_t s);
int ddk_linattn_context_kv(const float* kv, float* ctx, int B, int HW, int heads, void* workspace, size_t workspace_bytes, ddk_stream_t s);
int ddk_attention_fold(const float* ctx, const float* wqg, const float* c1q, const float* c2q, const float* wout, const float* bout, float* A,
                       float* a1, float* a2, int B, int C, int heads, ddk_stream_t s);
size_t ddk_attention_kv_context_workspace_bytes(int B, int HW);
int ddk_attention_kv_context_ok(int B, int HW, int C, int heads);
int ddk_attention_kv_context(const float* x, const float* w_kv, const float* c1, const float* c2, float ln_eps, float* ctx, int B, int HW,
                             void* workspace, size_t workspace_bytes, ddk_stream_t s);
int ddk_linattn_fused_small(const float* qkv, float* ctx, float* out, int B, int HW, int heads, ddk_stream_t s);
int ddk_linattn_apply(const float* qkv, const float* ctx, float* out, int B, int HW, int heads, ddk_stream_t s);
int ddk_pack_qkv_operand(const float* folded_w, float* dst, int heads, int c_pad, ddk_stream_t s);
int ddk_linattn_small_from_x(const float* x, const float* w_operand, const float* c1, const float* c2, float ln_eps, float* ctx,
                             float* out, int B, int HW, int C, int heads, ddk_stream_t s);

int ddk_time_mlp(const int64_t* t, const float* freqs, const float* w1t, const float* b1, const float* w2t,
                 const float* b2, float* act, float* raw, int B, int dim, ddk_stream_t s);
int ddk_time_proj(const float* act, const float* wt, const float* bias, float* out, int B, int dim, int n_out,
                  ddk_stream_t s);

int ddk_conv1x1_small_n(const float* x, const float* w, const float* bias, float* out, long long M, int C,
                        int n_out, ddk_stream_t s);

int ddk_q_sample(const float* x, const float* eps, const int64_t* t, const float* sqrt_acp,
                 const float* sqrt_1m_acp, float* out, int B, long long per, ddk_stream_t s);
int ddk_p_sample_update(float* x, const float* eps_hat, const float* noise, const int64_t* t,
                        const float* c_recip, const float* c_recipm1, const float* c1, const float* c2,
                        const float* sigma, int B, long long per, uint64_t seed, uint32_t stream_id,
                        ddk_stream_t s);
int ddk_p_sample_update_multistep(float* x, const float* eps_hat, float* x0_hist, const int64_t* t, const float* c_recip,
                                  const float* c_recipm1, const float* c1, const float* c2, const float* c3, int B, long long per,
                                  ddk_stream_t s);
int ddk_p_sample_update_inpaint(float* x, const float* eps_hat, const float* known, const float* mask, const int64_t* t,
                                const float* c_recip, const float* c_recipm1, const float* c1, const float* c2, const float* sigma,
                                const float* ka, const float* kb, const float* ja, const float* jb, int B, long long per, uint64_t seed,
                                uint32_t stream_id, ddk_stream_t s);
int ddk_p_sample_update_restore(float* x, const float* eps_hat, const float* y, int n, const int64_t* t, const float* c_recip,
                                const float* c_recipm1, const float* c1, const float* c2, const float* sigma, int B, int H, int W,
                                int channels, uint64_t seed, uint32_t stream_id, ddk_stream_t s);
int ddk_p_sample_update_restore_masked(float* x, const float* eps_hat, const float* y, const float* mask, int n, const int64_t* t,
                                       const float* c_recip, const float* c_recipm1, const float* c1, const float* c2, const float* sigma,
                                       int B, int H, int W, int channels, uint64_t seed, uint32_t stream_id, ddk_stream_t s);
int ddk_p_sample_update_restore_multistep(float* x, const float* eps_hat, float* x0_hist, const float* y, const float* mask, int n,
                                          const int64_t* t, const float* c_recip, const float* c_recipm1, const float* c1, const float* c2,
                                          const float* c3, int B, int H, int W, int channels, ddk_stream_t s);
int ddk_p_sample_update_restore_noisy(float* x, const float* eps_hat, const float* y, const float* mask, int n, const int64_t* t,
                                      const float* c_recip, const float* c_recipm1, const float* c1, const float* c2, const float* sigma,
                                      const float* lam, const float* sgm, int B, int H, int W, int channels, uint64_t seed, uint32_t stream_id,
                                      ddk_stream_t s);
int ddk_p_sample_update_restore_gray(float* x, const float* eps_hat, const float* y, const float* mask, int n, int weights, const int64_t* t,
                                     const float* c_recip, const float* c_recipm1, const float* c1, const float* c2, const float* sigma,
                                     const float* lam, const float* sgm, int B, int H, int W, int channels, uint64_t seed, uint32_t stream_id,
                                     ddk_stream_t s);
int ddk_final_tail(const float* raw, const float* partials, int tiles_per_image, const float* gamma, const float* beta, float eps,
                   const float* w, const float* bias, int n_out, float* eps_out, float* x, const float* noise, const int64_t* t,
                   const float* c_recip, const float* c_recipm1, const float* c1, const float* c2, const float* sigma, uint64_t seed,
                   uint32_t stream_id, int B, int HW, int C, int groups, ddk_stream_t s);
int ddk_randn(float* out, long long n, uint64_t seed, uint32_t step, uint32_t stream_id, ddk_stream_t s);
int ddk_fix_samples(const float* x_nchw, float* out_nhwc, int B, int C, int H, int W, ddk_stream_t s);
size_t ddk_vlb_terms_workspace_bytes(int B, long long per);
int ddk_vlb_terms(const float* x, const float* x_t, const float* eps_hat, const float* eps, const int64_t* t,
                  const float* c_recip, const float* c_recipm1, const float* c1, const float* c2,
                  const float* post_logvar, float* vlb, float* sqerr, int B, long long per, void* workspace,
                  size_t workspace_bytes, ddk_stream_t s);
int ddk_sq_err_sum(const float* a, const float* b, float* per_sample, int B, long long per, ddk_stream_t s);
size_t ddk_image_metrics_workspace_bytes(int N, int H, int W, int C);
int ddk_image_metrics(const uint8_t* a, const uint8_t* b, const uint8_t* mask, int N, int H, int W, int C,
                      unsigned long long* sq_sum_count, float* ssim, void* workspace, size_t workspace_bytes, ddk_stream_t s);

typedef struct ddk_unet_config {
    int in_ch;
    int chan;
    int n_levels;
    int mults[8];
} ddk_unet_config;

typedef struct ddk_unet ddk_unet;

ddk_unet* ddk_unet_create(const ddk_unet_config* cfg);
void ddk_unet_destroy(ddk_unet* u);
int ddk_unet_num_slots(const ddk_unet* u);
const char* ddk_unet_slot_name(const ddk_unet* u, int slot);
long long ddk_unet_slot_numel(const ddk_unet* u, int slot);
size_t ddk_unet_packed_bytes(const ddk_unet* u);
int ddk_unet_pack_slot(const ddk_unet* u, int slot, const float* canonical, void* packed, ddk_stream_t s);
int ddk_unet_finalize_pack(const ddk_unet* u, void* packed, ddk_stream_t s);
size_t ddk_unet_workspace_bytes(const ddk_unet* u, int B, int H, int W);
int ddk_unet_forward(const ddk_unet* u, const void* packed, const float* x, const int64_t* t, float* out,
                     int B, int H, int W, void* workspace, size_t workspace_bytes, ddk_stream_t s);
#define DDK_OPT_CLUSTER_GROUPNORM 1
#define DDK_OPT_ATTENTION_FOLD 3
#define DDK_OPT_FOLD_DOWNSAMPLE_REDUCE 5
#define DDK_OPT_ATTENTION_KV_CONTEXT 6
#define DDK_OPT_LEVEL_CHAIN 7
#define DDK_OPT_FIRST_GROUPNORM 8
#define DDK_OPT_RESTORE_FUSED_TAIL 12
int ddk_unet_set_option(ddk_unet* u, int option, int value);
int ddk_unet_cluster_check(const ddk_unet* u, void* workspace, int B, int H, int W, ddk_stream_t s);
unsigned ddk_debug_cluster_timeouts(void);
int ddk_debug_clock_probe(unsigned long long* out, int workgroups, ddk_stream_t s);
int ddk_debug_occupy(int workgroups, int lds_bytes, int microseconds, ddk_stream_t s);
double ddk_unet_flops(const ddk_unet* u, int B, int H, int W);
double ddk_unet_flops_executed(const ddk_unet* u, int B, int H, int W);

typedef struct ddk_sampler_args {
    const ddk_unet* unet;
    const void* packed;
    float* x;
    const float* noise;
    const float* c_recip;
    const float* c_recipm1;
    const float* c1;
    const float* c2;
    const float* sigma;
    int B, H, W;
    int t_start;
    int t_end;
    uint64_t seed;
    uint32_t stream_id;
    int use_graph;
    void* workspace;
    size_t workspace_bytes;
} ddk_sampler_args;

size_t ddk_sampler_workspace_bytes(const ddk_unet* u, int B, int H, int W, int t_start);
int ddk_sampler_run(const ddk_sampler_args* a, ddk_stream_t s);
int ddk_sampler_run_spaced(const ddk_sampler_args* a, const int64_t* timestep_map, ddk_stream_t s);
size_t ddk_sampler_multistep_workspace_bytes(const ddk_unet* u, int B, int H, int W, int t_start);
int ddk_sampler_run_multistep(const ddk_sampler_args* a, const int64_t* timestep_map, const float* c3, ddk_stream_t s);
typedef struct ddk_inpaint_args {
    const int64_t* timestep_map;
    const float* known;
    const float* mask;
    const float* ka;
    const float* kb;
    const float* ja;
    const float* jb;
} ddk_inpaint_args;
size_t ddk_sampler_inpaint_workspace_bytes(const ddk_unet* u, int B, int H, int W, int n_ops);
int ddk_sampler_run_inpaint(const ddk_sampler_args* a, const ddk_inpaint_args* ip, ddk_stream_t s);
size_t ddk_sampler_restore_workspace_bytes(const ddk_unet* u, int B, int H, int W, int t_start);
int ddk_sampler_restore_tail_parts(const ddk_unet* u, int B, int H, int W, int n);
int ddk_sampler_run_restore(const ddk_sampler_args* a, const int64_t* timestep_map, const float* y, int n, ddk_stream_t s);
size_t ddk_sampler_restore_masked_workspace_bytes(const ddk_unet* u, int B, int H, int W, int t_start, int n);
int ddk_sampler_restore_masked_tail_parts(const ddk_unet* u, int B, int H, int W, int n);
int ddk_sampler_run_restore_masked(const ddk_sampler_args* a, const int64_t* timestep_map, const float* y, const float* mask, int n,
                                   ddk_stream_t s);
size_t ddk_sampler_restore_multistep_workspace_bytes(const ddk_unet* u, int B, int H, int W, int t_start, int n);
int ddk_sampler_restore_multistep_tail_parts(const ddk_unet* u, int B, int H, int W, int n);
int ddk_sampler_run_restore_multistep(const ddk_sampler_args* a, const int64_t* timestep_map, const float* c3, const float* y,
                                      const float* mask, int n, ddk_stream_t s);
size_t ddk_sampler_restore_noisy_workspace_bytes(const ddk_unet* u, int B, int H, int W, int t_start, int n);
int ddk_sampler_restore_noisy_tail_parts(const ddk_unet* u, int B, int H, int W, int n);
int ddk_sampler_run_restore_noisy(const ddk_sampler_args* a, const int64_t* timestep_map, const float* lam, const float* sgm, const float* y,
                                  const float* mask, int n, ddk_stream_t s);
size_t ddk_sampler_restore_gray_workspace_bytes(const ddk_unet* u, int B, int H, int W, int t_start, int n);
int ddk_sampler_restore_gray_tail_parts(const ddk_unet* u, int B, int H, int W, int n);
int ddk_sampler_run_restore_gray(const ddk_sampler_args* a, const int64_t* timestep_map, const float* lam, const float* sgm, const float* y,
                                 const float* mask, int n, int weights, ddk_stream_t s);
int ddk_sampler_invalidate(ddk_unet* u);
int ddk_sampler_release_workspace(ddk_unet* u, const void* workspace);

typedef struct ddk_vlb_sweep_args {
    const ddk_unet* unet;
    const void* packed;
    const float* x;
    const float* noise;
    const float* sqrt_acp;
    const float* sqrt_1m_acp;
    const float* c_recip;
    const float* c_recipm1;
    const float* c1;
    const float* c2;
    const float* post_logvar;
    int B, H, W;
    int T;
    uint64_t seed;
    uint32_t stream_id;
    int use_graph;
    void* workspace;
    size_t workspace_bytes;
    float* vlb_t;
    float* l_simple_t;
} ddk_vlb_sweep_args;

size_t ddk_vlb_sweep_workspace_bytes(const ddk_unet* u, int B, int H, int W, int T);
int ddk_vlb_sweep_run(const ddk_vlb_sweep_args* a, ddk_stream_t s);



int ddk_pack_conv_weight_wino_dgrad(const float* w_oihw, float* dst, int O, int I, int c_lo, int c_hi, int o_pad, ddk_stream_t s);
int ddk_pack_convT_weight_wino(const float* w_iohw, float* dst, int I, int O, int i_pad, ddk_stream_t s);
int ddk_convT_wino_splits(int B, int H, int W, int cin, int N);
int ddk_pack_conv_weight_dgrad(const float* w_oihw, float* dst, int O, int I, int KH, int KW, int i_pad, int o_pad,
                               ddk_stream_t s);
int ddk_zero_stuff2(const float* in, float* out, int B, int H, int W, int Ho, int Wo, int C, ddk_stream_t s);
size_t ddk_conv_wgrad_workspace_bytes(int kind, int B, int H, int W, int cx, int N);
int ddk_conv_wgrad(int kind, const float* x, const float* dy, float* grad_w, int B, int H, int W, int cx, int c_real,
                   int cw, int c_off, int N, void* workspace, size_t workspace_bytes, ddk_stream_t s);
int ddk_conv_wgrad_bias(int kind, const float* x, const float* dy, float* grad_w, float* grad_b, int B, int H, int W, int cx, int c_real,
                        int cw, int c_off, int N, void* workspace, size_t workspace_bytes, ddk_stream_t s);
int ddk_bias_grad(const float* dy, float* grad_b, long long M, int N, int accumulate, void* workspace,
                  size_t workspace_bytes, ddk_stream_t s);
size_t ddk_groupnorm_train_workspace_bytes(int B, int HW, int C, int groups);
int ddk_dropout_epoch(unsigned long long set_to, int bump, ddk_stream_t s);
int ddk_groupnorm_mish_train_fwd(const float* x, const float* gamma, const float* beta, const float* temb,
                                 int temb_stride, const float* addend, float drop_p, uint64_t seed, uint32_t layer,
                                 float* out, int B, int HW, int C, int groups, float eps, void* workspace,
                                 size_t workspace_bytes, ddk_stream_t s);
int ddk_groupnorm_mish_bwd(const float* x, const float* gamma, const float* beta, float drop_p, uint64_t seed,
                           uint32_t layer, const float* dy, float* dx, float* part, int B, int HW, int C, int groups,
                           float eps, void* workspace, size_t workspace_bytes, ddk_stream_t s);
int ddk_groupnorm_mish_train_fwd_slabs(const float* slabs, int nslab, long long slab_stride, const float* conv_bias, float* raw_out,
                                       const float* gamma, const float* beta, const float* temb, int temb_stride,
                                       const float* addend, float drop_p, uint64_t seed, uint32_t layer, float* out, int B, int HW,
                                       int C, int groups, float eps, ddk_stream_t s);
int ddk_groupnorm_mish_bwd_slabs(const float* x, const float* gamma, const float* beta, float drop_p, uint64_t seed, uint32_t layer,
                                 const float* dy_slabs, int nslab, long long slab_stride, float* dx, float* part, int B, int HW,
                                 int C, int groups, float eps, ddk_stream_t s);
int ddk_rows_sum(const float* rows, int nrows, long long row_stride, float* out, int n, int accumulate, ddk_stream_t s);
int ddk_rows_sum_batched(const float* rows, int nbatch, long long batch_stride, int nrows, long long row_stride, float* out,
                         int n, int accumulate, ddk_stream_t s);
int ddk_rows_sum_targets(const float* rows, int nbatch, long long batch_stride, int nrows, long long row_stride, float* out0, float* out1,
                         float* out2, float* out3, int n, int accumulate, ddk_stream_t s);
typedef struct ddk_rows_sum_job {
    const float* rows;
    float* out[4];
    long long batch_stride, row_stride;
    long long block0;
    int nbatch, nrows, n, reserved;
} ddk_rows_sum_job;
int ddk_rows_sum_jobs(const ddk_rows_sum_job* jobs_host, int n, ddk_stream_t s);
int ddk_multi_add(const float* src, const long long* table, int nseg, long long max_count, ddk_stream_t s);
enum {
    DDK_PACK_CONV = 0,
    DDK_PACK_CONVT = 1,
    DDK_PACK_DGRAD = 2,
    DDK_PACK_WINO = 3,
    DDK_PACK_WINO_DGRAD = 4
};
typedef struct ddk_pack_job {
    const float* src;
    float* dst;
    long long total;
    long long block0;
    int kind;
    int p[7];
} ddk_pack_job;
typedef struct ddk_wgrad_reduce_job {
// ... 61 lines not shown
```

Before: 26.09.

## Add split-row fused LN+QKV+linear-attention kernel with cross-workgroup pair exchange

Adds attn_split_kernel. For each (sample, head) it launches two workgroups, each taking half of the spatial rows. Each workgroup computes the LayerNorm-folded QKV projection with MFMA from a DMA ring buffer, then its partial softmax-K context. The two halves swap max, denominator and context partials through global memory using a cluster-style counter wait, and each then applies the merged context to its own Q rows. The goal is to put more CUs to work on the small 8x8 and 16x16 attention layers at low batch and to fuse the projection with the attention. The cost is a cross-workgroup spin-wait that relies on co-residency, with a NaN poison path if the wait times out.

After: 26.53, median of 6. 1.02x the previous value.

```diff
diff --git a/downsampled-diffusion_amd/csrc/attention.hip b/downsampled-diffusion_amd/csrc/attention.hip
--- a/downsampled-diffusion_amd/csrc/attention.hip
+++ b/downsampled-diffusion_amd/csrc/attention.hip
@@ -1,5 +1,6 @@
 #include <cstdlib>
 
+#include "cluster_sync.h"
 #include "conv_common.h"
 
 namespace ddk {
@@ -672,6 +673,311 @@
     linattn_small_core<ROWS>(ks, vs, qs, cs, smax, ctx, out, b, h, HW, heads);
 }
 
+constexpr int AS_REC = 1152;
+constexpr int AS_CNT = 32;
+constexpr int AS_RING = 4;
+
+template <int ROWS>
+struct AttnSplitGeom {
+    static_assert(ROWS == 128 || ROWS == 32, "half of a 16x16 or of an 8x8 map");
+    static constexpr int XP = ROWS / 8;
+    static constexpr int NP = XP + 12;
+    static constexpr int SLOT = (ROWS + 96) * 32;
+    static constexpr int NB = ROWS == 128 ? 3 : 1;
+    static constexpr int UNITS = ROWS == 128 ? 4 : 3;
+    static constexpr int KPART = UNITS * NB * 16 * 64;
+    static constexpr int SCR = KPART > 8 * 32 * 33 ? KPART : 8 * 32 * 33;
+    static constexpr int RING_FL = AS_RING * SLOT;
+    static_assert(SCR + 2 * ROWS * DH + ROWS * (DH + 1) <= RING_FL, "k, v, q of the half live behind the scratch area in the drained ring");
+    static constexpr int TAIL = DH * (DH + 4) + 2 * ROWS + 16 * DH + 16 * DH + DH + 192 + AS_REC + 32;
+    static constexpr int LDS_FL = RING_FL + TAIL;
+};
+
+struct AttnSplitParams {
+    const float* x;
+    const float* w;
+    const float* c1;
+    const float* c2;
+    float eps;
+    float* ctx;
+    float* out;
+    unsigned* cnt;
+    float* rec;
+    unsigned* fail;
+    int C;
+};
+
+__device__ __forceinline__ void wait_vmcnt_le(int n) {
+    if (n >= 8) wait_vmcnt<8>();
+    else if (n >= 6) wait_vmcnt<6>();
+    else if (n >= 4) wait_vmcnt<4>();
+    else if (n >= 3) wait_vmcnt<3>();
+    else if (n >= 2) wait_vmcnt<2>();
+    else wait_vmcnt<0>();
+}
+
+template <int ROWS>
+__global__ __launch_bounds__(512) void attn_split_kernel(const AttnSplitParams p) {
+    using G = AttnSplitGeom<ROWS>;
+    constexpr int HW = 2 * ROWS, HC = 4 * DH;
+    extern __shared__ __attribute__((aligned(16))) float smem[];
+    float* scr = smem;
+    float* ks = smem + G::SCR;
+    float* vs = ks + ROWS * DH;
+    float* qs = vs + ROWS * DH;
+    float* cs = smem + G::RING_FL;
+    float* rowstat = cs + DH * (DH + 4);
+    float* smax = rowstat + 2 * ROWS;
+    float* dpart = smax + 16 * DH;
+    float* mx = dpart + 16 * DH;
+    float* cfold = mx + DH;
+    float* own = cfold + 192;
+    int* gave_up = reinterpret_cast<int*>(own + AS_REC);
+    const int tid = threadIdx.x, lane = tid & 63;
+    const int wid = __builtin_amdgcn_readfirstlane(tid >> 6);
+    const int half = blockIdx.x, h = blockIdx.y, b = blockIdx.z;
+    const int C = p.C, nch = C >> 5;
+    const float* xb = p.x + ((long long)b * HW + half * ROWS) * C;
+    const unsigned lds_base = (unsigned)(size_t)(__attribute__((address_space(3))) float*)smem;
+
+    const int prow = lane >> 3, ppos = lane & 7;
+    const int npw = (G::NP - wid + 7) >> 3;
+    unsigned voff[4];
+#pragma unroll
+    for (int j = 0; j < 4; ++j) {
+        const int pj = wid + 8 * j;
+        const int r = 8 * (pj < G::XP ? pj : pj - G::XP) + prow;
+        const int src = pj < G::XP ? r : (r >> 5) * HC + h * DH + (r & 31);
+        voff[j] = (unsigned)((src * C + ((ppos ^ ((r >> 1) & 7)) << 2)) * 4);
+    }
+    auto issue = [&](int chunk) {
+        const unsigned dst = lds_base + (unsigned)(((chunk & (AS_RING - 1)) * G::SLOT) * 4);
+#pragma unroll
+        for (int j = 0; j < 4; ++j) {
+            const int pj = wid + 8 * j;
+            if (pj < G::NP) lds_dma16_s(pj < G::XP ? xb : p.w, voff[j] + (unsigned)(chunk * 128), dst + (unsigned)(pj * 1024));
+        }
+    };
+    for (int c = 0; c < AS_RING - 1 && c < nch; ++c) issue(c);
+    if (tid < 192) {
+        const int n = tid % 96;
+        const int col = (n >> 5) * HC + h * DH + (n & 31);
+        cfold[tid] = tid < 96 ? p.c1[col] : p.c2[col];
+    }
+    if (tid < 4 * ROWS) {
+        const int row = tid >> 2, sub = tid & 3, n16 = C >> 4;
+        const float4* rp = reinterpret_cast<const float4*>(xb + (long long)row * C);
+        float4 v[16];
+        float s = 0.f;
+#pragma unroll
+        for (int i = 0; i < 16; ++i)
+            if (i < n16) {
+                v[i] = rp[sub + 4 * i];
+                s += (v[i].x + v[i].y) + (v[i].z + v[i].w);
+            }
+        s += __shfl_xor(s, 1, 64);
+        s += __shfl_xor(s, 2, 64);
+        const float inv_c = 1.0f / (float)C;
+        const float mean = s * inv_c;
+        float qq = 0.f;
+#pragma unroll
+        for (int i = 0; i < 16; ++i)
+            if (i < n16) {
+                const float a0 = v[i].x - mean, a1 = v[i].y - mean, a2 = v[i].z - mean, a3 = v[i].w - mean;
+                qq += (a0 * a0 + a1 * a1) + (a2 * a2 + a3 * a3);
+            }
+        qq += __shfl_xor(qq, 1, 64);
+        qq += __shfl_xor(qq, 2, 64);
+        if (sub == 0) {
+            const float r = 1.0f / (sqrtf(qq * inv_c) + p.eps);
+            rowstat[2 * row] = r;
+            rowstat[2 * row + 1] = r * mean;
+        }
+    }
+
+    const int pl = lane & 31, hl = lane >> 5;
+    const bool active = ROWS == 128 || wid < 6;
+    const int kh = ROWS == 128 ? wid >> 2 : (wid >= 3 ? 1 : 0);
+    const int unit = ROWS == 128 ? (wid & 3) : (wid >= 3 ? wid - 3 : wid);
+    const int pb = ROWS == 128 ? unit : 0, blk0 = ROWS == 128 ? 0 : unit;
+    f32x16 acc[G::NB];
+#pragma unroll
+    for (int i = 0; i < G::NB; ++i)
+#pragma unroll
+        for (int r = 0; r < 16; ++r) acc[i][r] = 0.f;
+    const int fsw = (pl >> 1) & 7;
+    for (int c = 0; c < nch; ++c) {
+        const int later = nch - 1 - c < AS_RING - 2 ? nch - 1 - c : AS_RING - 2;
+        wait_vmcnt_le(later * npw);
+        asm volatile("s_waitcnt lgkmcnt(0)\n\ts_barrier" ::: "memory");
+        if (c + AS_RING - 1 < nch) issue(c + AS_RING - 1);
+        if (active) {
+            const float* Xs = smem + (c & (AS_RING - 1)) * G::SLOT + pb * (32 * 32);
+            const float* Ws = smem + (c & (AS_RING - 1)) * G::SLOT + ROWS * 32 + blk0 * (32 * 32);
+#pragma unroll
+            for (int q2 = 0; q2 < 2; ++q2) {
+                const int off = pl * 32 + (((2 * (2 * kh + q2) + hl) ^ fsw) << 2);
+                const float4 xv = *reinterpret_cast<const float4*>(Xs + off);
+                float4 wv[G::NB];
+#pragma unroll
+                for (int i = 0; i < G::NB; ++i) wv[i] = *reinterpret_cast<const float4*>(Ws + i * (32 * 32) + off);
+#pragma unroll
+                for (int e = 0; e < 4; ++e) {
+                    const float xe = e == 0 ? xv.x : e == 1 ? xv.y : e == 2 ? xv.z : xv.w;
+#pragma unroll
+                    for (int i = 0; i < G::NB; ++i)
+                        acc[i] = __builtin_amdgcn_mfma_f32_32x32x2f32(e == 0 ? wv[i].x : e == 1 ? wv[i].y : e == 2 ? wv[i].z : wv[i].w, xe, acc[i], 0, 0, 0);
+                }
+            }
+        }
+    }
+    __syncthreads();
+    if (active && kh == 1) {
+#pragma unroll
+        for (int i = 0; i < G::NB; ++i)
+#pragma unroll
+            for (int r = 0; r < 16; ++r) scr[((unit * G::NB + i) * 16 + r) * 64 + lane] = acc[i][r];
+    }
+    __syncthreads();
+    if (active && kh == 0) {
+        const int n = pb * 32 + pl;
+        const float r = rowstat[2 * n], rm = rowstat[2 * n + 1];
+#pragma unroll
+        for (int i = 0; i < G::NB; ++i) {
+            const int blk = blk0 + i;
+#pragma unroll
+            for (int q = 0; q < 4; ++q) {
+                const int d0 = 8 * q + 4 * hl;
+                float o4[4];
+#pragma unroll
+                for (int e = 0; e < 4; ++e) {
+                    const float a = acc[i][4 * q + e] + scr[((unit * G::NB + i) * 16 + 4 * q + e) * 64 + lane];
+                    o4[e] = r * a - rm * cfold[blk * 32 + d0 + e] + cfold[96 + blk * 32 + d0 + e];
+                }
+                if (blk == 0) {
+#pragma unroll
+                    for (int e = 0; e < 4; ++e) qs[n * (DH + 1) + d0 + e] = o4[e];
+                } else {
+                    *reinterpret_cast<float4*>((blk == 1 ? ks : vs) + n * DH + d0) = make_float4(o4[0], o4[1], o4[2], o4[3]);
+                }
+            }
+        }
+    }
+    __syncthreads();
+
+    {
+        const int d = tid & 31, ng = tid >> 5;
+        float m = -INFINITY;
+        for (int n = ng; n < ROWS; n += 16) m = fmaxf(m, ks[n * DH + d]);
+        smax[ng * DH + d] = m;
+        __syncthreads();
+        if (tid < DH) {
+            float mm = smax[tid];
+#pragma unroll
+            for (int j = 1; j < 16; ++j) mm = fmaxf(mm, smax[j * DH + tid]);
+            mx[tid] = mm;
+        }
+        __syncthreads();
+#pragma unroll
+        for (int j = 0; j < ROWS / 16; ++j) {
+            const int i = tid + j * 512;
+            ks[i] = __expf(ks[i] - mx[i & 31]);
+        }
+        __syncthreads();
+        float t = 0.f;
+        for (int n = ng; n < ROWS; n += 16) t += ks[n * DH + d];
+        dpart[ng * DH + d] = t;
+    }
+    {
+        constexpr int RPW = ROWS / 8;
+        f32x16 cacc;
+#pragma unroll
+        for (int r = 0; r < 16; ++r) cacc[r] = 0.f;
+        const float* kp = ks + (wid * RPW + hl) * DH + pl;
+        const float* vp = vs + (wid * RPW + hl) * DH + pl;
+#pragma unroll
+        for (int j = 0; j < RPW / 2; ++j) cacc = __builtin_amdgcn_mfma_f32_32x32x2f32(kp[j * 2 * DH], vp[j * 2 * DH], cacc, 0, 0, 0);
+#pragma unroll
+        for (int r = 0; r < 16; ++r) scr[(wid * 32 + (r & 3) + 8 * (r >> 2) + 4 * hl) * 33 + pl] = cacc[r];
+    }
+    __syncthreads();
+    const int md = (tid >> 3) & 31, me0 = (tid & 7) * 4;
+    if (tid < 256) {
+        float den = 0.f;
+#pragma unroll
+        for (int g = 0; g < 16; ++g) den += dpart[g * DH + md];
+#pragma unroll
+        for (int e = 0; e < 4; ++e) {
+            float t = scr[md * 33 + me0 + e];
+#pragma unroll
+            for (int w = 1; w < 8; ++w) t += scr[(w * 32 + md) * 33 + me0 + e];
+            own[2 * DH + md * DH + me0 + e] = t;
+        }
+        if (me0 == 0) { own[md] = mx[md]; own[DH + md] = den; }
+    }
+    __syncthreads();
+    unsigned* cnt = p.cnt + (b * 4 + h) * AS_CNT;
+    float* rec = p.rec + (long long)(b * 4 + h) * 2 * AS_REC;
+    if (wid == 0) {
+        unsigned* mine = reinterpret_cast<unsigned*>(rec + half * AS_REC);
+#pragma unroll
+        for (int i = 0; i < (2 * DH + DH * DH) / 64; ++i)
+            __hip_atomic_store(mine + lane + 64 * i, __float_as_uint(own[lane + 64 * i]), __ATOMIC_RELAXED, __HIP_MEMORY_SCOPE_AGENT);
+        asm volatile("s_waitcnt vmcnt(0)" ::: "memory");
+        if (lane == 0) {
+            __hip_atomic_fetch_add(cnt, 1u, __ATOMIC_RELAXED, __HIP_MEMORY_SCOPE_AGENT);
+            *gave_up = cl_wait_ge<2>(cnt, 2u, p.fail) ? 1 : 0;
+        }
+    }
+    __syncthreads();
+    const bool poisoned = *gave_up != 0;
+    if (tid < 256) {
+        const unsigned* theirs = reinterpret_cast<const unsigned*>(rec + (half ^ 1) * AS_REC);
+        const float tm = __uint_as_float(__hip_atomic_load(theirs + md, __ATOMIC_RELAXED, __HIP_MEMORY_SCOPE_AGENT));
+        const float td = __uint_as_float(__hip_atomic_load(theirs + DH + md, __ATOMIC_RELAXED, __HIP_MEMORY_SCOPE_AGENT));
+        float ta[4];
+#pragma unroll
+        for (int e = 0; e < 4; ++e)
+            ta[e] = __uint_as_float(__hip_atomic_load(theirs + 2 * DH + md * DH + me0 + e, __ATOMIC_RELAXED, __HIP_MEMORY_SCOPE_AGENT));
+        if (tid == 0) cl_depart(cnt, cnt + 1, 2u);
+        const float om = own[md], od = own[DH + md];
+        const float m0 = half ? tm : om, m1 = half ? om : tm;
+        const float d0 = half ? td : od, d1 = half ? od : td;
+        const float M = fmaxf(m0, m1);
+        const float w0 = expf(m0 - M), w1 = expf(m1 - M);
+        float den = 0.f;
+        den += d0 * w0;
+        den += d1 * w1;
+        const float inv = poisoned ? __builtin_nanf("") : 1.0f / den;
+        float c4[4];
+#pragma unroll
+        for (int e = 0; e < 4; ++e) {
+            const float oa = own[2 * DH + md * DH + me0 + e];
+            const float a0 = half ? ta[e] : oa, a1 = half ? oa : ta[e];
+            float a = 0.f;
+            a += a0 * w0;
+            a += a1 * w1;
+            c4[e] = a * inv;
+            cs[md * (DH + 4) + me0 + e] = c4[e];
+        }
+        if (half == 0) *reinterpret_cast<float4*>(p.ctx + (((long long)b * 4 + h) * DH + md) * DH + me0) = make_float4(c4[0], c4[1], c4[2], c4[3]);
+    }
+    __syncthreads();
+    if (wid < ROWS / 32) {
+        const int n0 = wid * 32;
+        f32x16 oacc;
+#pragma unroll
+        for (int r = 0; r < 16; ++r) oacc[r] = 0.f;
+        const float* qp = qs + (n0 + pl) * (DH + 1) + hl;
+        const float* cp = cs + hl * (DH + 4) + pl;
+#pragma unroll
+        for (int j = 0; j < DH / 2; ++j) oacc = __builtin_amdgcn_mfma_f32_32x32x2f32(qp[2 * j], cp[2 * j * (DH + 4)], oacc, 0, 0, 0);
+        float* op = p.out + ((long long)b * HW + half * ROWS + n0) * HC + h * DH + pl;
+#pragma unroll
+        for (int r = 0; r < 16; ++r) op[((r & 3) + 8 * (r >> 2) + 4 * hl) * HC] = oacc[r];
+    }
+}
+
 __global__ __launch_bounds__(256) void qkv_operand_pack_kernel(const float* __restrict__ lnw, float* __restrict__ wop, int heads, int cp,
                                                                long long total) {
     const int nch = cp >> 5, HC = heads * DH;
@@ -878,6 +1184,10 @@
     DDK_HIP(hipFuncSetAttribute(reinterpret_cast<const void*>(linattn_small_kernel<256>), hipFuncAttributeMaxDynamicSharedMemorySize, 160 * 1024));
     DDK_HIP(hipFuncSetAttribute(reinterpret_cast<const void*>(linattn_small_qkv_kernel<1>), hipFuncAttributeMaxDynamicSharedMemorySize, 160 * 1024));
     DDK_HIP(hipFuncSetAttribute(reinterpret_cast<const void*>(linattn_small_qkv_kernel<4>), hipFuncAttributeMaxDynamicSharedMemorySize, 160 * 1024));
+    DDK_HIP(hipFuncSetAttribute(reinterpret_cast<const void*>(attn_split_kernel<128>), hipFuncAttributeMaxDynamicSharedMemorySize,
+                                (int)(AttnSplitGeom<128>::LDS_FL * sizeof(float))));
+    DDK_HIP(hipFuncSetAttribute(reinterpret_cast<const void*>(attn_split_kernel<32>), hipFuncAttributeMaxDynamicSharedMemorySize,
+                                (int)(AttnSplitGeom<32>::LDS_FL * sizeof(float))));
     return DDK_OK;
 }
 
@@ -932,6 +1242,30 @@
     return check_launch("linattn_merge_kernel");
 }
 
+constexpr int AS_CUS = 256;
+bool attn_split_ok(int B, int HW, int C, int heads) {
+    return B > 0 && (HW == 64 || HW == 256) && C >= 32 && C <= 256 && C % 32 == 0 && heads == 4 && 8 * (long long)B <= AS_CUS &&
+           conv_wino_cluster_device_ok();
+}
+size_t attn_split_counter_words(int B) { return (size_t)B * 4 * AS_CNT; }
+size_t attn_split_record_floats(int B) { return (size_t)B * 4 * 2 * AS_REC; }
+size_t attn_split_workspace_bytes(int B) { return B > 0 ? (32 + attn_split_counter_words(B) + attn_split_record_floats(B)) * sizeof(float) : 0; }
+unsigned attention_cluster_timeouts() { return cl_timeouts_read(); }
+
+int attn_split(const float* x, const float* w, const float* c1, const float* c2, float ln_eps, float* ctx, float* out, int B, int HW, int C,
+               unsigned* counters, float* records, unsigned* fail, hipStream_t st) {
+    DDK_REQUIRE(x && w && c1 && c2 && ctx && out && counters && records, "attn_split: null pointer");
+    DDK_REQUIRE(attn_split_ok(B, HW, C, 4), "attn_split: needs H*W of 64 or 256, C % 32 == 0, C <= 256, 4 heads, 8 * B <= the CU count of a whole MI355X");
+    DDK_REQUIRE(aligned16(x) && aligned16(w) && aligned16(ctx) && aligned16(out) && aligned16(counters) && aligned16(records), "attn_split: alignment");
+    DDK_TRY(ensure_device_init());
+    const AttnSplitParams p{x, w, c1, c2, ln_eps, ctx, out, counters, records, fail, C};
+    if (HW == 256)
+        hipLaunchKernelGGL(attn_split_kernel<128>, dim3(2, 4, (unsigned)B), dim3(512), AttnSplitGeom<128>::LDS_FL * sizeof(float), st, p);
+    else
+        hipLaunchKernelGGL(attn_split_kernel<32>, dim3(2, 4, (unsigned)B), dim3(512), AttnSplitGeom<32>::LDS_FL * sizeof(float), st, p);
+    return check_launch("attn_split_kernel");
+}
+
 bool attn_fold_ok(int C, int heads) { return C == FOLD_C && heads * DH == FOLD_C; }
 size_t attn_fold_out_floats(int B) { return (size_t)B * (FOLD_C * FOLD_C + 2 * FOLD_C); }
 
@@ -971,6 +1305,20 @@
                              void* workspace, size_t workspace_bytes, ddk_stream_t s) {
     return ddk::attn_kvctx(x, w_kv, c1, c2, ln_eps, ctx, B, HW, workspace, workspace_bytes, ddk::as_stream(s));
 }
+size_t ddk_attention_split_workspace_bytes(int B) { return ddk::attn_split_workspace_bytes(B); }
+int ddk_attention_split_ok(int B, int HW, int C, int heads) { return ddk::attn_split_ok(B, HW, C, heads) ? 1 : 0; }
+int ddk_attention_split_from_x(const float* x, const float* w_folded, const float* c1, const float* c2, float ln_eps, float* ctx, float* out,
+                               int B, int HW, int C, int heads, void* workspace, size_t workspace_bytes, ddk_stream_t s) {
+    using namespace ddk;
+    DDK_REQUIRE(workspace && B > 0 && heads == 4, "attention_split_from_x: arguments (4 heads)");
+    if (workspace_bytes < attn_split_workspace_bytes(B)) {
+        set_error("attention_split_from_x: workspace too small (%zu < %zu)", workspace_bytes, attn_split_workspace_bytes(B));
+        return DDK_ERR_WORKSPACE;
+    }
+    unsigned* words = static_cast<unsigned*>(workspace);
+    return attn_split(x, w_folded, c1, c2, ln_eps, ctx, out, B, HW, C, words + 32, static_cast<float*>(workspace) + 32 + attn_split_counter_words(B),
+                      words, as_stream(s));
+}
 int ddk_attention_fold(const float* ctx, const float* wqg, const float* c1q, const float* c2q, const float* wout, const float* bout, float* A,
                        float* a1, float* a2, int B, int C, int heads, ddk_stream_t s) {
     return ddk::attn_fold(ctx, wqg, c1q, c2q, wout, bout, A, a1, a2, B, C, heads, ddk::as_stream(s));
diff --git a/downsampled-diffusion_amd/csrc/ddk_internal.h b/downsampled-diffusion_amd/csrc/ddk_internal.h
--- a/downsampled-diffusion_amd/csrc/ddk_internal.h
+++ b/downsampled-diffusion_amd/csrc/ddk_internal.h
@@ -152,12 +152,14 @@
 unsigned conv_wino_cluster_timeouts();
 unsigned conv_first_cluster_timeouts();
 unsigned level_chain_cluster_timeouts();
+unsigned attention_cluster_timeouts();
 constexpr size_t CL_PAIR_WORDS = 128 * 16;
 inline size_t cl_fail_offset(int B) { return (size_t)B * 8 * 16; }
 inline size_t cl_front_floats(int B) { return cl_fail_offset(B) + 16; }
 inline size_t cl_chain_offset(int B) { return cl_front_floats(B); }
 inline size_t cl_pair_offset(int B) { return cl_chain_offset(B) + (size_t)B * 64; }
-inline size_t cl_counter_floats(int B) { return cl_pair_offset(B) + CL_PAIR_WORDS; }
+inline size_t cl_attn_offset(int B) { return cl_pair_offset(B) + CL_PAIR_WORDS; }
+inline size_t cl_counter_floats(int B) { return cl_attn_offset(B) + (size_t)B * 4 * 32; }
 struct ClWords { unsigned* counters; unsigned* fail; };
 inline ClWords cl_words(float* cl, int B) { return {reinterpret_cast<unsigned*>(cl), reinterpret_cast<unsigned*>(cl + cl_fail_offset(B))}; }
 int cluster_fail_check(unsigned* word, hipStream_t st, const char* who, const char* tail);
@@ -237,6 +239,11 @@
               float* a1, float* a2, int B, int C, int heads, hipStream_t st);
 int linattn_apply(const float* qkv, const float* ctx, float* out, int B, int HW, int heads, hipStream_t st);
 int linattn_fused_small(const float* qkv, float* ctx, float* out, int B, int HW, int heads, hipStream_t st);
+bool attn_split_ok(int B, int HW, int C, int heads);
+size_t attn_split_counter_words(int B);
+size_t attn_split_record_floats(int B);
+int attn_split(const float* x, const float* w, const float* c1, const float* c2, float ln_eps, float* ctx, float* out, int B, int HW, int C,
+               unsigned* counters, float* records, unsigned* fail, hipStream_t st);
 bool linattn_small_qkv_ok(int HW, int C);
 int linattn_small_qkv_init_device();
 int qkv_operand_pack(const float* lnw, float* wop, int heads, int cp, hipStream_t st);
diff --git a/downsampled-diffusion_amd/csrc/unet_plan.hip b/downsampled-diffusion_amd/csrc/unet_plan.hip
--- a/downsampled-diffusion_amd/csrc/unet_plan.hip
+++ b/downsampled-diffusion_amd/csrc/unet_plan.hip
@@ -110,6 +110,7 @@
     int cluster_np_max = 8;
     bool cluster_split = true;
     bool attn_kvctx = true;
+    bool attn_split = true;
     bool fold_down_reduce = false;
     bool restore_fused = true;
     bool first_gn = true;
@@ -409,6 +410,7 @@
         {DDK_OPT_ATTENTION_KV_CONTEXT, true, [](ddk_unet& p, int v) { p.attn_kvctx = v != 0; }},
         {DDK_OPT_FIRST_GROUPNORM, true, [](ddk_unet& p, int v) { p.first_gn = v != 0; }},
         {DDK_OPT_RESTORE_FUSED_TAIL, true, [](ddk_unet& p, int v) { p.restore_fused = v != 0; }},
+        {DDK_OPT_ATTENTION_SPLIT, true, [](ddk_unet& p, int v) { p.attn_split = v != 0; }},
         {DDK_OPT_LEVEL_CHAIN, true, [](ddk_unet& p, int v) {
              p.level_chain = v == 1 ? 9 : v == 2 ? 1 : v == 3 ? 15 : v == 4 ? 6 : v == 8 ? 2 : v == 16 ? 4 : v != 0 ? 9 : 0;
          }},
@@ -433,7 +435,8 @@
 }
 extern "C" unsigned ddk_debug_cluster_timeouts(void) {
     unsigned sum = 0;
-    for (unsigned v : {ddk::conv_wino_cluster_timeouts(), ddk::conv_first_cluster_timeouts(), ddk::level_chain_cluster_timeouts()}) {
+    for (unsigned v : {ddk::conv_wino_cluster_timeouts(), ddk::conv_first_cluster_timeouts(), ddk::level_chain_cluster_timeouts(),
+                       ddk::attention_cluster_timeouts()}) {
         if (v == ~0u) return ~0u;
         sum += v;
     }
@@ -575,6 +578,7 @@
     if (attn_kvctx_ok(B, H * W, a.c, HEADS)) upd(ly.splitk, attn_kvctx_workspace_bytes(B, H * W) / 4);
     upd(ly.splitk, conv_workspace_bytes(DDK_CONV1X1, B, H, W, a.c, 3 * HIDDEN) / 4);
     upd(ly.splitk, conv_workspace_bytes(DDK_CONV1X1, B, H, W, HIDDEN, a.c) / 4);
+    if ((H * W == 64 || H * W == 256) && B <= 32) upd(ly.cl, cl_counter_floats(B) + attn_split_record_floats(B));
 }
 
 static bool chain_plain(const ResW& r, bool wino) {
@@ -870,6 +874,12 @@
                           a2, c.B, a.c, HEADS, c.st));
         const ConvLnFold lnA{a1, a2, LN_EPS};
         return conv1x1_ws(x, A, nullptr, x, out, M, a.c, &lnA, c.st, c.B);
+    }
+    if (!c.u.generic && c.u.attn_split && c.allow_cluster && a.c >= 128 && attn_split_ok(c.B, H * W, a.c, HEADS)) {
+        float* cl = c.W + c.ly.off_cl;
+        DDK_TRY(attn_split(x, c.P + a.qkv_lnw, c.P + a.ln_c1, c.P + a.ln_c2, LN_EPS, ctx, o, c.B, H * W, a.c,
+                           reinterpret_cast<unsigned*>(cl + cl_attn_offset(c.B)), cl + cl_counter_floats(c.B), cl_words(cl, c.B).fail, c.st));
+        return run_conv(c, DDK_CONV1X1, a.out, o, HIDDEN, nullptr, 0, x, out, H, W, a.c);
     }
     if (!c.u.generic && conv_ln_fold_ok(c.B, H, W, a.c, 3 * HIDDEN)) {
         const ConvLnFold ln{c.P + a.ln_c1, c.P + a.ln_c2, LN_EPS};
diff --git a/downsampled-diffusion_amd/ddk/lib.py b/downsampled-diffusion_amd/ddk/lib.py
--- a/downsampled-diffusion_amd/ddk/lib.py
+++ b/downsampled-diffusion_amd/ddk/lib.py
@@ -115,6 +115,9 @@
     "ddk_attention_kv_context_workspace_bytes": (_SZ, [_I, _I]),
     "ddk_attention_kv_context_ok": (_I, [_I, _I, _I, _I]),
     "ddk_attention_kv_context": (_I, [_P, _P, _P, _P, _F, _P, _I, _I, _P, _SZ, _P]),
+    "ddk_attention_split_workspace_bytes": (_SZ, [_I]),
+    "ddk_attention_split_ok": (_I, [_I, _I, _I, _I]),
+    "ddk_attention_split_from_x": (_I, [_P, _P, _P, _P, _F, _P, _P, _I, _I, _I, _I, _P, _SZ, _P]),
     "ddk_pack_qkv_operand": (_I, [_P, _P, _I, _I, _P]),
     "ddk_linattn_small_from_x": (_I, [_P, _P, _P, _P, _F, _P, _P, _I, _I, _I, _I, _P]),
     "ddk_conv3x3_gn_mish_ok": (_I, [_I, _I, _I, _I, _I, _I]),
diff --git a/downsampled-diffusion_amd/ddk/ops.py b/downsampled-diffusion_amd/ddk/ops.py
--- a/downsampled-diffusion_amd/ddk/ops.py
+++ b/downsampled-diffusion_amd/ddk/ops.py
@@ -1173,6 +1173,30 @@
     return out, ctx
 
 
+def attention_split_workspace(batch, device):
+    nbytes = L.load().ddk_attention_split_workspace_bytes(batch)
+    return torch.zeros(max(nbytes, 128) // 4, device=device, dtype=torch.float32)
+
+
+def attention_split_from_x(x, w_qkv, ln_g, ln_b, heads=4, eps=LN_EPS, workspace=None):
+    b, h, w, c = x.shape
+    lib = L.load()
+    if not lib.ddk_attention_split_ok(b, h * w, c, heads):
+        raise L.DDKError(f"attention_split_from_x: shape {tuple(x.shape)} with {heads} heads not eligible "
+                         "(H*W of 64 or 256, C % 32 == 0, C <= 256, 4 heads, 8 * B <= the CU count)")
+    wq = w_qkv.reshape(w_qkv.shape[0], -1).to(torch.float32)
+    g, bb = ln_g.reshape(-1).to(torch.float32), ln_b.reshape(-1).to(torch.float32)
+    lnw = (wq * g[None, :]).contiguous()
+    c1 = lnw.sum(dim=1).contiguous()
+    c2 = (wq * bb[None, :]).sum(dim=1).contiguous()
+    ws = attention_split_workspace(b, x.device) if workspace is None else workspace
+    ctx = torch.empty((b, heads, 32, 32), device=x.device, dtype=torch.float32)
+    out = torch.empty((b, h, w, heads * 32), device=x.device, dtype=torch.float32)
+    L.check(lib.ddk_attention_split_from_x(L.ptr(_f32(x)), L.ptr(lnw), L.ptr(c1), L.ptr(c2), eps, L.ptr(ctx), L.ptr(out), b, h * w, c, heads,
+                                           L.ptr(ws), ws.numel() * 4, L.stream()), "attention_split_from_x")
+    return out, ctx
+
+
 def linattn_train(qkv, heads=4):
     out, ctx = linattn(qkv, heads)
     b, h, w, _ = qkv.shape
diff --git a/downsampled-diffusion_amd/ddk/plan.py b/downsampled-diffusion_amd/ddk/plan.py
--- a/downsampled-diffusion_amd/ddk/plan.py
+++ b/downsampled-diffusion_amd/ddk/plan.py
@@ -99,6 +99,7 @@
     OPT_LEVEL_CHAIN = 7
     OPT_FIRST_GROUPNORM = 8
     OPT_RESTORE_FUSED_TAIL = 12
+    OPT_ATTENTION_SPLIT = 13
 
     def set_option(self, option, value):
         L.check(self._lib.ddk_unet_set_option(self.handle, option, int(value)), "unet_set_option")
diff --git a/include/ddk.h b/include/ddk.h
--- a/include/ddk.h
+++ b/include/ddk.h
@@ -133,6 +133,10 @@
 int ddk_attention_kv_context_ok(int B, int HW, int C, int heads);
 int ddk_attention_kv_context(const float* x, const float* w_kv, const float* c1, const float* c2, float ln_eps, float* ctx, int B, int HW,
                              void* workspace, size_t workspace_bytes, ddk_stream_t s);
+size_t ddk_attention_split_workspace_bytes(int B);
+int ddk_attention_split_ok(int B, int HW, int C, int heads);
+int ddk_attention_split_from_x(const float* x, const float* w_folded, const float* c1, const float* c2, float ln_eps, float* ctx, float* out,
+                               int B, int HW, int C, int heads, void* workspace, size_t workspace_bytes, ddk_stream_t s);
 int ddk_linattn_fused_small(const float* qkv, float* ctx, float* out, int B, int HW, int heads, ddk_stream_t s);
 int ddk_linattn_apply(const float* qkv, const float* ctx, float* out, int B, int HW, int heads, ddk_stream_t s);
 int ddk_pack_qkv_operand(const float* folded_w, float* dst, int heads, int c_pad, ddk_stream_t s);
@@ -220,6 +224,7 @@
 #define DDK_OPT_LEVEL_CHAIN 7
 #define DDK_OPT_FIRST_GROUPNORM 8
 #define DDK_OPT_RESTORE_FUSED_TAIL 12
+#define DDK_OPT_ATTENTION_SPLIT 13
 int ddk_unet_set_option(ddk_unet* u, int option, int value);
 int ddk_unet_cluster_check(const ddk_unet* u, void* workspace, int B, int H, int W, ddk_stream_t s);
 unsigned ddk_debug_cluster_timeouts(void);
```
